# jiny2001/dcscn-super-resolution

Hardware: AMD Instinct MI355X
Metric: LR Mpixels/sec at 48x48 patches, L12_F196to48 x2 (higher is better)
Workload: dtype f32-equivalent (3x3 stack, wide 1x1 convs and folded tail: f16 hi/lo split, 3 products per MAC, f32 accumulate -- error at the f32 kernels' level, same parity bars; everything else f32)

## Files before the change

dcscn-super-resolution_amd/build.py:

```python

import os
import shutil
import subprocess
import sys
from concurrent.futures import ThreadPoolExecutor

PKG_DIR = os.path.dirname(os.path.abspath(__file__))
CSRC = os.path.join(PKG_DIR, "csrc")
INCLUDE = os.path.join(os.path.dirname(PKG_DIR), "include")
LIB_NAME = "libdcscn_hip.so"
LIB_PATH = os.path.join(PKG_DIR, LIB_NAME)
SOURCES = ["api.hip", "graph.hip", "pack.hip", "exec.hip", "kernels.hip", "resample.hip", "ensemble.hip", "color.hip", "metrics.hip", "conv_k1.hip", "conv_k3.hip", "conv_k5.hip", "conv_k7.hip", "conv_wino2.hip", "conv_nin.hip", "feat_stream.hip", "conv_nin_h.hip", "conv_nin_h_w8.hip", "conv3_h.hip", "conv3_h8.hip", "conv5_h.hip", "conv3_h_p16.hip", "conv3_h8_p16.hip", "feat_stream_redo.hip", "feat3_stream.hip", "train.hip", "train_data.hip"]
HEADERS = [os.path.join(CSRC, h) for h in ("kernels.h", "plan.h", "conv_igemm.hpp", "conv_wino2.hpp", "conv_nin.hpp", "conv_variants.hpp", "feat_stream.hpp", "tail_stream.hpp", "feat3_stream.hpp",
                                              "split16.hpp", "split16_pack.hpp", "p16.hpp", "conv_nin_h.hpp", "conv3_h.hpp", "conv3_h8.hpp", "conv5_h.hpp")] + \
          [os.path.join(INCLUDE, "dcscn.h")]
ARCH = "gfx950"
NO_PK_F32 = ["-Xclang", "-target-feature", "-Xclang", "-packed-fp32-ops"]
FLAGS = ["--offload-arch=" + ARCH, "-O3", "-std=c++17", "-fPIC", "-Wall", "-Wno-unused-function"] + NO_PK_F32
EXTRA_FLAGS = {"conv_wino2.hip": ["-fno-slp-vectorize", "-Rpass-analysis=kernel-resource-usage"],
               "conv_nin.hip": ["-fno-slp-vectorize", "-Rpass-analysis=kernel-resource-usage"],
               "conv_nin_h.hip": ["-fno-slp-vectorize", "-Rpass-analysis=kernel-resource-usage"], "conv_nin_h_w8.hip": ["-fno-slp-vectorize", "-Rpass-analysis=kernel-resource-usage"], "conv3_h.hip": ["-fno-slp-vectorize", "-Rpass-analysis=kernel-resource-usage"], "conv3_h8.hip": ["-fno-slp-vectorize", "-Rpass-analysis=kernel-resource-usage"], "conv3_h_p16.hip": ["-fno-slp-vectorize", "-Rpass-analysis=kernel-resource-usage"], "conv3_h8_p16.hip": ["-fno-slp-vectorize", "-Rpass-analysis=kernel-resource-usage"], "conv5_h.hip": ["-fno-slp-vectorize", "-Rpass-analysis=kernel-resource-usage"], "color.hip": ["-ffp-contract=off"], "metrics.hip": ["-ffp-contract=off"], "feat_stream.hip": ["-fno-slp-vectorize", "-Rpass-analysis=kernel-resource-usage"], "feat_stream_redo.hip": ["-fno-slp-vectorize"], "feat3_stream.hip": ["-fno-slp-vectorize", "-Rpass-analysis=kernel-resource-usage"]}
NO_SCRATCH = ("conv_wino2.hip", "conv_nin.hip", "feat_stream.hip", "conv_nin_h.hip", "conv_nin_h_w8.hip", "conv_nin_h_w8.hip", "conv3_h.hip", "conv3_h8.hip", "conv5_h.hip", "conv3_h_p16.hip", "conv3_h8_p16.hip", "feat3_stream.hip")


def hipcc_path():
    for cand in (shutil.which("hipcc"), "/opt/rocm/bin/hipcc"):
        if cand and os.path.isfile(cand):
            return cand
    raise RuntimeError("hipcc not found; the DCSCN HIP extension cannot be built")


def _stale(target, deps):
    if not os.path.isfile(target):
        return True
    t = os.path.getmtime(target)
    return any(os.path.getmtime(d) > t for d in deps)


def _run(cmd):
    proc = subprocess.run(cmd, stdout=subprocess.PIPE, stderr=subprocess.STDOUT, text=True)
    proc.stdout = "\n".join(ln for ln in proc.stdout.splitlines() if "'-packed-fp32-ops' is not a recognized feature" not in ln)
    if proc.returncode != 0:
        raise RuntimeError("command failed (%d): %s\n%s" % (proc.returncode, " ".join(cmd), proc.stdout))
    if any(cmd[-3].endswith(n) for n in NO_SCRATCH if len(cmd) >= 3):
        import re
        bad = [ln for ln in proc.stdout.splitlines() if re.search(r"(ScratchSize \[bytes/lane\]|VGPRs Spill): [1-9]", ln)]
        if bad:
            os.remove(cmd[-1])
            raise RuntimeError("register spill in a kernel that must not spill (%s):\n%s" % (cmd[-3], "\n".join(bad[:6])))
        return ""
    return proc.stdout


def build(force=False, verbose=False):
    hipcc = hipcc_path()
    obj_dir = os.path.join(PKG_DIR, "build")
    os.makedirs(obj_dir, exist_ok=True)
    jobs = []
    objs = []
    for src in SOURCES:
        src_path = os.path.join(CSRC, src)
        obj = os.path.join(obj_dir, os.path.splitext(src)[0] + ".o")
        objs.append(obj)
        if force or _stale(obj, [src_path, os.path.abspath(__file__)] + HEADERS):
            jobs.append([hipcc] + FLAGS + EXTRA_FLAGS.get(src, []) + ["-I", INCLUDE, "-c", src_path, "-o", obj])
    if jobs:
        with ThreadPoolExecutor(max_workers=len(jobs)) as pool:
            for out in pool.map(_run, jobs):
                if verbose and out.strip():
                    print(out, file=sys.stderr)
    if jobs or force or _stale(LIB_PATH, objs):
        out = _run([hipcc, "--offload-arch=" + ARCH, "-shared", "-fPIC"] + objs + ["-o", LIB_PATH])
        if verbose and out.strip():
            print(out, file=sys.stderr)
    return LIB_PATH


if __name__ == "__main__":
    print(build(force="--force" in sys.argv, verbose=True))
```

dcscn-super-resolution_amd/csrc/api.hip:

```cpp
#include "plan.h"

#pragma clang fp contract(off)

namespace dcscn_impl {

thread_local std::string g_global_error;

void set_global_error(const char* fmt, ...) {
    char buf[512];
    va_list ap;
    va_start(ap, fmt);
    vsnprintf(buf, sizeof buf, fmt, ap);
    va_end(ap);
    g_global_error = buf;
}

int fail(dcscn_ctx* h, int code, const char* fmt, ...) {
    char buf[512];
    va_list ap;
    va_start(ap, fmt);
    vsnprintf(buf, sizeof buf, fmt, ap);
    va_end(ap);
    if (h) h->error = buf;
    g_global_error = buf;
// ... 22 lines not shown
    if (!out || layers <= 0 || gamma <= 0.0) {
        set_global_error("dcscn_filter_schedule: bad arguments");
        return DCSCN_ERR_INVALID_ARG;
    }
    std::vector<int> s;
    filter_schedule(layers, filters, std::min(filters, min_filters), gamma, s);
    for (int i = 0; i < layers; ++i) out[i] = s[i];
    return DCSCN_OK;
}

int dcscn_create(const dcscn_config* cfg, int device, dcscn_handle* out) {
    if (!cfg || !out) return fail(nullptr, DCSCN_ERR_INVALID_ARG, "dcscn_create: null argument");
    *out = nullptr;
    if (cfg->struct_size != (int32_t)sizeof(dcscn_config))
        return fail(nullptr, DCSCN_ERR_INVALID_ARG, "dcscn_create: struct_size %d != %zu", cfg->struct_size, sizeof(dcscn_config));
    dcscn_config c = *cfg;
    c.min_filters = std::min(c.filters, c.min_filters);
    c.reconstruct_layers = std::max(c.reconstruct_layers, 1);
    if (c.scale < 2 || c.scale > 4) return fail(nullptr, DCSCN_ERR_UNSUPPORTED, "scale %d (supported: 2, 3, 4)", c.scale);
    if (c.layers < 1 || c.layers > 256 || c.filters < 1) return fail(nullptr, DCSCN_ERR_INVALID_ARG, "bad layers/filters");
    if (c.layers > 1 && !(c.filters_decay_gamma > 0.0)) return fail(nullptr, DCSCN_ERR_INVALID_ARG, "filters_decay_gamma must be > 0");
    if (c.cnn_size != 1 && c.cnn_size != 3 && c.cnn_size != 5 && c.cnn_size != 7)
        return fail(nullptr, DCSCN_ERR_UNSUPPORTED, "cnn_size %d (supported: 1, 3, 5, 7)", c.cnn_size);
    if (c.channels != 1) return fail(nullptr, DCSCN_ERR_UNSUPPORTED, "channels %d (the reference itself only supports 1)", c.channels);
    if (c.batch_norm) return fail(nullptr, DCSCN_ERR_UNSUPPORTED, "batch_norm is not implemented");
    float dummy;
    if (kernel_act(c.activator, &dummy) < 0) return fail(nullptr, DCSCN_ERR_INVALID_ARG, "Not implemented activator:%d", c.activator);
    if (c.legacy_no_c && c.use_nin) return fail(nullptr, DCSCN_ERR_INVALID_ARG, "legacy_no_c requires use_nin = 0");
    if (c.reconstruct_layers > 1 && c.reconstruct_filters < 1) return fail(nullptr, DCSCN_ERR_INVALID_ARG, "reconstruct_filters must be positive");

    int ndev = 0;
    hipError_t e = hipGetDeviceCount(&ndev);
    if (e != hipSuccess || ndev <= 0)
        return fail(nullptr, DCSCN_ERR_HIP, "no HIP device available (%s); this library has no CPU fallback",
                    e != hipSuccess ? hipGetErrorString(e) : "device count 0");
    if (device < 0 || device >= ndev) return fail(nullptr, DCSCN_ERR_INVALID_ARG, "device %d out of range [0, %d)", device, ndev);

    dcscn_ctx* h = new (std::nothrow) dcscn_ctx();
    if (!h) return fail(nullptr, DCSCN_ERR_NOMEM, "out of host memory");
    h->cfg = c;
    h->device = device;
    int rc = DCSCN_OK;
    do {
        if ((e = hipSetDevice(device)) != hipSuccess) { rc = fail(h, DCSCN_ERR_HIP, "hipSetDevice: %s", hipGetErrorString(e)); break; }
        hipDeviceProp_t prop;
        if ((e = hipGetDeviceProperties(&prop, device)) != hipSuccess) { rc = fail(h, DCSCN_ERR_HIP, "hipGetDeviceProperties: %s", hipGetErrorString(e)); break; }
        if (strncmp(prop.gcnArchName, "gfx950", 6) != 0) {
            rc = fail(h, DCSCN_ERR_HIP, "device %d is %s; this library is built for gfx950 (MI355X) only", device, prop.gcnArchName);
            break;
        }
        h->n_cus = prop.multiProcessorCount > 0 ? prop.multiProcessorCount : 256;
        if ((e = hipStreamCreateWithFlags(&h->stream, hipStreamNonBlocking)) != hipSuccess) { rc = fail(h, DCSCN_ERR_HIP, "hipStreamCreate: %s", hipGetErrorString(e)); break; }
        if ((e = hipEventCreateWithFlags(&h->done_ev, hipEventDisableTiming)) != hipSuccess) { rc = fail(h, DCSCN_ERR_HIP, "hipEventCreate: %s", hipGetErrorString(e)); break; }
        if ((e = conv_init_kernels()) != hipSuccess) { rc = fail(h, DCSCN_ERR_HIP, "kernel attribute setup: %s", hipGetErrorString(e)); break; }
        {
            size_t free_b = 0, total_b = 0;
            if (hipMemGetInfo(&free_b, &total_b) == hipSuccess && free_b > 0)
                h->workspace_budget = std::min<int64_t>(h->workspace_budget, std::max<int64_t>((int64_t)(free_b / 10 * 6), (int64_t)256 << 20));
        }
        rc = build_graph(h);
    } while (0);
    if (rc != DCSCN_OK) {
        g_global_error = h->error;
        dcscn_destroy(h);
        return rc;
    }
    *out = h;
    return DCSCN_OK;
}

int dcscn_num_tensors(dcscn_handle h) { return h ? (int)h->tensors.size() : -DCSCN_ERR_INVALID_ARG; }

int dcscn_tensor_info(dcscn_handle h, int index, char* name, int name_capacity, int64_t* shape, int* rank) {
    if (!h) return DCSCN_ERR_INVALID_ARG;
    if (index < 0 || index >= (int)h->tensors.size() || !name || name_capacity <= 0 || !shape || !rank)
        return fail(h, DCSCN_ERR_INVALID_ARG, "dcscn_tensor_info: bad argument");
    const TensorSpec& t = h->tensors[index];
    snprintf(name, (size_t)name_capacity, "%s", t.name.c_str());
    *rank = (int)t.shape.size();
    for (int i = 0; i < 4; ++i) shape[i] = i < *rank ? t.shape[i] : 1;
    return DCSCN_OK;
}

int dcscn_set_tensor(dcscn_handle h, const char* name, const float* data, const int64_t* shape, int rank) {
    if (!h) return DCSCN_ERR_INVALID_ARG;
    if (!name || !data || !shape) return fail(h, DCSCN_ERR_INVALID_ARG, "dcscn_set_tensor: null argument");
    if (h->finalized) return fail(h, DCSCN_ERR_STATE, "dcscn_set_tensor after dcscn_finalize");
    auto it = h->tensor_index.find(name);
    if (it == h->tensor_index.end()) return fail(h, DCSCN_ERR_SHAPE, "variable '%s' is not part of this graph", name);
    TensorSpec& t = h->tensors[it->second];
    bool same = rank == (int)t.shape.size();
    for (int i = 0; same && i < rank; ++i) same = shape[i] == t.shape[i];
    if (!same) {
        std::string want, got;
        for (int64_t d : t.shape) want += std::to_string(d) + ",";
        for (int i = 0; i < rank && i < 8; ++i) got += std::to_string(shape[i]) + ",";
        return fail(h, DCSCN_ERR_SHAPE, "variable '%s': shape [%s] does not match graph shape [%s]", name, got.c_str(), want.c_str());
    }
    size_t count = 1;
    for (int64_t d : t.shape) count *= (size_t)d;
    for (size_t i = 0; i < count; ++i)
        if (!std::isfinite(data[i])) return fail(h, DCSCN_ERR_INVALID_ARG, "variable '%s' holds a non-finite value", name);
    t.data.assign(data, data + count);
    t.set = true;
    return DCSCN_OK;
}

static int pack_ops(dcscn_ctx* h) {
    const size_t first = h->device_allocs.size();
    int rc = DCSCN_OK;
    for (Op& op : h->ops) {
        rc = finalize_op(h, op);
        if (rc) break;
    }
    h->pack_allocs.insert(h->pack_allocs.end(), h->device_allocs.begin() + first, h->device_allocs.end());
    h->device_allocs.resize(first);
    return rc;
}

}

namespace dcscn_impl {
int repack_weights(dcscn_ctx* h) {
    HIP_TRY(h, hipDeviceSynchronize());
    if (h->graph_exec) {
        (void)hipGraphExecDestroy(h->graph_exec);
        h->graph_exec = nullptr;
        h->graph_key = dcscn_ctx::GraphKey();
    }
    h->graph_seen = dcscn_ctx::GraphKey();
    for (void* p : h->pack_allocs) (void)hipFree(p);
    h->pack_allocs.clear();
    return pack_ops(h);
}
}

extern "C" {

int dcscn_finalize(dcscn_handle h) {
    if (!h) return DCSCN_ERR_INVALID_ARG;
    if (h->finalized) return DCSCN_OK;
    for (const TensorSpec& t : h->tensors)
        if (!t.set) return fail(h, DCSCN_ERR_MISSING_TENSOR, "variable '%s' was never set", t.name.c_str());
    HIP_TRY(h, hipSetDevice(h->device));
    if (h->fold_tail) fold_linear_tail(h);
    fuse_tail_stream(h);
    fuse_feat_stream(h);
    densify_features(h);
    fuse_feat3_stream(h);
    fold_whole_tail(h);
    int rc0 = pack_ops(h);
    if (rc0) return rc0;
    plan_p16(h);
    for (Op& op : h->ops) {
        int rc = DCSCN_OK;
        if (op.kind == OP_CONV && op.shape.nin && op.h16.on && op.h16.in16_ok) {
            op.h16.h_tab16.assign((size_t)4 * op.h16.n_chunks, NinSrcQuad{0, 0, 0});
            rc = upload(h, op.h16.h_tab16.data(), op.h16.h_tab16.size() * sizeof(NinSrcQuad), (void**)&op.h16.d_tab16);
            if (rc) return rc;
        }
        auto alloc_srctab = [&](Op& o) {
            if (o.multi.empty()) return (int)DCSCN_OK;
            o.h_srctab.assign(std::max<size_t>((size_t)4 * o.n_chunks, (size_t)8 * ((o.cin_phys + kNinHKC - 1) / kNinHKC)), NinSrcQuad{0, 0, 0});
            return upload(h, o.h_srctab.data(), o.h_srctab.size() * sizeof(NinSrcQuad), (void**)&o.d_srctab);
        };
        rc = alloc_srctab(op);
        if (rc) return rc;
        for (Op& sub : op.fused) {
            rc = alloc_srctab(sub);
            if (rc) return rc;
        }
    }
    h->finalized = true;
    return DCSCN_OK;
}

int dcscn_num_layers(dcscn_handle h) { return h ? (int)h->layers.size() : -DCSCN_ERR_INVALID_ARG; }

int dcscn_layer_info_get(dcscn_handle h, int index, dcscn_layer_info* out) {
    if (!h) return DCSCN_ERR_INVALID_ARG;
    if (!out || index < 0 || index >= (int)h->layers.size()) return fail(h, DCSCN_ERR_INVALID_ARG, "dcscn_layer_info_get: bad argument");
    *out = h->layers[index];
    return DCSCN_OK;
}

int dcscn_num_ops(dcscn_handle h) { return h ? (int)h->ops.size() : -DCSCN_ERR_INVALID_ARG; }

int dcscn_op_info_get(dcscn_handle h, int index, dcscn_op_info* out) {
    if (!h) return DCSCN_ERR_INVALID_ARG;
    if (!out || index < 0 || index >= (int)h->ops.size()) return fail(h, DCSCN_ERR_INVALID_ARG, "dcscn_op_info_get: bad argument");
    const Op& op = h->ops[index];
    memset(out, 0, sizeof *out);
    snprintf(out->name, sizeof out->name, "%s", op.name.c_str());
    const bool s16 = op_on_split16(h, op);
    snprintf(out->kernel, sizeof out->kernel, "%s", kernel_name(op_kernel(h, op)));
    out->kernel_size = op.ks;
    out->in_channels = op.cin;
    out->out_channels = op.cout;
    out->resolution = op.res;
    out->macs_per_lr_pixel = op.macs;
    out->bytes_per_lr_pixel = op.bytes;
    out->executed_macs_per_lr_pixel = op.macs;
    if (op.kind == OP_FOLDX && h->finalized && s16) {
        out->nt = 1; out->kc = 32; out->n_tiles = 1;
        out->executed_macs_per_lr_pixel = 3 * 25 * (int64_t)op.h16.n_chunks * 32 * 16;
    }
    if (op.kind == OP_CONV && h->finalized) {
        out->mt = op.shape.mt; out->nt = op.shape.nt; out->kc = op.shape.kc; out->n_tiles = op.n_tiles;
        const int64_t r2 = (int64_t)op.res * op.res;
        const int64_t k_exec = (int64_t)op.n_chunks * op.shape.kc;
        if (s16) {
            const int64_t tiles = (int64_t)op.h16.n_tiles * (op.h16.nt - 1) + op.h16.n_full;
            out->nt = op.h16.nt; out->kc = 32; out->n_tiles = op.h16.n_tiles;
            const int64_t ksteps = op.shape.nin ? op.h16.n_chunks : op.fold_s > 0 ? 25 * (int64_t)op.h16.n_chunks
                                                : 9 * (int64_t)(op.h16.n_chunks - (op.h16.tail_octs ? 1 : 0)) + (op.h16.tail_octs ? c3h_tail_steps(op.h16.tail_octs) : 0);
            out->executed_macs_per_lr_pixel = r2 * 3 * ksteps * 32 * tiles * 16;
        } else if (op.shape.nin) {
            const int64_t tiles = (int64_t)op.n_tiles * (op.shape.nt - 1) + op.n_full;
            out->executed_macs_per_lr_pixel = r2 * k_exec * tiles * 16;
        } else if (op.shape.wino) {
            const int64_t tiles = (int64_t)op.n_tiles * (op.shape.nt - 1) + op.n_full;
            out->executed_macs_per_lr_pixel = r2 * 4 * k_exec * tiles * 16;
        } else {
            out->executed_macs_per_lr_pixel = r2 * op.ks * op.ks * k_exec * (int64_t)op.n_tiles * op.shape.nt * 16;
        }
    }
    return DCSCN_OK;
}

int dcscn_set_option(dcscn_handle h, const char* key, int64_t value) {
    if (!h) return DCSCN_ERR_INVALID_ARG;
    if (!key) return fail(h, DCSCN_ERR_INVALID_ARG, "dcscn_set_option: null key");
    if (!strcmp(key, "sub_batch_pixels")) {
        if (value < 1) return fail(h, DCSCN_ERR_INVALID_ARG, "sub_batch_pixels must be >= 1");
        h->sub_batch_pixels = value;
        return DCSCN_OK;
    }
    if (!strcmp(key, "workspace_budget_bytes")) {
        if (value < 1) return fail(h, DCSCN_ERR_INVALID_ARG, "workspace_budget_bytes must be >= 1");
        h->workspace_budget = value;
        return DCSCN_OK;
    }
    if (!strcmp(key, "spatial_tiling")) {
        h->spatial_tiling = value != 0;
        return DCSCN_OK;
    }
    if (!strcmp(key, "fold_whole_tail")) {
        if (h->finalized) return fail(h, DCSCN_ERR_STATE, "the fold_whole_tail option must be set before dcscn_finalize");
        h->fold_whole = value != 0;
        return DCSCN_OK;
    }
    if (!strcmp(key, "fold_linear_tail")) {
        if (h->finalized) return fail(h, DCSCN_ERR_STATE, "the fold_linear_tail option must be set before dcscn_finalize");
        h->fold_tail = value != 0;
        h->fold_force = value == 2;
        return DCSCN_OK;
    }
    if (!strcmp(key, "stream_tail")) {
        if (h->finalized) return fail(h, DCSCN_ERR_STATE, "the stream_tail option must be set before dcscn_finalize");
        h->stream_tail = value != 0;
        return DCSCN_OK;
    }
    if (!strcmp(key, "stream_features")) {
        if (h->finalized) return fail(h, DCSCN_ERR_STATE, "the stream_features option must be set before dcscn_finalize");
        h->stream_features = value != 0;
        return DCSCN_OK;
    }
    if (!strcmp(key, "stream_nin")) {
        if (h->finalized) return fail(h, DCSCN_ERR_STATE, "the stream_nin option must be set before dcscn_finalize");
        h->stream_nin = value != 0;
        return DCSCN_OK;
    }
    if (!strcmp(key, "stream_dense")) {
        if (h->finalized) return fail(h, DCSCN_ERR_STATE, "the stream_dense option must be set before dcscn_finalize");
        h->stream_dense = value != 0;
        return DCSCN_OK;
    }
    if (!strcmp(key, "dense_features")) {
        if (h->finalized) return fail(h, DCSCN_ERR_STATE, "the dense_features option must be set before dcscn_finalize");
        h->dense_features = value != 0;
        return DCSCN_OK;
    }
    if (!strcmp(key, "nin_gemm")) {
        if (h->finalized) return fail(h, DCSCN_ERR_STATE, "the nin_gemm option must be set before dcscn_finalize");
        h->nin = value != 0;
        return DCSCN_OK;
    }
    if (!strcmp(key, "winograd")) {
        if (h->finalized) return fail(h, DCSCN_ERR_STATE, "the winograd option must be set before dcscn_finalize");
        h->winograd = value != 0;
        return DCSCN_OK;
    }
    if (!strcmp(key, "split16")) {
        h->split16 = value != 0;
        h->split16_mask = value == 2 ? 1 : value == 3 ? 2 : 3;
        return DCSCN_OK;
    }
    if (!strcmp(key, "p16")) {
        h->p16 = value != 0;
        return DCSCN_OK;
    }
    if (!strcmp(key, "conv3_h8")) {
        h->conv3_h8 = value != 0;
        return DCSCN_OK;
    }
    if (!strcmp(key, "nin_h8")) {
        h->nin_h8 = value != 0;
        return DCSCN_OK;
    }
    if (!strcmp(key, "debug_digest")) {
        if ((int)h->ops.size() + 1 > 1024) return fail(h, DCSCN_ERR_UNSUPPORTED, "debug_digest: more than 1023 launches");
        h->debug_digest = value != 0;
        return DCSCN_OK;
    }
    if (!strcmp(key, "debug_poison")) {
        h->debug_poison = (int)value;
        return DCSCN_OK;
    }
    if (!strcmp(key, "profile")) {
        h->profile = value != 0;
        return DCSCN_OK;
    }
    if (!strcmp(key, "graph_replay")) {
        h->graph_replay = value != 0;
        if (!h->graph_replay && h->graph_exec) {
            (void)hipGraphExecDestroy(h->graph_exec);
            h->graph_exec = nullptr;
        }
        h->graph_seen = dcscn_ctx::GraphKey{};
        return DCSCN_OK;
    }
    return fail(h, DCSCN_ERR_INVALID_ARG, "unknown option '%s'", key);
}

int dcscn_forward_device(dcscn_handle h, const float* x, const float* x2, float* y, int n, int height, int width, void* stream) {
    if (!h) return DCSCN_ERR_INVALID_ARG;
    if (h->finalized)
        if (int rc_ = train_sync_inference(h)) return rc_;
    return run_forward(h, x, x2, y, n, height, width, stream ? (hipStream_t)stream : h->stream);
}

static int ensure_io(dcscn_ctx* h, size_t lr_floats, size_t hr_floats) {
    int rc = grow(h, &h->io_x, &h->io_x_cap, lr_floats, h->stream, DCSCN_ERR_HIP);
    if (!rc) rc = grow(h, &h->io_x2, &h->io_x2_cap, hr_floats, h->stream, DCSCN_ERR_HIP);
    if (!rc) rc = grow(h, &h->io_y, &h->io_y_cap, hr_floats, h->stream, DCSCN_ERR_HIP);
    return rc;
}

static int forward_host_chunked(dcscn_ctx* h, const float* x, const float* x2, float* y, int n, int height, int width) {
    const int s = h->cfg.scale;
    const size_t lr1 = (size_t)height * width, hr1 = lr1 * s * s;
    int rc = ensure_io(h, lr1 * n, hr1 * n);
    if (rc) return rc;
    const int chunks = (hr1 * n * sizeof(float) >= ((size_t)8 << 20) && n >= 8) ? 4 : 1;
    while ((int)h->host_ev.size() < chunks) {
        hipEvent_t e;
        HIP_TRY(h, hipEventCreateWithFlags(&e, hipEventDisableTiming));
        h->host_ev.push_back(e);
    }
    int begin[5];
    for (int i = 0; i <= chunks; ++i) begin[i] = (int)((int64_t)n * i / chunks);
    auto span = [&](int i, int* b, int* cnt) { *b = begin[chunks - 1 - i] ; *cnt = begin[chunks - i] - begin[chunks - 1 - i]; };
    auto download = [&](int i) -> int {
        int b, cnt;
        span(i, &b, &cnt);
        HIP_TRY(h, hipEventSynchronize(h->host_ev[i]));
        HIP_TRY(h, hipMemcpy(y + (size_t)b * hr1, h->io_y + (size_t)b * hr1, (size_t)cnt * hr1 * sizeof(float), hipMemcpyDeviceToHost));
        return DCSCN_OK;
    };
    for (int i = 0; i < chunks; ++i) {
        int b, cnt;
        span(i, &b, &cnt);
        if (cnt > 0) {
            HIP_TRY(h, hipMemcpy(h->io_x + (size_t)b * lr1, x + (size_t)b * lr1, (size_t)cnt * lr1 * sizeof(float), hipMemcpyHostToDevice));
            if (x2) HIP_TRY(h, hipMemcpy(h->io_x2 + (size_t)b * hr1, x2 + (size_t)b * hr1, (size_t)cnt * hr1 * sizeof(float), hipMemcpyHostToDevice));
            else rc = resize_device(h, h->io_x + (size_t)b * lr1, h->io_x2 + (size_t)b * hr1, cnt, height, width, height * s, width * s, h->stream);
            if (!rc) rc = run_forward(h, h->io_x + (size_t)b * lr1, h->io_x2 + (size_t)b * hr1, h->io_y + (size_t)b * hr1, cnt, height, width, h->stream);
            if (rc) return rc;
        }
        HIP_TRY(h, hipEventRecord(h->host_ev[i], h->stream));
        if (i > 0 && (rc = download(i - 1))) return rc;
    }
    if ((rc = download(chunks - 1))) return rc;
    return DCSCN_OK;
}

int dcscn_forward(dcscn_handle h, const float* x, const float* x2, float* y, int n, int height, int width) {
    if (!h) return DCSCN_ERR_INVALID_ARG;
    if (!h->finalized) return fail(h, DCSCN_ERR_STATE, "dcscn_forward before dcscn_finalize");
    if (int rc_ = train_sync_inference(h)) return rc_;
    if (n < 0 || height <= 0 || width <= 0) return fail(h, DCSCN_ERR_INVALID_ARG, "bad shape n=%d h=%d w=%d", n, height, width);
    if (n == 0) return DCSCN_OK;
    if (!x || !x2 || !y) return fail(h, DCSCN_ERR_INVALID_ARG, "null image pointer");
    HIP_TRY(h, hipSetDevice(h->device));
    return forward_host_chunked(h, x, x2, y, n, height, width);
}

int dcscn_resample_table(int in_size, int out_size, int* ksize, int* bounds, double* weights, int capacity) {
    if (in_size <= 0 || out_size <= 0 || !ksize) return DCSCN_ERR_INVALID_ARG;
    std::vector<int> b;
    std::vector<double> k;
    *ksize = resample_coeffs(in_size, out_size, &b, &k);
    if (!bounds && !weights) return DCSCN_OK;
    if (!bounds || !weights || capacity < (int)k.size()) return DCSCN_ERR_INVALID_ARG;
    std::copy(b.begin(), b.end(), bounds);
    std::copy(k.begin(), k.end(), weights);
    return DCSCN_OK;
}

int dcscn_resize_bicubic(dcscn_handle h, const float* in, float* out, int n, int height, int width, int out_height, int out_width) {
    if (!h) return DCSCN_ERR_INVALID_ARG;
    if (n < 0 || height <= 0 || width <= 0 || out_height <= 0 || out_width <= 0)
        return fail(h, DCSCN_ERR_INVALID_ARG, "bad shape n=%d %dx%d -> %dx%d", n, height, width, out_height, out_width);
    if (n == 0) return DCSCN_OK;
    if (!in || !out) return fail(h, DCSCN_ERR_INVALID_ARG, "null image pointer");
    HIP_TRY(h, hipSetDevice(h->device));
    const size_t ni = (size_t)n * height * width, no = (size_t)n * out_height * out_width;
    int rc = grow(h, &h->rs_in, &h->rs_in_cap, ni, h->stream);
    if (!rc) rc = grow(h, &h->rs_out, &h->rs_out_cap, no, h->stream);
    if (rc) return rc;
    HIP_TRY(h, hipMemcpy(h->rs_in, in, ni * sizeof(float), hipMemcpyHostToDevice));
    rc = resize_device(h, h->rs_in, h->rs_out, n, height, width, out_height, out_width, h->stream);
    if (rc) return rc;
    HIP_TRY(h, hipStreamSynchronize(h->stream));
    HIP_TRY(h, hipMemcpy(out, h->rs_out, no * sizeof(float), hipMemcpyDeviceToHost));
    return DCSCN_OK;
}

int dcscn_resize_bicubic_device(dcscn_handle h, const float* in, float* out, int n, int height, int width, int out_height,
                                int out_width, void* stream) {
    if (!h) return DCSCN_ERR_INVALID_ARG;
    if (n < 0 || height <= 0 || width <= 0 || out_height <= 0 || out_width <= 0)
        return fail(h, DCSCN_ERR_INVALID_ARG, "bad shape n=%d %dx%d -> %dx%d", n, height, width, out_height, out_width);
    if (n == 0) return DCSCN_OK;
    if (!in || !out) return fail(h, DCSCN_ERR_INVALID_ARG, "null image pointer");
    HIP_TRY(h, hipSetDevice(h->device));
    hipStream_t st = stream ? (hipStream_t)stream : h->stream;
    if (h->has_last && h->last_stream != st) HIP_TRY(h, hipStreamWaitEvent(st, h->done_ev, 0));
    const int rc = resize_device(h, in, out, n, height, width, out_height, out_width, st);
    if (rc) return rc;
    return forward_done(h, st);
}

int dcscn_forward_lr(dcscn_handle h, const float* x, float* y, int n, int height, int width) {
    if (!h) return DCSCN_ERR_INVALID_ARG;
    if (!h->finalized) return fail(h, DCSCN_ERR_STATE, "dcscn_forward_lr before dcscn_finalize");
    if (int rc_ = train_sync_inference(h)) return rc_;
    if (n < 0 || height <= 0 || width <= 0) return fail(h, DCSCN_ERR_INVALID_ARG, "bad shape n=%d h=%d w=%d", n, height, width);
    if (n == 0) return DCSCN_OK;
    if (!x || !y) return fail(h, DCSCN_ERR_INVALID_ARG, "null image pointer");
    HIP_TRY(h, hipSetDevice(h->device));
    return forward_host_chunked(h, x, nullptr, y, n, height, width);
}

static int ensemble_on_device(dcscn_ctx* h, int height, int width, int n) {
    const int s = h->cfg.scale;
    const size_t lr = (size_t)height * width, hr = lr * s * s;
    const int na = std::min(n, 4), nb = n - na;
    int rc = grow(h, &h->ens_x, &h->ens_x_cap, n * lr, h->stream);
    if (!rc) rc = grow(h, &h->ens_x2, &h->ens_x2_cap, n * hr, h->stream);
    if (!rc) rc = grow(h, &h->ens_y, &h->ens_y_cap, n * hr, h->stream);
    if (!rc) rc = grow(h, &h->ens_out, &h->ens_out_cap, 2 * hr, h->stream);
// ... 158 lines not shown

static int metric_shape(dcscn_ctx* h, int height, int width, int border, const char* what, int* sh, int* sw) {
    if (height <= 0 || width <= 0) return fail(h, DCSCN_ERR_INVALID_ARG, "%s: bad shape h=%d w=%d", what, height, width);
    if (border < 0) return fail(h, DCSCN_ERR_INVALID_ARG, "%s: negative border_size %d (win_size cannot be placed)", what, border);
    *sh = height - 2 * border;
    *sw = width - 2 * border;
    if (*sh < kMetricTaps || *sw < 1)
        return fail(h, DCSCN_ERR_INVALID_ARG, "%s: win_size exceeds image extent (%d x %d after shaving %d: needs %d rows and 1 column)", what,
                    *sh, *sw, border, kMetricTaps);
    return DCSCN_OK;
}

static int metric_buffers(dcscn_ctx* h, int sh, int sw) {
    return grow(h, &h->met_buf, &h->met_buf_cap, (size_t)8 + 2 * (size_t)metric_segments(sh) * sw, h->stream);
}

static int metric_enqueue(dcscn_ctx* h, int slot, const double* a64, const float* a32, const double* b64, const float* b32, int width, int border,
                          int sh, int sw) {
    double* part_s = h->met_buf + 8;
    long long* part_e = reinterpret_cast<long long*>(part_s + (size_t)metric_segments(sh) * sw);
    HIP_TRY(h, metrics_launch(a64, a32, b64, b32, width, border, sh, sw, metric_weights(), part_s, part_e,
                              reinterpret_cast<long long*>(h->met_buf) + 4 * slot, h->stream));
    return DCSCN_OK;
}

static int metric_download(dcscn_ctx* h, dcscn_metrics* first, dcscn_metrics* second) {
    long long words[8];
    HIP_TRY(h, hipStreamSynchronize(h->stream));
    HIP_TRY(h, hipMemcpy(words, h->met_buf, sizeof words, hipMemcpyDeviceToHost));
    dcscn_metrics* outs[2] = {first, second};
    for (int i = 0; i < 2; ++i) {
        if (!outs[i]) continue;
        dcscn_metrics& m = *outs[i];
        m.sq_err_sum = words[4 * i];
        m.n_pixels = words[4 * i + 1];
        memcpy(&m.ssim, &words[4 * i + 2], sizeof(double));
        const double err = (double)m.sq_err_sum / (double)m.n_pixels;
        m.psnr = m.sq_err_sum == 0 ? (double)INFINITY : 10.0 * log10((255.0 * 255.0) / err);
    }
    return DCSCN_OK;
}

int dcscn_psnr_ssim(dcscn_handle h, const double* a, const double* b, int height, int width, int border_size, dcscn_metrics* out) {
    if (!h) return DCSCN_ERR_INVALID_ARG;
    if (!a || !b || !out) return fail(h, DCSCN_ERR_INVALID_ARG, "dcscn_psnr_ssim: null pointer");
    int sh, sw;
    int rc = metric_shape(h, height, width, border_size, "dcscn_psnr_ssim", &sh, &sw);
    if (rc) return rc;
    HIP_TRY(h, hipSetDevice(h->device));
    const size_t n = (size_t)height * width;
    rc = grow(h, &h->col_d, &h->col_d_cap, 2 * n, h->stream);
    if (!rc) rc = grow(h, &h->col_d2, &h->col_d2_cap, 2 * n, h->stream);
    if (!rc) rc = metric_buffers(h, sh, sw);
    if (rc) return rc;
    const double* da = reinterpret_cast<const double*>(h->col_d);
    const double* db = reinterpret_cast<const double*>(h->col_d2);
    HIP_TRY(h, hipMemcpy(h->col_d, a, n * sizeof(double), hipMemcpyHostToDevice));
    HIP_TRY(h, hipMemcpy(h->col_d2, b, n * sizeof(double), hipMemcpyHostToDevice));
    rc = metric_enqueue(h, 0, da, nullptr, db, nullptr, width, border_size, sh, sw);
    if (!rc) rc = metric_download(h, out, nullptr);
    return rc;
}

int dcscn_evaluate_rgb_metrics(dcscn_handle h, const uint8_t* rgb, int height, int width, int n_ensemble, int border_size, dcscn_metrics* model,
                               dcscn_metrics* bicubic, double* y) {
    if (!h) return DCSCN_ERR_INVALID_ARG;
    if (!h->finalized) return fail(h, DCSCN_ERR_STATE, "dcscn_evaluate_rgb_metrics before dcscn_finalize");
    if (!rgb || !model) return fail(h, DCSCN_ERR_INVALID_ARG, "dcscn_evaluate_rgb_metrics: null pointer");
    int sh, sw;
    int rc = metric_shape(h, height, width, border_size, "dcscn_evaluate_rgb_metrics", &sh, &sw);
    if (!rc) rc = evaluate_rgb_on_device(h, rgb, height, width, n_ensemble, "dcscn_evaluate_rgb_metrics");
    if (!rc) rc = metric_buffers(h, sh, sw);
    if (rc) return rc;
    const double* true_y = reinterpret_cast<const double*>(h->col_d);
    rc = metric_enqueue(h, 0, true_y, nullptr, n_ensemble > 1 ? reinterpret_cast<const double*>(h->ens_out) : nullptr,
                        n_ensemble > 1 ? nullptr : h->io_y, width, border_size, sh, sw);
    if (!rc && bicubic) rc = metric_enqueue(h, 1, true_y, nullptr, nullptr, h->io_x2, width, border_size, sh, sw);
    if (!rc) rc = metric_download(h, model, bicubic);
    if (!rc && y) rc = download_sr(h, (size_t)height * width, n_ensemble, y);
    return rc;
}

int dcscn_sr_rgb(dcscn_handle h, const uint8_t* rgb, const uint8_t* rgb_upscaled, int height, int width, int n_ensemble, double* y, double* rgb_out) {
    if (!h) return DCSCN_ERR_INVALID_ARG;
    if (!h->finalized) return fail(h, DCSCN_ERR_STATE, "dcscn_sr_rgb before dcscn_finalize");
    if (int rc_ = train_sync_inference(h)) return rc_;
    if (!rgb || !rgb_upscaled || !rgb_out) return fail(h, DCSCN_ERR_INVALID_ARG, "dcscn_sr_rgb: null pointer");
    if (n_ensemble < 1 || n_ensemble > 8) return fail(h, DCSCN_ERR_INVALID_ARG, "n_ensemble %d outside [1, 8]", n_ensemble);
    if (height <= 0 || width <= 0) return fail(h, DCSCN_ERR_INVALID_ARG, "bad shape h=%d w=%d", height, width);
    HIP_TRY(h, hipSetDevice(h->device));
    const int s = h->cfg.scale;
    const size_t lrn = (size_t)height * width, hr = lrn * s * s;
    int rc = ensure_io(h, lrn, hr);
    if (!rc) rc = grow(h, &h->col_rgb, &h->col_rgb_cap, (3 * hr + 3) / 4 + (3 * lrn + 3) / 4 + 4, h->stream);
    if (!rc) rc = grow(h, &h->col_d2, &h->col_d2_cap, 6 * hr, h->stream);
    if (rc) return rc;
    uint8_t* d_up = reinterpret_cast<uint8_t*>(h->col_rgb);
    uint8_t* d_lr = d_up + ((3 * hr + 15) & ~(size_t)15);
    HIP_TRY(h, hipMemcpy(d_lr, rgb, 3 * lrn, hipMemcpyHostToDevice));
    HIP_TRY(h, hipMemcpy(d_up, rgb_upscaled, 3 * hr, hipMemcpyHostToDevice));
    HIP_TRY(h, rgb_to_y_launch(d_lr, nullptr, h->io_x, (long long)lrn, h->stream));
    rc = sr_from_lr_on_device(h, height, width, n_ensemble);
    if (rc) return rc;
    HIP_TRY(h, y_cbcr_to_rgb_launch(n_ensemble > 1 ? reinterpret_cast<const double*>(h->ens_out) : nullptr, n_ensemble > 1 ? nullptr : h->io_y,
                                    nullptr, d_up, reinterpret_cast<double*>(h->col_d2), (long long)hr, h->stream));
    if (y) rc = download_sr(h, hr, n_ensemble, y);
    else HIP_TRY(h, hipStreamSynchronize(h->stream));
    if (rc) return rc;
    HIP_TRY(h, hipMemcpy(rgb_out, h->col_d2, 3 * hr * sizeof(double), hipMemcpyDeviceToHost));
    return DCSCN_OK;
}

int dcscn_get_profile(dcscn_handle h, double* ms, int capacity) {
    if (!h) return DCSCN_ERR_INVALID_ARG;
    if (!ms || capacity < 0) return fail(h, DCSCN_ERR_INVALID_ARG, "dcscn_get_profile: bad argument");
    const int nops = (int)h->ops.size();
    std::vector<double> acc(nops + 1, 0.0);
    const int forwards = h->ev_forwards;
    if (h->ev_used > 0) {
        HIP_TRY(h, hipDeviceSynchronize());
        const size_t launches = h->ev_used / 2;
        for (size_t l = 0; l < launches && l < h->ev_op.size(); ++l) {
            float t = 0.0f;
            HIP_TRY(h, hipEventElapsedTime(&t, h->ev[2 * l], h->ev[2 * l + 1]));
            acc[std::min(std::max(h->ev_op[l], 0), nops)] += t;
        }
    }
    h->ev_used = 0;
    h->ev_forwards = 0;
    h->ev_op.clear();
    if (forwards > 1)
        for (double& v : acc) v /= forwards;
    for (int i = 0; i < std::min(capacity, nops + 1); ++i) ms[i] = acc[i];
    return DCSCN_OK;
}

int dcscn_debug_digests(dcscn_handle h, uint64_t* out, int capacity) {
    if (!h) return DCSCN_ERR_INVALID_ARG;
    if (!out || capacity < 0) return fail(h, DCSCN_ERR_INVALID_ARG, "dcscn_debug_digests: bad argument");
    if (!h->d_digest) return fail(h, DCSCN_ERR_STATE, "dcscn_debug_digests: no forward has run with the debug_digest option on");
    HIP_TRY(h, hipDeviceSynchronize());
    const int n = std::min(capacity, (int)h->ops.size() + 1);
    HIP_TRY(h, hipMemcpy(out, h->d_digest, (size_t)n * sizeof(uint64_t), hipMemcpyDeviceToHost));
    return DCSCN_OK;
}

int64_t dcscn_workspace_bytes(dcscn_handle h) { return h ? (int64_t)h->arena_bytes : -1; }

int dcscn_num_presplit_tensors(dcscn_handle h) {
    if (!h) return -DCSCN_ERR_INVALID_ARG;
    if (!h->finalized || !p16_active(h)) return 0;
    int n = 0;
    for (const WsBuf& b : h->bufs) n += b.p16_ok && b.stride > 0;
    return n;
}

const char* dcscn_last_error(dcscn_handle h) { return h ? h->error.c_str() : g_global_error.c_str(); }

int dcscn_get_stream(dcscn_handle h, void** stream) {
    if (!h) return DCSCN_ERR_INVALID_ARG;
    if (!stream) return fail(h, DCSCN_ERR_INVALID_ARG, "dcscn_get_stream: null pointer");
    *stream = (void*)h->stream;
    return DCSCN_OK;
}

int dcscn_synchronize(dcscn_handle h) {
    if (!h) return DCSCN_ERR_INVALID_ARG;
    HIP_TRY(h, hipSetDevice(h->device));
    if (h->has_last) HIP_TRY(h, hipStreamSynchronize(h->last_stream));
    HIP_TRY(h, hipStreamSynchronize(h->stream));
    return DCSCN_OK;
}

int dcscn_destroy(dcscn_handle h) {
    if (!h) return DCSCN_OK;
    (void)hipSetDevice(h->device);
    if (h->has_last) (void)hipStreamSynchronize(h->last_stream);
    if (h->stream) (void)hipStreamSynchronize(h->stream);
    if (h->graph_exec) (void)hipGraphExecDestroy(h->graph_exec);
    if (h->done_ev) (void)hipEventDestroy(h->done_ev);
    for (hipEvent_t e : h->host_ev) (void)hipEventDestroy(e);
    for (hipEvent_t e : h->ev) (void)hipEventDestroy(e);
    train_free(h);
    train_batches_free(h);
    for (void* p : h->device_allocs) (void)hipFree(p);
    for (void* p : h->pack_allocs) (void)hipFree(p);
    if (h->arena) (void)hipFree(h->arena);
    if (h->d_zrec) (void)hipFree(h->d_zrec);
    if (h->d_digest) (void)hipFree(h->d_digest);
    for (float* p : {h->io_x, h->io_x2, h->io_y, h->tile_x, h->tile_x2, h->tile_y, h->rs_tmp, h->rs_in, h->rs_out, h->ens_x, h->ens_x2, h->ens_y, h->ens_out, h->col_rgb, h->col_d,
                     h->col_d2, h->col_y32})
        if (p) (void)hipFree(p);
    if (h->met_buf) (void)hipFree(h->met_buf);
    if (h->stream) (void)hipStreamDestroy(h->stream);
    delete h;
    return DCSCN_OK;
}

}
```

dcscn-super-resolution_amd/csrc/conv_nin_h.hip:

```cpp
#include "conv_nin_h.hpp"

namespace dcscn {

constexpr int kNinHStages = 3;
constexpr int kNinHMaxTable = 16 * 1024;

template <int NT>
static hipError_t nin_h_set_attr() {
    hipError_t e = hipFuncSetAttribute(reinterpret_cast<const void*>(&conv_nin_h<NT, 0, kNinHStages>), hipFuncAttributeMaxDynamicSharedMemorySize,
                                       NinHGeom<NT, kNinHStages>::LDS_BYTES);
    if (e != hipSuccess) return e;
    e = hipFuncSetAttribute(reinterpret_cast<const void*>(&conv_nin_h<NT, 2, kNinHStages>), hipFuncAttributeMaxDynamicSharedMemorySize,
                            NinHGeom<NT, kNinHStages>::LDS_BYTES + kNinHMaxTable);
    if (e != hipSuccess) return e;
    return hipFuncSetAttribute(reinterpret_cast<const void*>(&conv_nin_h<NT, 1, kNinHStages>), hipFuncAttributeMaxDynamicSharedMemorySize,
                               NinHGeom<NT, kNinHStages>::LDS_BYTES + kNinHMaxTable);
}

hipError_t nin_h8_init_kernels();
hipError_t nin_h8_launch(const ConvArgs& a, int n_groups, hipStream_t stream);
constexpr int kNinH8MinChunks = 32;

hipError_t nin_h_init_kernels() {
    hipError_t e = nin_h8_init_kernels();
    if (e != hipSuccess) return e;
    e = nin_h_set_attr<1>();
    if (e == hipSuccess) e = nin_h_set_attr<2>();
    if (e == hipSuccess) e = nin_h_set_attr<3>();
    if (e == hipSuccess) e = nin_h_set_attr<4>();
    if (e == hipSuccess) e = nin_h_set_attr<5>();
    return e != hipSuccess ? e : nin_h_set_attr<6>();
}

template <int NT>
static hipError_t nin_h_launch_one(const ConvArgs& a, int n_groups, hipStream_t stream) {
    using G = NinHGeom<NT, kNinHStages>;
    const long long npix = (long long)a.N * a.H * a.W;
    const dim3 grid((unsigned)((npix + G::PIX - 1) / G::PIX), (unsigned)n_groups);
    if (a.in16.base) {
        const size_t table = (size_t)a.n_chunks * 64;
        if (!a.srctab || table > (size_t)kNinHMaxTable || npix > kP16MaxPixels) return hipErrorInvalidValue;
        hipLaunchKernelGGL((conv_nin_h<NT, 2, kNinHStages>), grid, dim3(NinHGeom<NT, kNinHStages>::THREADS), G::LDS_BYTES + table, stream, a);
    } else if (a.srctab) {
        const size_t table = (size_t)a.n_chunks * 128;
        if (table > (size_t)kNinHMaxTable) return hipErrorInvalidValue;
        hipLaunchKernelGGL((conv_nin_h<NT, 1, kNinHStages>), grid, dim3(NinHGeom<NT, kNinHStages>::THREADS), G::LDS_BYTES + table, stream, a);
    } else {
        hipLaunchKernelGGL((conv_nin_h<NT, 0, kNinHStages>), grid, dim3(NinHGeom<NT, kNinHStages>::THREADS), G::LDS_BYTES, stream, a);
    }
    return hipGetLastError();
}

hipError_t nin_h_launch(int nt, const ConvArgs& a, int n_groups, bool w8, hipStream_t stream) {
    if (a.n_full < 1 || a.n_full > n_groups || (nt == 1 && a.n_full != n_groups) || !a.wpack16) return hipErrorInvalidValue;
    if (w8 && nt == 6 && a.in16.base && a.n_chunks >= kNinH8MinChunks && a.n_full == n_groups) return nin_h8_launch(a, n_groups, stream);
    switch (nt) {
        case 1: return nin_h_launch_one<1>(a, n_groups, stream);
        case 2: return nin_h_launch_one<2>(a, n_groups, stream);
        case 3: return nin_h_launch_one<3>(a, n_groups, stream);
        case 4: return nin_h_launch_one<4>(a, n_groups, stream);
        case 5: return nin_h_launch_one<5>(a, n_groups, stream);
        case 6: return nin_h_launch_one<6>(a, n_groups, stream);
        default: return hipErrorInvalidValue;
    }
}

}
```

dcscn-super-resolution_amd/csrc/conv_nin_h.hpp:

```cpp
#pragma once
#include "conv_nin.hpp"
#include "split16.hpp"
#include "p16.hpp"

namespace dcscn {

template <int NT, int S = 2, int WAVES = 4, int MT_ = 2>
struct NinHGeom {
    static constexpr int W = WAVES;
    static constexpr int THREADS = 64 * W;
    static constexpr int KC = 32;
    static constexpr int PIX = 16 * MT_ * W;
    static constexpr int MT = MT_;
    static constexpr int PSTRIDE = 128;
    static constexpr int A_SLOTS = PIX * 8;
    static constexpr int A_DMA = A_SLOTS / 64;
    static constexpr int A_BYTES = A_SLOTS * 16;
    static constexpr int A_ROUNDS = A_DMA / W;
    static constexpr int B_BYTES = NT * 2048;
    static constexpr int B_PIECES = 2 * NT;
    static constexpr int B_ROUNDS = (B_PIECES + W - 1) / W;
    static constexpr int B_STAGE = B_BYTES;
    static constexpr int B_BASE = S * A_BYTES;
    static constexpr int BA_BASE = S * A_BYTES + 2 * B_STAGE;
    static constexpr int LDS_BYTES = BA_BASE + NT * 128;
    static_assert(S == 2 || S == 3, "2 or 3 input stages");
};

template <int NT, int NTV, int SRC, int S, int WAVES, int MT>
__device__ __forceinline__ void conv_nin_h_body(const ConvArgs& a, float* smem, long long pix0, int ntile) {
    using G = NinHGeom<NT, S, WAVES, MT>;
    constexpr bool MULTI = SRC != 0, IN16 = SRC == 2;
    const int tid = threadIdx.x;
    const int lane = tid & 63;
    const int wave = __builtin_amdgcn_readfirstlane(tid >> 6);
    const int lj = lane & 15;
    const int lk = lane >> 4;
    const long long npix = (long long)a.N * a.H * a.W;
    const unsigned lds0 = (unsigned)(uintptr_t)(__attribute__((address_space(3))) float*)smem;

    const int d_kq = (((lane & 7) >> 1) - ((lane >> 4) & 3)) & 3;
    const int dq = 2 * d_kq + ((lane & 1) ^ (d_kq & 1));
    unsigned a_off[G::A_ROUNDS];
    long long a_pix[G::A_ROUNDS];
    static_for<0, G::A_ROUNDS>([&](auto r_) DCSCN_INL {
        constexpr int r = decltype(r_)::value;
        long long p = pix0 + (wave + G::W * r) * 8 + (lane >> 3);
        p = p < npix ? p : npix - 1;
        a_pix[r] = p;
        a_off[r] = (unsigned)((p - pix0) * a.in_stride * 4);
    });
    const float* a_base = a.in + (size_t)pix0 * a.in_stride + a.in_off;
    const char* b_base = reinterpret_cast<const char*>(a.wpack16) + (size_t)ntile * a.n_chunks * G::B_BYTES;
    const unsigned b_off = (unsigned)(lane * 16);

    auto dma_b = [&](auto r_, int chunk, unsigned stage) DCSCN_INL {
        constexpr int r = decltype(r_)::value;
        const int piece = (wave + G::W * r) % G::B_PIECES;
        glds16(b_base + (size_t)chunk * G::B_BYTES + 1024 * piece, b_off, lds0 + G::B_BASE + stage * G::B_STAGE + (unsigned)piece * 1024u);
    };
    typedef const volatile __attribute__((address_space(3))) u32x4* lds_u32x4_ptr;
    u32x4 ent = {0u, 0u, 0u, 0u};
    auto load_ent = [&](int chunk) DCSCN_INL {
        if constexpr (IN16) ent = *(lds_u32x4_ptr)(uintptr_t)(lds0 + G::LDS_BYTES + (unsigned)(chunk * 4 + d_kq) * 16u);
        else if constexpr (MULTI) ent = *(lds_u32x4_ptr)(uintptr_t)(lds0 + G::LDS_BYTES + (unsigned)(chunk * 8 + dq) * 16u);
    };
    auto dma_a = [&](auto r_, int chunk, unsigned stage) DCSCN_INL {
        constexpr int r = decltype(r_)::value;
        if constexpr (MULTI) {
            const char* src = reinterpret_cast<const char*>(((unsigned long long)ent.y << 32) | ent.x) + (unsigned long long)a_pix[r] * ent.z + (IN16 ? (dq & 1) * 16 : 0);
            glds16v(src, lds0 + stage * G::A_BYTES + (unsigned)(wave + G::W * r) * 1024u);
        } else {
            const int c0 = chunk * G::KC + 4 * dq;
            glds16(a_base, a_off[r] + (unsigned)((c0 < a.cin_phys ? c0 : 0) * 4), lds0 + stage * G::A_BYTES + (unsigned)(wave + G::W * r) * 1024u);
        }
    };

    {
        if constexpr (MULTI)
            for (int i = tid; i < (IN16 ? 4 : 8) * a.n_chunks; i += G::THREADS)
                *reinterpret_cast<f32x4*>(reinterpret_cast<char*>(smem) + G::LDS_BYTES + 16 * i) = reinterpret_cast<const f32x4*>(a.srctab)[i];
        __syncthreads();
    }

    if (tid < NTV * 4) *reinterpret_cast<f32x4*>(reinterpret_cast<char*>(smem) + G::BA_BASE + tid * 16) = reinterpret_cast<const f32x4*>(a.bias + ntile * NT * 16)[tid];
    else if (tid >= 64 && tid < 64 + NTV * 4 && a.act == ACT_ALPHA)
        *reinterpret_cast<f32x4*>(reinterpret_cast<char*>(smem) + G::BA_BASE + NT * 64 + (tid - 64) * 16) = reinterpret_cast<const f32x4*>(a.alpha + ntile * NT * 16)[tid - 64];

    f32x4 acc[G::MT][NTV];
    static_for<0, G::MT>([&](auto m_) DCSCN_INL {
        static_for<0, NTV>([&](auto n_) DCSCN_INL { acc[decltype(m_)::value][decltype(n_)::value] = f32x4{0.0f, 0.0f, 0.0f, 0.0f}; });
    });

    const unsigned a_rel = (unsigned)((16 * G::MT * wave + lj) * G::PSTRIDE + ((((lk + (lj >> 1)) & 3) << 1) | (lk & 1)) * 16);
    const unsigned a_lane = lds0 + a_rel, a_lane2 = lds0 + (a_rel ^ 16u);
    const unsigned b_lane = lds0 + (unsigned)(G::B_BASE + lane * 16);
    typedef const volatile __attribute__((address_space(3))) f32x4* lds_f32x4_ptr;
    typedef const volatile __attribute__((address_space(3))) h8* lds_h8_ptr;
    const float m1 = opaque_minus_one();

    const int last = a.n_chunks - 1;
    static_for<0, G::B_ROUNDS>([&](auto r_) DCSCN_INL { dma_b(r_, 0, 0); });
    load_ent(0);
    static_for<0, S>([&](auto st_) DCSCN_INL {
        constexpr int st = decltype(st_)::value;
        static_for<0, G::A_ROUNDS>([&](auto r_) DCSCN_INL { dma_a(r_, last < st ? last : st, st); });
        load_ent(last < st + 1 ? last : st + 1);
    });
    asm volatile("s_waitcnt vmcnt(0)" ::: "memory");
    __syncthreads();
    f32x4 xa[G::MT], xb[G::MT];
    static_for<0, G::MT>([&](auto m_) DCSCN_INL {
        constexpr int m = decltype(m_)::value;
        xa[m] = *(lds_f32x4_ptr)(uintptr_t)(a_lane + m * 16 * G::PSTRIDE);
        xb[m] = *(lds_f32x4_ptr)(uintptr_t)(a_lane2 + m * 16 * G::PSTRIDE);
    });
    __syncthreads();
    unsigned sa = 0;
    for (int chunk = 0; chunk < a.n_chunks; ++chunk) {
        const unsigned sb = chunk & 1;
        const int cb = chunk + 1 < last ? chunk + 1 : last;
        const int ca = chunk + S < last ? chunk + S : last;
        const unsigned sn = sa + 1 == S ? 0 : sa + 1;
        const unsigned Bs = b_lane + sb * G::B_STAGE;
        const unsigned An = a_lane + sn * G::A_BYTES, An2 = a_lane2 + sn * G::A_BYTES;
        static_for<0, G::B_ROUNDS>([&](auto r_) DCSCN_INL { dma_b(r_, cb, sb ^ 1); });
        f32x4 na[G::MT], nb[G::MT];
        static_for<0, G::MT>([&](auto m_) DCSCN_INL {
            constexpr int m = decltype(m_)::value;
            h8 xh, xl;
            if constexpr (IN16) { xh = __builtin_bit_cast(h8, xa[m]); xl = __builtin_bit_cast(h8, xb[m]); }
            else split8(xa[m], xb[m], m1, xh, xl);
            static_for<0, NTV>([&](auto n_) DCSCN_INL {
                constexpr int n = decltype(n_)::value;
                const h8 wh = *(lds_h8_ptr)(uintptr_t)(Bs + (2 * n) * 1024);
                const h8 wl = *(lds_h8_ptr)(uintptr_t)(Bs + (2 * n + 1) * 1024);
                acc[m][n] = __builtin_amdgcn_mfma_f32_16x16x32_f16(wl, xh, acc[m][n], 0, 0, 0);
                acc[m][n] = __builtin_amdgcn_mfma_f32_16x16x32_f16(wh, xl, acc[m][n], 0, 0, 0);
                acc[m][n] = __builtin_amdgcn_mfma_f32_16x16x32_f16(wh, xh, acc[m][n], 0, 0, 0);
                if constexpr (m * NTV + n < G::A_ROUNDS) dma_a(std::integral_constant<int, m * NTV + n>{}, ca, sa);
            });
            if constexpr (m == G::MT - 1 && G::MT * NTV < G::A_ROUNDS)
                static_for<G::MT * NTV, G::A_ROUNDS>([&](auto r_) DCSCN_INL { dma_a(r_, ca, sa); });
            na[m] = *(lds_f32x4_ptr)(uintptr_t)(An + m * 16 * G::PSTRIDE);
            nb[m] = *(lds_f32x4_ptr)(uintptr_t)(An2 + m * 16 * G::PSTRIDE);
        });
        load_ent(chunk + S + 1 < last ? chunk + S + 1 : last);
        if constexpr (S == 2) asm volatile("s_waitcnt vmcnt(0)" ::: "memory");
        else asm volatile("s_waitcnt vmcnt(%0)" ::"n"(G::A_ROUNDS) : "memory");
        __syncthreads();
        static_for<0, G::MT>([&](auto m_) DCSCN_INL { xa[decltype(m_)::value] = na[decltype(m_)::value]; xb[decltype(m_)::value] = nb[decltype(m_)::value]; });
        sa = sn;
    }
    if constexpr (S > 2) asm volatile("s_waitcnt vmcnt(0)" ::: "memory");

    const int cbase = ntile * NT * 16 + 4 * lk;
    const int obase = cbase - 16 * (ntile > a.n_full ? ntile - a.n_full : 0);
    const int act = a.act;
    const float inv = a.inv_scale;
    float chk[G::MT];
    static_for<0, G::MT>([&](auto m_) DCSCN_INL { chk[decltype(m_)::value] = 0.0f; });
    const float zero = opaque_zero();
    const h2 zero2 = p16_opaque_zero2();
    auto finish = [&](auto act_c) DCSCN_INL {
        constexpr int ACT_C = decltype(act_c)::value;
        const int act_e = ACT_C >= 0 ? ACT_C : act;
        static_for<0, NTV>([&](auto n_) DCSCN_INL {
            constexpr int n = decltype(n_)::value;
            const int c = obase + n * 16;
            const f32x4 bv = *reinterpret_cast<const f32x4*>(reinterpret_cast<const char*>(smem) + G::BA_BASE + (n * 4 + lk) * 16);
            f32x4 av = {0.0f, 0.0f, 0.0f, 0.0f};
            if (act_e == ACT_ALPHA) av = *reinterpret_cast<const f32x4*>(reinterpret_cast<const char*>(smem) + G::BA_BASE + NT * 64 + (n * 4 + lk) * 16);
            const bool first = c < a.split;
            float* optr = first ? a.out0.ptr : a.out1.ptr;
            const int ostride = first ? a.out0.stride : a.out1.stride;
            const int ooff = first ? a.out0.off : a.out1.off;
            const int owidth = first ? a.out0.width : a.out1.width;
            const int cc = first ? c : c - a.split;
            const OutDesc& od = first ? a.out0 : a.out1;
            if (od.p16.base != nullptr) {
                const int oct0 = (ooff + cc - 4 * lk) >> 3;
                const int chunk = oct0 >> 2, rem = od.p16.octs - 4 * chunk;
                const int rec = rem >= 4 ? 128 : 32 * rem;
                char* base = od.p16.base + (long long)chunk * od.p16.plane + 128 + (oct0 & 3) * 32 + lk * 16;
                const bool chan_ok = oct0 + (lk >> 1) < od.p16.octs;
                static_for<0, G::MT>([&](auto m_) DCSCN_INL {
                    constexpr int m = decltype(m_)::value;
                    const long long p = pix0 + 16 * G::MT * wave + 16 * m + lj;
                    f32x4 v = acc[m][n] * inv + bv;
                    v.x = activate1(v.x, av.x, act_e);
                    v.y = activate1(v.y, av.y, act_e);
                    v.z = activate1(v.z, av.z, act_e);
                    v.w = activate1(v.w, av.w, act_e);
                    if (ACT_C < 0 && p < npix && chan_ok) chk[m] = nonfinite_acc(chk[m], acc[m][n], zero);
                    const u32x4 unit = p16_unit(v, m1, chk[m], zero2, p < npix && chan_ok);
                    if (p < npix && chan_ok) *reinterpret_cast<u32x4*>(base + (size_t)p * rec) = unit;
                });
            } else if (cc < owidth) {
                static_for<0, G::MT>([&](auto m_) DCSCN_INL {
                    constexpr int m = decltype(m_)::value;
                    const long long p = pix0 + 16 * G::MT * wave + 16 * m + lj;
                    f32x4 v = acc[m][n] * inv + bv;
                    v.x = activate1(v.x, av.x, act_e);
                    v.y = activate1(v.y, av.y, act_e);
                    v.z = activate1(v.z, av.z, act_e);
                    v.w = activate1(v.w, av.w, act_e);
                    if (p < npix) {
                        chk[m] = nonfinite_acc(chk[m], acc[m][n], zero);
                        *reinterpret_cast<f32x4*>(optr + (size_t)p * ostride + ooff + cc) = v;
                    }
                });
            }
        });
    };
    if (act == ACT_ALPHA) finish(std::integral_constant<int, ACT_ALPHA>{});
    else if (act == ACT_NONE) finish(std::integral_constant<int, ACT_NONE>{});
    else finish(std::integral_constant<int, -1>{});
    static_for<0, G::MT>([&](auto m_) DCSCN_INL {
        constexpr int m = decltype(m_)::value;
        if (chk[m] != chk[m] && a.redo) {
            long long p = pix0 + 16 * G::MT * wave + 16 * m + lj;
            p = p < npix ? p : npix - 1;
            a.redo[0] = 1;
            a.redo[1 + (int)(p / ((long long)a.H * a.W))] = 1;
        }
    });
}

template <int NT, int SRC = 0, int S = 2, int WPS = 2, int WAVES = 4, int MT = 2>
__global__ __launch_bounds__(64 * WAVES, (WPS * WAVES / 4) * 128 / (16 * MT * WAVES) > 0 ? (WPS * WAVES / 4) * 128 / (16 * MT * WAVES) : 1) void conv_nin_h(const ConvArgs a) {
    extern __shared__ __attribute__((aligned(16))) float smem[];
    const long long pix0 = (long long)blockIdx.x * NinHGeom<NT, S, WAVES, MT>::PIX;
    const int ntile = blockIdx.y;
    if (ntile < a.n_full) conv_nin_h_body<NT, NT, SRC, S, WAVES, MT>(a, smem, pix0, ntile);
    else if constexpr (NT >= 2) conv_nin_h_body<NT, NT - 1, SRC, S, WAVES, MT>(a, smem, pix0, ntile);
}

}
```

dcscn-super-resolution_amd/csrc/conv_nin_h_w8.hip:

```cpp
#include "conv_nin_h.hpp"

namespace dcscn {

constexpr int kNinH8Stages = 3;
constexpr int kNinH8MaxTable = 16 * 1024;
constexpr int kNinH8Waves = 8, kNinH8Tiles = 2;

hipError_t nin_h8_init_kernels() {
    return hipFuncSetAttribute(reinterpret_cast<const void*>(&conv_nin_h<6, 2, kNinH8Stages, 2, kNinH8Waves, kNinH8Tiles>),
                               hipFuncAttributeMaxDynamicSharedMemorySize, NinHGeom<6, kNinH8Stages, kNinH8Waves, kNinH8Tiles>::LDS_BYTES + kNinH8MaxTable);
}

hipError_t nin_h8_launch(const ConvArgs& a, int n_groups, hipStream_t stream) {
    using G = NinHGeom<6, kNinH8Stages, kNinH8Waves, kNinH8Tiles>;
    const long long npix = (long long)a.N * a.H * a.W;
    const size_t table = (size_t)a.n_chunks * 64;
    if (!a.in16.base || !a.srctab || table > (size_t)kNinH8MaxTable || npix > kP16MaxPixels) return hipErrorInvalidValue;
    const dim3 grid((unsigned)((npix + G::PIX - 1) / G::PIX), (unsigned)n_groups);
    hipLaunchKernelGGL((conv_nin_h<6, 2, kNinH8Stages, 2, kNinH8Waves, kNinH8Tiles>), grid, dim3(G::THREADS), G::LDS_BYTES + table, stream, a);
    return hipGetLastError();
}

}
```

dcscn-super-resolution_amd/csrc/exec.hip:

```cpp
#include "plan.h"

#pragma clang fp contract(off)

namespace dcscn_impl {


static int ensure_workspace(dcscn_ctx* h, int nb, int H, int W, hipStream_t stream) {
    const bool want16 = p16_active(h);
    if (h->arena && nb <= h->lay_n && H == h->lay_h && W == h->lay_w && want16 == h->p16_now) return DCSCN_OK;
    std::vector<size_t> offsets(h->bufs.size()), sizes(h->bufs.size());
    size_t total = 0;
    for (size_t i = 0; i < h->bufs.size(); ++i) {
        const WsBuf& b = h->bufs[i];
        offsets[i] = total;
        sizes[i] = ws_tensor_bytes(b, (long long)nb * H * b.res * W * b.res, want16);
        total += ws_granules(sizes[i]);
    }
    const size_t redo_ints = 1 + (size_t)nb;
    h->redo_off = total;
    h->redo_ints = redo_ints;
    total += ws_granules(redo_ints * sizeof(int32_t));
    total = std::max<size_t>(total, 256);
    if (total > h->arena_bytes) {
        if (h->has_last) HIP_TRY(h, hipStreamSynchronize(h->last_stream));
        HIP_TRY(h, hipStreamSynchronize(h->stream));
        if (h->arena) HIP_TRY(h, hipFree(h->arena));
        h->arena = nullptr;
        h->arena_bytes = 0;
        h->lay_n = h->lay_h = h->lay_w = 0;
        hipError_t e = hipMalloc(&h->arena, total);
        if (e != hipSuccess) {
            (void)hipGetLastError();
            return fail(h, DCSCN_ERR_NOMEM, "workspace of %zu bytes: %s", total, hipGetErrorString(e));
        }
        h->arena_bytes = total;
    } else if (h->has_last && h->last_stream != stream) {
        HIP_TRY(h, hipStreamWaitEvent(stream, h->done_ev, 0));
    }
    for (size_t i = 0; i < h->bufs.size(); ++i) {
        WsBuf& b = h->bufs[i];
        b.offset = offsets[i];
        b.bytes = sizes[i];
        b.p16 = want16 && b.p16_ok && b.stride > 0;
        b.plane = p16_plane_bytes((long long)nb * H * b.res * W * b.res);
    }
    h->p16_now = want16;
    HIP_TRY(h, hipMemsetAsync(h->arena, 0, total, stream));
    h->carve_gen += 1;
    h->lay_n = nb;
    h->lay_h = H;
    h->lay_w = W;
    return DCSCN_OK;
}

static P16Desc p16_desc(const dcscn_ctx* h, int id) {
    const WsBuf& b = h->bufs[id];
    return P16Desc{static_cast<char*>(h->arena) + b.offset, b.plane, b.octs, 0};
}

bool op_on_split16(const dcscn_ctx* h, const Op& op) {
    if (op.kind == OP_STREAM || op.kind == OP_TAIL || op.kind == OP_STREAM3 || op.kind == OP_FOLDX) return h->split16 && op.h16.on && (h->split16_mask & 1);
    return op.kind == OP_CONV && h->split16 && op.h16.on && (h->split16_mask & (op.shape.nin ? 2 : 1));
}

static bool op_takes_h8(const dcscn_ctx* h, const Op& op) {
    if (!op_on_split16(h, op) || !h->conv3_h8 || op.shape.nin || op.fold_s > 0) return false;
    ConvArgs a{};
    a.n_full = op.h16.n_full; a.ps = op.ps; a.res = op.residual ? reinterpret_cast<const float*>(1) : nullptr; a.act = op.act; a.n_chunks = op.h16.n_chunks;
    if (!c3e_eligible(op.h16.nt, a, op.h16.n_tiles)) return false;
    const bool on16 = p16_active(h);
    const bool in16 = on16 && op.h16.in16_ok;
    bool all16 = true, any16 = false;
    for_each_dst(op, [&](int buf, int) {
        const bool o = on16 && buf >= 0 && h->bufs[buf].p16_ok && h->bufs[buf].stride > 0;
        all16 = all16 && o; any16 = any16 || o;
    });
    return in16 ? all16 : !any16;
}


Kernel op_kernel(const dcscn_ctx* h, const Op& op, bool redo) {
    const bool s16 = !redo && op_on_split16(h, op);
    switch (op.kind) {
        case OP_CONV:
            if (s16) return op.shape.nin ? K_CONV_NIN_H : op.fold_s > 0 ? K_CONV5_H : op_takes_h8(h, op) ? K_CONV3_H8 : K_CONV3_H;
            return op.shape.nin ? K_CONV_NIN : op.shape.wino ? K_CONV_WINO2 : K_CONV_IGEMM;
        case OP_CIN1: return K_CONV_CIN1;
        case OP_COUT1: return K_CONV_COUT1;
        case OP_DW: return K_DEPTHWISE;
        case OP_STREAM: return K_FEAT_STREAM;
        case OP_TAIL: return K_TAIL_STREAM;
        case OP_STREAM3: return s16 ? K_FEAT3_STREAM : K_LAYER_BY_LAYER;
        case OP_FOLDX: return s16 ? K_CONV5_H : K_LAYER_BY_LAYER;
    }
    return K_CONV_IGEMM;
}

const char* kernel_name(Kernel k) {
    static const char* const names[] = {"conv_igemm", "conv_wino2", "conv_nin", "conv_nin_h", "conv5_h", "conv3_h8", "conv3_h", "conv_cin1", "conv_cout1",
                                        "depthwise", "feat_stream", "tail_stream", "feat3_stream", "layer by layer"};
    static_assert(sizeof names / sizeof names[0] == K_LAYER_BY_LAYER + 1, "one name per Kernel");
    return names[k];
}

struct Pass {
    int nb, H, W;
    const float* x; const float* x2; float* y;
    hipStream_t stream;
    bool redo;
};

static int32_t* redo_flags(const dcscn_ctx* h) { return reinterpret_cast<int32_t*>(static_cast<char*>(h->arena) + h->redo_off); }

template <class Args>
static int stream_geometry(Args& a, const Pass& p, int halo, int workgroups) {
    a.N = p.nb; a.H = p.H; a.W = p.W;
    a.halo = halo;
    if (p.W <= kStreamPX) { a.n_strips = 1; a.useful_w = p.W; }
    else { a.useful_w = kStreamPX - 2 * a.halo; a.n_strips = (p.W + a.useful_w - 1) / a.useful_w; }
    const int64_t cols = (int64_t)p.nb * a.n_strips;
    const int want = (int)std::max<int64_t>(1, (512 + cols - 1) / cols);
    a.useful_h = std::max(32, (p.H + want - 1) / want);
    a.n_blocks = (p.H + a.useful_h - 1) / a.useful_h;
    a.rows_c = a.n_blocks == 1 ? p.H : a.useful_h + 2 * a.halo;
    a.n_jobs = (int)(cols * a.n_blocks);
    a.jobs_per_wg = (a.n_jobs + workgroups - 1) / workgroups;
    return (a.n_jobs + a.jobs_per_wg - 1) / a.jobs_per_wg;
}

static int launch_stream3(dcscn_ctx* h, const Op& op, const Pass& p) {
    Stream3Args a = op.stream3;
    a.x = p.x;
    a.blob = op.d_w;
    const int grid = stream_geometry(a, p, a.L + (a.nin.on ? 1 : 0), h->n_cus);
    auto out_desc = [&](int id, int lo, int hi) {
        S3Out o{};
        o.ptr = buf_ptr(h, id);
        o.stride = h->bufs[id].stride;
        o.width = h->bufs[id].stride;
        o.p16 = h->bufs[id].p16 ? p16_desc(h, id) : P16Desc{nullptr, 0, 0, 0};
        o.lo = lo; o.hi = hi < 0 ? o.width : hi;
        return o;
    };
    if (a.nin.on) {
        for (int i = 0; i < kS3MaxL; ++i) a.out[i] = S3Out{};
        a.out[a.L] = out_desc(op.extra_out[0], 0, 8);
        a.out2 = out_desc(op.extra_out[0], 8, 32);
    } else {
        for (size_t i = 0; i < op.extra_out.size(); ++i) a.out[i] = out_desc(op.extra_out[i], 0, -1);
    }
    a.redo = redo_flags(h);
    HIP_TRY(h, stream3_launch(a, grid, p.stream));
    return DCSCN_OK;
}

static int launch_foldx(dcscn_ctx* h, const Op& op, const Pass& p) {
    ConvArgs b{};
    b.in = buf_ptr(h, op.in_buf);
    b.in_stride = h->bufs[op.in_buf].stride;
    b.in_off = op.in_off;
    b.cin_phys = op.cin_phys;
    if (h->p16_now && op.h16.in16_ok) {
        b.in16 = p16_desc(h, op.in_buf);
        b.in = nullptr;
    }
    b.n_chunks = op.h16.n_chunks;
    b.wpack16 = op.h16.d_w;
    b.bias = op.h16.d_bias;
    b.inv_scale = op.h16.inv_scale;
    b.act = ACT_NONE;
    b.N = p.nb; b.H = p.H; b.W = p.W;
    b.tiles_x = (p.W + 15) / 16;
    b.tiles_y = (p.H + 15) / 16;
    b.out0.ptr = p.y; b.out0.stride = 1; b.out0.width = 1;
    b.out1 = b.out0;
    b.split = kNoSplit;
    b.ps = op.fold_s; b.ps_c = 1;
    b.res = p.x2; b.res_stride = 1;
    b.fold = 2;
    b.redo = redo_flags(h);
    HIP_TRY(h, c5h_launch(1, b, p.stream));
    HIP_TRY(h, c5h_border_launch(b, p.stream));
    return DCSCN_OK;
}

static int launch_tail(dcscn_ctx* h, const Op& op, const Pass& p, bool stream16) {
    TailArgs a = op.tail;
    a.c2 = buf_ptr(h, op.in_buf);
    a.c2_stride = h->bufs[op.in_buf].stride;
    a.x2 = p.x2;
    a.y = p.y;
    a.blob = stream16 ? static_cast<const float*>(op.h16.d_w) : op.d_w;
    a.redo = redo_flags(h); a.redo_check = p.redo ? 1 : 0;
    const int grid = stream_geometry(a, p, 2, 256);
    HIP_TRY(h, tail_launch(a, grid, stream16, p.stream));
    return DCSCN_OK;
}

static int launch_stream(dcscn_ctx* h, const Op& op, const Pass& p, bool stream16) {
    StreamArgs a = op.stream;
    a.x = p.x;
    a.out = buf_ptr(h, op.out_buf[0]);
    a.out_stride = h->bufs[op.out_buf[0]].stride;
    a.blob = stream16 ? static_cast<const float*>(op.h16.d_w) : op.d_w;
    a.redo = redo_flags(h); a.redo_check = p.redo ? 1 : 0;
    const int grid = stream_geometry(a, p, a.L + 1, 256);
    HIP_TRY(h, stream_launch(a, grid, stream16, p.stream));
    return DCSCN_OK;
}

static int launch_dw(dcscn_ctx* h, const Op& op, const Pass& p) {
    DwArgs a{};
    a.in = op.in_buf == EXT_X ? p.x : buf_ptr(h, op.in_buf);
    a.in_stride = op.in_buf == EXT_X ? 1 : h->bufs[op.in_buf].stride;
    a.in_off = op.in_off;
    a.chan_map = op.d_map;
    a.w = op.d_w;
    a.ks = op.ks;
    a.cin = op.cin;
    a.cout_phys = pad4(op.cin);
    a.N = p.nb; a.H = p.H * op.res; a.W = p.W * op.res;
    a.out = buf_ptr(h, op.out_buf[0]);
    a.out_stride = pad4(op.cin);
    a.redo = redo_flags(h); a.redo_check = p.redo ? 1 : 0;
    HIP_TRY(h, depthwise_launch(a, p.stream));
    return DCSCN_OK;
}

static int launch_cout1(dcscn_ctx* h, const Op& op, const Pass& p) {
    Cout1Args a{};
    a.in = buf_ptr(h, op.in_buf);
    a.in_stride = h->bufs[op.in_buf].stride;
    a.in_off = op.in_off;
    a.cin_phys = op.cin_phys;
    a.w = op.d_w;
    a.scale = op.out_scale;
    a.bias = 0.0f;
    a.ks = op.ks;
    a.N = p.nb; a.H = p.H * op.res; a.W = p.W * op.res;
    a.out = p.y;
    a.out_stride = 1;
    a.res = op.residual ? p.x2 : nullptr;
    a.res_stride = 1;
    a.redo = redo_flags(h); a.redo_check = p.redo ? 1 : 0;
    HIP_TRY(h, cout1_launch(a, p.stream));
    return DCSCN_OK;
}

static int launch_cin1(dcscn_ctx* h, const Op& op, const Pass& p) {
    Cin1Args a{};
    a.x = p.x;
    a.w = op.d_w; a.bias = op.d_bias; a.alpha = op.d_alpha;
    a.act = op.act;
    a.ks = op.ks;
    a.N = p.nb; a.H = p.H * op.res; a.W = p.W * op.res;
    a.cs = op.out_width[0];
    a.out.ptr = buf_ptr(h, op.out_buf[0]);
    a.out.stride = h->bufs[op.out_buf[0]].stride;
    a.out.off = op.out_off[0];
    a.out.width = op.out_width[0];
    if (!p.redo && h->bufs[op.out_buf[0]].p16) a.out.p16 = p16_desc(h, op.out_buf[0]);
    a.redo = redo_flags(h); a.redo_check = p.redo ? 1 : 0;
    HIP_TRY(h, cin1_launch(a, p.stream));
    return DCSCN_OK;
}

static int launch_conv(dcscn_ctx* h, const Op& op, const Pass& p, Kernel kernel) {
    const int Hr = p.H * op.res, Wr = p.W * op.res;
    ConvArgs a{};
    a.in = buf_ptr(h, op.in_buf);
    a.in_stride = op.in_stride_override > 0 ? op.in_stride_override : h->bufs[op.in_buf].stride;
    a.in_off = op.in_off;
    a.cin_phys = op.cin_phys;
    a.n_chunks = op.n_chunks;
    a.wpack = op.d_w; a.bias = op.d_bias; a.alpha = op.d_alpha;
    a.act = op.act;
    a.N = p.nb; a.H = Hr; a.W = Wr;
    a.tiles_x = (Wr + 15) / 16;
    a.tiles_y = (Hr + 4 * op.shape.mt - 1) / (4 * op.shape.mt);
    a.n_full = op.n_full;
    for (int i = 0; i < 2; ++i) {
        OutDesc& o = i == 0 ? a.out0 : a.out1;
        const int id = op.out_buf[i];
        o.ptr = id == EXT_Y ? p.y : buf_ptr(h, id);
        o.stride = id == EXT_Y ? 1 : h->bufs[id].stride;
        o.off = op.out_off[i];
        o.width = op.out_width[i];
    }
    a.split = op.split;
    a.ps = op.ps;
    a.ps_c = op.ps == 1 ? 1 : op.ps_c;
    a.vec4 = op.vec4 ? 1 : 0;
    a.res = op.residual ? p.x2 : nullptr;
    a.res_stride = 1;
    a.dww = op.d_dww;
    a.dwk = op.dwk;
    a.fold = op.fold_s > 0 ? 1 : 0;
    a.srctab = op.multi.empty() ? nullptr : op.d_srctab;
    a.redo = redo_flags(h);
    if (kernel == K_CONV_NIN || kernel == K_CONV_WINO2 || kernel == K_CONV_IGEMM) {
        a.redo_check = p.redo ? 1 : 0;
        if (kernel == K_CONV_NIN) HIP_TRY(h, nin_launch(op.shape.nt, a, op.n_tiles, p.stream));
        else if (kernel == K_CONV_WINO2) HIP_TRY(h, wino_launch(op.shape.nt, a, op.n_tiles, p.stream));
        else HIP_TRY(h, conv_launch(op.shape, a, op.n_tiles, p.stream));
        return DCSCN_OK;
    }
    ConvArgs b = a;
    b.wpack16 = op.h16.d_w;
    b.inv_scale = op.h16.inv_scale;
    b.n_chunks = op.h16.n_chunks;
    b.n_full = op.h16.n_full;
    if (h->p16_now && op.h16.in16_ok) {
        b.in16 = p16_desc(h, op.multi.empty() ? op.in_buf : op.multi[0].first);
        b.in = nullptr;
        if (op.shape.nin) b.srctab = op.h16.d_tab16;
    }
    if (op.out_buf[0] >= 0 && h->bufs[op.out_buf[0]].p16) b.out0.p16 = p16_desc(h, op.out_buf[0]);
    if (op.out_buf[1] >= 0 && h->bufs[op.out_buf[1]].p16) b.out1.p16 = p16_desc(h, op.out_buf[1]);
    if (kernel == K_CONV_NIN_H) {
        HIP_TRY(h, nin_h_launch(op.h16.nt, b, op.h16.n_tiles, h->nin_h8, p.stream));
    } else if (kernel == K_CONV5_H) {
        b.bias = op.h16.d_bias;
        HIP_TRY(h, c5h_launch(op.h16.nt, b, p.stream));
    } else {
        b.bias = op.h16.d_bias;
        b.tail_octs = op.h16.tail_octs;
        b.alpha = op.h16.d_alpha;
        b.tiles_y = (Hr + 15) / 16;
        if (kernel == K_CONV3_H8) HIP_TRY(h, c3e_launch(op.h16.nt, b, op.h16.n_tiles, h->n_cus, p.stream));
        else HIP_TRY(h, c3h_launch(op.h16.nt, b, op.h16.n_tiles, p.stream));
    }
    return DCSCN_OK;
}

static int launch_op(dcscn_ctx* h, const Op& op, const Pass& p) {
    const Kernel kernel = op_kernel(h, op, p.redo);
    if (kernel == K_LAYER_BY_LAYER) {
        for (const Op& sub : op.fused) {
            const int rc = launch_op(h, sub, p);
            if (rc) return rc;
        }
        return DCSCN_OK;
    }
    switch (op.kind) {
        case OP_STREAM3: return launch_stream3(h, op, p);
        case OP_FOLDX: return launch_foldx(h, op, p);
        case OP_TAIL: return launch_tail(h, op, p, !p.redo && op_on_split16(h, op));
        case OP_STREAM: return launch_stream(h, op, p, !p.redo && op_on_split16(h, op));
        case OP_DW: return launch_dw(h, op, p);
        case OP_COUT1: return launch_cout1(h, op, p);
        case OP_CIN1: return launch_cin1(h, op, p);
        case OP_CONV: return launch_conv(h, op, p, kernel);
    }
    return DCSCN_OK;
}

static int halo_lr_pixels(const dcscn_ctx* h) {
    double r = 0.0;
    for (const Op& op : h->ops) {
        const int k = op.kind == OP_CONV && op.dwk ? op.dwk : op.ks;
        r += (double)(op.halo >= 0 ? op.halo : k / 2) / op.res;
    }
    return (int)std::ceil(r - 1e-9);
}

static int run_tiled(dcscn_ctx* h, const float* x, const float* x2, float* y, int n, int H, int W, int64_t pass_pixels, hipStream_t stream) {
    const int R = halo_lr_pixels(h), s = h->cfg.scale;
    int Ht = (int)std::min<int64_t>(H, std::max<int64_t>(1, (int64_t)std::sqrt((double)pass_pixels)));
    int Wt = (int)std::min<int64_t>(W, std::max<int64_t>(1, pass_pixels / Ht));
    if (Wt == W) Ht = (int)std::min<int64_t>(H, pass_pixels / Wt);
    if ((Ht < H && Ht <= 2 * R) || (Wt < W && Wt <= 2 * R))
        return fail(h, DCSCN_ERR_NOMEM, "image %dx%d needs spatial tiling, but a pass of %lld LR pixels is too small for windows "
                    "with a %d-pixel halo; raise sub_batch_pixels / workspace_budget_bytes", H, W, (long long)pass_pixels, R);
    auto starts = [&](int full, int win) {
        std::vector<int> v;
        if (win >= full) { v.push_back(0); return v; }
        const int stride = win - 2 * R;
        for (int a = 0; a + win < full; a += stride) v.push_back(a);
        v.push_back(full - win);
        return v;
    };
    const std::vector<int> ys = starts(H, Ht), xs = starts(W, Wt);
    const size_t tiles = (size_t)n * ys.size() * xs.size();
    const size_t lr = tiles * Ht * Wt, hr = lr * s * s;
    if ((lr > h->tile_x_cap || hr > h->tile_x2_cap || hr > h->tile_y_cap) && h->has_last) HIP_TRY(h, hipStreamSynchronize(h->last_stream));
    int rc = grow(h, &h->tile_x, &h->tile_x_cap, lr, stream, DCSCN_ERR_HIP);
    if (!rc) rc = grow(h, &h->tile_x2, &h->tile_x2_cap, hr, stream, DCSCN_ERR_HIP);
    if (!rc) rc = grow(h, &h->tile_y, &h->tile_y_cap, hr, stream, DCSCN_ERR_HIP);
    if (rc) return rc;
    size_t t = 0;
    for (int img = 0; img < n; ++img)
        for (int wy : ys)
            for (int wx : xs) {
                HIP_TRY(h, hipMemcpy2DAsync(h->tile_x + t * Ht * Wt, (size_t)Wt * sizeof(float),
                                            x + ((size_t)img * H + wy) * W + wx, (size_t)W * sizeof(float),
                                            (size_t)Wt * sizeof(float), Ht, hipMemcpyDeviceToDevice, stream));
                HIP_TRY(h, hipMemcpy2DAsync(h->tile_x2 + t * Ht * Wt * s * s, (size_t)Wt * s * sizeof(float),
                                            x2 + ((size_t)img * H * s + (size_t)wy * s) * W * s + (size_t)wx * s, (size_t)W * s * sizeof(float),
                                            (size_t)Wt * s * sizeof(float), (size_t)Ht * s, hipMemcpyDeviceToDevice, stream));
                ++t;
            }
    if ((rc = run_forward(h, h->tile_x, h->tile_x2, h->tile_y, (int)tiles, Ht, Wt, stream))) return rc;
    auto owned = [&](const std::vector<int>& st, size_t i, int full, int* lo, int* hi) {
        *lo = st[i] + (st[i] > 0 ? R : 0);
        *hi = i + 1 < st.size() ? st[i + 1] + R : full;
    };
    t = 0;
    for (int img = 0; img < n; ++img)
        for (size_t iy = 0; iy < ys.size(); ++iy)
            for (size_t ix = 0; ix < xs.size(); ++ix) {
                int y0, y1, x0, x1;
                owned(ys, iy, H, &y0, &y1);
                owned(xs, ix, W, &x0, &x1);
                if (y1 > y0 && x1 > x0) {
                    const float* src = h->tile_y + t * Ht * Wt * s * s + ((size_t)(y0 - ys[iy]) * s) * Wt * s + (size_t)(x0 - xs[ix]) * s;
                    float* dst = y + ((size_t)img * H * s + (size_t)y0 * s) * W * s + (size_t)x0 * s;
                    HIP_TRY(h, hipMemcpy2DAsync(dst, (size_t)W * s * sizeof(float), src, (size_t)Wt * s * sizeof(float),
                                                (size_t)(x1 - x0) * s * sizeof(float), (size_t)(y1 - y0) * s,
                                                hipMemcpyDeviceToDevice, stream));
                }
                ++t;
            }
    return DCSCN_OK;
}


static void pass_pixels(const dcscn_ctx* h, int64_t* pass, int64_t* budget) {
    const bool want16 = p16_active(h);
    constexpr long long kRef = 1 << 20;
    int64_t ws_per_lr_pixel = 0;
    for (const WsBuf& b : h->bufs) ws_per_lr_pixel += (int64_t)b.res * b.res * (int64_t)(ws_tensor_bytes(b, kRef, want16) / kRef);
    ws_per_lr_pixel += (ws_per_lr_pixel + 63) / 64;
    *budget = h->workspace_budget / std::max<int64_t>(ws_per_lr_pixel, 1);
    if (want16) *budget = std::min<int64_t>(*budget, kP16MaxPixels / ((int64_t)h->p16_max_res * h->p16_max_res));
    *pass = std::min(h->sub_batch_pixels, *budget);
}

static int refill_tables(dcscn_ctx* h, hipStream_t stream) {
    std::vector<Op*> with_tables;
    for (Op& op : h->ops) {
        with_tables.push_back(&op);
        for (Op& sub : op.fused) with_tables.push_back(&sub);
    }
    for (Op* opp : with_tables) {
        Op& op = *opp;
        if (op.multi.empty() || !op.d_srctab) continue;
        const unsigned long long pad_ptr = (unsigned long long)(uintptr_t)buf_ptr(h, op.multi[0].first);
        size_t q = 0;
        for (const auto& sg : op.multi) {
            const char* base = reinterpret_cast<const char*>(buf_ptr(h, sg.first));
            const unsigned stride = (unsigned)(h->bufs[sg.first].stride * sizeof(float));
            for (int c4 = 0; c4 < ((sg.second + 7) & ~7) / 4 && q < op.h_srctab.size(); ++c4, ++q)
                op.h_srctab[q] = c4 < sg.second / 4 ? NinSrcQuad{(unsigned long long)(uintptr_t)(base + 16 * c4), stride, 1u} : NinSrcQuad{pad_ptr, 0, 0};
        }
        for (; q < op.h_srctab.size(); ++q) op.h_srctab[q] = NinSrcQuad{pad_ptr, 0, 0};
        HIP_TRY(h, hipMemcpyAsync(op.d_srctab, op.h_srctab.data(), op.h_srctab.size() * sizeof(NinSrcQuad), hipMemcpyHostToDevice, stream));
    }
    for (Op& op : h->ops) {
        if (!op.h16.d_tab16 || !h->p16_now || !op.h16.in16_ok) continue;
        std::vector<std::pair<int, int>> srcs = op.multi;
        if (srcs.empty()) srcs.push_back({op.in_buf, op.cin_phys});
        const unsigned long long zero_rec = (unsigned long long)(uintptr_t)buf_ptr(h, srcs[0].first);
        size_t q = 0;
        for (const auto& sg : srcs) {
            const WsBuf& wb = h->bufs[sg.first];
            const char* base = reinterpret_cast<const char*>(buf_ptr(h, sg.first));
            for (int o = 0; o < wb.octs && q < op.h16.h_tab16.size(); ++o, ++q)
                op.h16.h_tab16[q] = NinSrcQuad{(unsigned long long)(uintptr_t)(base + (long long)(o >> 2) * wb.plane + 128 + (o & 3) * 32),
                                               (unsigned)p16_rec_bytes(wb.octs, o >> 2), 1u};
        }
        for (; q < op.h16.h_tab16.size(); ++q) op.h16.h_tab16[q] = NinSrcQuad{zero_rec, 0, 0};
        HIP_TRY(h, hipMemcpyAsync(op.h16.d_tab16, op.h16.h_tab16.data(), op.h16.h_tab16.size() * sizeof(NinSrcQuad), hipMemcpyHostToDevice, stream));
    }
    h->h_zrec.clear();
    for (const WsBuf& wb : h->bufs)
        if (wb.p16)
            for (int c = 0; c < (wb.octs + 3) / 4; ++c) h->h_zrec.push_back((unsigned long long)(uintptr_t)(static_cast<char*>(h->arena) + wb.offset + (long long)c * wb.plane));
    if (!h->h_zrec.empty()) {
        if (h->h_zrec.size() > h->zrec_cap) {
            const int rc = grow(h, &h->d_zrec, &h->zrec_cap, h->h_zrec.size() * 2, stream, DCSCN_ERR_HIP);
            if (rc) return rc;
        }
        HIP_TRY(h, hipMemcpyAsync(h->d_zrec, h->h_zrec.data(), h->h_zrec.size() * sizeof(unsigned long long), hipMemcpyHostToDevice, stream));
    }
    h->tables_gen = h->carve_gen;
    return DCSCN_OK;
}

static int profile_begin(dcscn_ctx* h, int op_index, const Pass& p, size_t* evi) {
    *evi = h->ev_used;
    h->ev_used += 2;
    h->ev_op.push_back(op_index);
    HIP_TRY(h, hipEventRecord(h->ev[*evi], p.stream));
    return DCSCN_OK;
}

static int run_pass(dcscn_ctx* h, const Pass& p) {
    const int nops = (int)h->ops.size(), s = h->cfg.scale;
    const size_t y_floats = (size_t)p.nb * p.H * s * p.W * s;
    bool any_h16 = false;
    for (const Op& op : h->ops) any_h16 = any_h16 || op_on_split16(h, op);
    if (any_h16)
        HIP_TRY(h, pass_begin_launch(redo_flags(h), (int)h->redo_ints, h->p16_now ? h->d_zrec : nullptr, h->p16_now ? (int)h->h_zrec.size() : 0, p.stream));
    for (int i = 0; i < nops; ++i) {
        const Op& op = h->ops[i];
        size_t evi = 0;
        if (h->profile)
            if (int rc = profile_begin(h, i, p, &evi)) return rc;
        if (h->debug_poison) HIP_TRY(h, debug_poison_launch(h->debug_poison, p.stream));
        if (int rc = launch_op(h, op, p)) return rc;
        if (h->profile) HIP_TRY(h, hipEventRecord(h->ev[evi + 1], p.stream));
        if (h->debug_digest) {
            for (int k = 0; k < 2; ++k) {
                const int idx = op.out_buf[k];
                if (k == 1 && idx == op.out_buf[0]) break;
                if (idx >= 0) {
                    const WsBuf& wb = h->bufs[idx];
                    HIP_TRY(h, debug_digest_launch(static_cast<const char*>(h->arena) + wb.offset, wb.p16 ? wb.bytes / 4 : (size_t)p.nb * p.H * wb.res * p.W * wb.res * wb.stride, h->d_digest + i, p.stream));
                } else if (idx == EXT_Y) {
                    HIP_TRY(h, debug_digest_launch(p.y, y_floats, h->d_digest + i, p.stream));
                }
            }
        }
    }
    if (any_h16) {
        Pass redo = p;
        redo.redo = true;
        size_t evi = 0;
        if (h->profile)
            if (int rc = profile_begin(h, nops, p, &evi)) return rc;
        for (const Op& op : h->ops) {
            if (!op.h16.rerun) continue;
            if (int rc = launch_op(h, op, redo)) return rc;
        }
        if (h->profile) HIP_TRY(h, hipEventRecord(h->ev[evi + 1], p.stream));
    }
    if (h->debug_digest) HIP_TRY(h, debug_digest_launch(p.y, y_floats, h->d_digest + nops, p.stream));
    return DCSCN_OK;
}

struct CaptureGuard {
    hipStream_t stream;
    bool capturing = false;
    ~CaptureGuard() {
        if (!capturing) return;
        hipGraph_t g = nullptr;
        (void)hipStreamEndCapture(stream, &g);
        if (g) (void)hipGraphDestroy(g);
    }
};

int forward_done(dcscn_ctx* h, hipStream_t stream) {
    HIP_TRY(h, hipEventRecord(h->done_ev, stream));
    h->last_stream = stream;
    h->has_last = true;
    return DCSCN_OK;
}

int run_forward(dcscn_ctx* h, const float* x, const float* x2, float* y, int n, int H, int W, hipStream_t stream) {
    if (!h->finalized) return fail(h, DCSCN_ERR_STATE, "dcscn_forward before dcscn_finalize");
    if (n < 0 || H <= 0 || W <= 0) return fail(h, DCSCN_ERR_INVALID_ARG, "bad shape n=%d h=%d w=%d", n, H, W);
    if (n == 0) return DCSCN_OK;
    if (!x || !x2 || !y) return fail(h, DCSCN_ERR_INVALID_ARG, "null image pointer");
    HIP_TRY(h, hipSetDevice(h->device));
    const int64_t per_image = (int64_t)H * W;
    int64_t pass_px, budget_px;
    pass_pixels(h, &pass_px, &budget_px);
    if (h->has_last && h->last_stream != stream) HIP_TRY(h, hipStreamWaitEvent(stream, h->done_ev, 0));
    if (per_image > budget_px && h->spatial_tiling) return run_tiled(h, x, x2, y, n, H, W, budget_px, stream);
    int nb = (int)std::max<int64_t>(1, std::min<int64_t>(n, pass_px / per_image));
    int rc = ensure_workspace(h, nb, H, W, stream);
    while (rc == DCSCN_ERR_NOMEM && nb > 1) {
        nb = (nb + 1) / 2;
        rc = ensure_workspace(h, nb, H, W, stream);
    }
    if (rc) return rc;
    if (h->tables_gen != h->carve_gen)
        if ((rc = refill_tables(h, stream))) return rc;
    const int s = h->cfg.scale;
    const int batches = (n + nb - 1) / nb;
    const int nops = (int)h->ops.size();
    if (h->profile) {
        const size_t need = h->ev_used + (size_t)batches * (nops + 1) * 2;
        while (h->ev.size() < need) {
            hipEvent_t e;
            HIP_TRY(h, hipEventCreate(&e));
            h->ev.push_back(e);
        }
        h->ev_forwards += 1;
    }
    dcscn_ctx::GraphKey gkey;
    gkey.x = x; gkey.x2 = x2; gkey.y = y; gkey.stream = stream; gkey.n = n; gkey.H = H; gkey.W = W;
    gkey.split16 = h->split16 ? h->split16_mask : 0;
    gkey.nb = nb;
    gkey.h8 = h->conv3_h8 ? 1 : 0;
    gkey.nin_h8 = h->nin_h8 ? 1 : 0;
    gkey.p16 = h->p16_now ? 1 : 0;
    gkey.carve = (unsigned long long)h->carve_gen;
    const bool graphs = h->graph_replay && !h->profile && !h->debug_digest && !h->debug_poison;
    if (graphs && h->graph_exec && gkey == h->graph_key) {
        HIP_TRY(h, hipGraphLaunch(h->graph_exec, stream));
        return forward_done(h, stream);
    }
    CaptureGuard capture{stream};
    if (graphs && gkey == h->graph_seen) {
        if (hipStreamBeginCapture(stream, hipStreamCaptureModeThreadLocal) == hipSuccess) capture.capturing = true;
        else (void)hipGetLastError();
    }
    h->graph_seen = gkey;
    if (h->debug_digest) {
        if (nops + 1 > 1024) return fail(h, DCSCN_ERR_UNSUPPORTED, "debug_digest: more than 1023 launches");
        if (!h->d_digest) HIP_TRY(h, hipMalloc((void**)&h->d_digest, 1024 * sizeof(unsigned long long)));
        HIP_TRY(h, hipMemsetAsync(h->d_digest, 0, 1024 * sizeof(unsigned long long), stream));
    }
    for (int b = 0; b < batches; ++b) {
        const size_t b0 = (size_t)b * nb;
        const Pass pass{std::min(nb, n - b * nb), H, W, x + b0 * H * W, x2 + b0 * H * s * W * s, y + b0 * H * s * W * s, stream, false};
        if ((rc = run_pass(h, pass))) return rc;
    }
    if (capture.capturing) {
        capture.capturing = false;
        hipGraph_t g = nullptr;
        hipError_t ce = hipStreamEndCapture(stream, &g);
        if (h->graph_exec) {
            (void)hipGraphExecDestroy(h->graph_exec);
            h->graph_exec = nullptr;
        }
        if (ce == hipSuccess) ce = hipGraphInstantiate(&h->graph_exec, g, nullptr, nullptr, 0);
        if (g) (void)hipGraphDestroy(g);
        if (ce == hipSuccess) ce = hipGraphLaunch(h->graph_exec, stream);
        if (ce != hipSuccess) {
            (void)hipGetLastError();
            if (h->graph_exec) (void)hipGraphExecDestroy(h->graph_exec);
            h->graph_exec = nullptr;
            h->graph_seen = dcscn_ctx::GraphKey{};
            const bool was = h->graph_replay;
            h->graph_replay = false;
            const int rr = run_forward(h, x, x2, y, n, H, W, stream);
            h->graph_replay = was;
            return rr;
        }
        h->graph_key = gkey;
    }
    return forward_done(h, stream);
}

int resample_table(dcscn_ctx* h, int in_size, int out_size, const dcscn_ctx::ResampleTable** out) {
    auto key = std::make_pair(in_size, out_size);
    auto it = h->resample_tables.find(key);
    if (it == h->resample_tables.end()) {
        std::vector<int> bounds;
        std::vector<double> kk;
        dcscn_ctx::ResampleTable t;
        t.ksize = resample_coeffs(in_size, out_size, &bounds, &kk);
        int rc = upload(h, bounds.data(), bounds.size() * sizeof(int), (void**)&t.d_bounds);
        if (!rc) rc = upload(h, kk.data(), kk.size() * sizeof(double), (void**)&t.d_kk);
        if (rc) return rc;
        it = h->resample_tables.emplace(key, t).first;
    }
    *out = &it->second;
    return DCSCN_OK;
}

int resize_device(dcscn_ctx* h, const float* in, float* out, int n, int H, int W, int OH, int OW, hipStream_t stream) {
    if (n <= 0) return DCSCN_OK;
    const float* src = in;
    if (OW != W) {
        const dcscn_ctx::ResampleTable* t;
        int rc = resample_table(h, W, OW, &t);
        if (rc) return rc;
        float* dst = out;
        if (OH != H) {
            rc = grow(h, &h->rs_tmp, &h->rs_tmp_cap, (size_t)n * H * OW, stream);
            if (rc) return rc;
            dst = h->rs_tmp;
        }
        HIP_TRY(h, resample_h_launch(src, dst, t->d_bounds, t->d_kk, t->ksize, (long long)n * H, W, OW, stream));
        src = dst;
    }
    if (OH != H) {
        const dcscn_ctx::ResampleTable* t;
        int rc = resample_table(h, H, OH, &t);
        if (rc) return rc;
        HIP_TRY(h, resample_v_launch(src, out, t->d_bounds, t->d_kk, t->ksize, n, H, OH, OW, stream));
    } else if (OW == W) {
        HIP_TRY(h, hipMemcpyAsync(out, in, (size_t)n * H * W * sizeof(float), hipMemcpyDeviceToDevice, stream));
    }
    return DCSCN_OK;
}

}
```

dcscn-super-resolution_amd/csrc/graph.hip:

```cpp
#include "plan.h"

#pragma clang fp contract(off)

namespace dcscn_impl {

void filter_schedule(int layers, int filters, int min_filters, double gamma, std::vector<int>& out) {
    out.clear();
    int n = filters;
    for (int i = 0; i < layers; ++i) {
        if (min_filters != 0 && i > 0) {
            const double x1 = (double)i / (double)(layers - 1);
            const double y1 = std::pow(x1, 1.0 / gamma);
            const double v = (double)(filters - min_filters) * (1.0 - y1) + (double)min_filters;
            n = (int)v;
        }
        out.push_back(n);
    }
}

int add_tensor(dcscn_ctx* h, const std::string& name, std::vector<int64_t> shape) {
    TensorSpec t;
    t.name = name;
    t.shape = std::move(shape);
    h->tensors.push_back(std::move(t));
// ... 619 lines not shown
    }
    if (consumers.empty() || h->concat_slices.size() < 2) return;
    std::vector<int> nb;
    for (const auto& sl : h->concat_slices) nb.push_back(new_buf(h, pad4(sl.second), 1));
    for (Op& op : h->ops) {
        for (size_t k = 0; k < h->concat_slices.size(); ++k) {
            const int off = h->concat_slices[k].first, w4 = pad4(h->concat_slices[k].second);
            for (int o = 0; o < 2; ++o)
                if (op.out_buf[o] == cat && op.out_off[o] == off) { op.out_buf[o] = nb[k]; op.out_off[o] = 0; }
            if (op.in_buf == cat && op.in_off == off && op.cin_phys == w4 && !(off == 0 && w4 == cat_stride)) { op.in_buf = nb[k]; op.in_off = 0; }
        }
    }
    for (int ci : consumers) {
        Op& op = h->ops[ci];
        for (size_t k = 0; k < nb.size(); ++k) op.multi.push_back({nb[k], pad4(h->concat_slices[k].second)});
    }
    release_if_unused(h, cat);
}

void fuse_feat3_stream(dcscn_ctx* h) {
    const dcscn_config& c = h->cfg;
    const int L = c.layers;
    if (!h->stream_dense || c.depthwise_separable || c.cnn_size != 3 || L < 2 || L > kS3MaxL || (int)h->ops.size() < L) return;
    int waves = 1;
    size_t lds = 0;
    for (int i = 0; i < L; ++i) {
        if (h->sched[i] > 32) return;
        if (i > 0) waves += 1;
        if (i + 1 < L) lds += (size_t)4 * kStreamRowPx * (2 * ((h->sched[i] + 7) / 8) + 1) * 16;
    }
    if (waves > kS3MaxWaves || lds > 158 * 1024) return;
    const Op& c1 = h->ops[0];
    if (c1.kind != OP_CIN1 || c1.ks != 3 || c1.in_buf != EXT_X || c1.act != ACT_ALPHA || c1.out_off[0] != 0 || c1.out_buf[0] < 0 || c1.segs.size() != 1) return;
    for (int i = 1; i < L; ++i) {
        const Op& o = h->ops[i];
        if (o.kind != OP_CONV || o.ks != 3 || o.dwk != 0 || o.ps != 1 || o.residual || o.act != ACT_ALPHA || o.segs.size() != 1 || o.tconv_s > 0 || o.fold_s > 0 ||
            o.res != 1 || o.cin != h->sched[i - 1] || o.cout != h->sched[i] || o.in_buf != h->ops[i - 1].out_buf[0] || o.in_off != 0 || o.out_off[0] != 0 ||
            o.out_buf[0] < 0 || has_second_dst(o) || !o.multi.empty())
            return;
        for (size_t k = 0; k < o.chan_map.size(); ++k)
            if (o.chan_map[k] != (int)k) return;
        for (int k = 0; k < i; ++k)
            if (h->ops[k].out_buf[0] == o.out_buf[0]) return;
    }
    bool nin_on = false;
    if (h->stream_nin && c.use_nin && L == 7 && c.nin_filters2 == 8 && c.nin_filters == 24 && (int)h->ops.size() >= L + 2) {
        const Op& nin = h->ops[L];
        const Op& b2 = h->ops[L + 1];
        auto octs = [&](int i) { return (h->sched[i] + 7) / 8; };
        bool ok = nin.kind == OP_CONV && nin.ks == 1 && nin.dwk == 0 && nin.segs.size() == 2 && nin.act == ACT_ALPHA && nin.ps == 1 && !nin.residual &&
                  nin.segs[0].dw1 < 0 && nin.segs[1].dw1 < 0 && (int)nin.multi.size() == L && nin.out_buf[0] >= 0 && nin.out_buf[1] >= 0 &&
                  nin.out_off[0] == 0 && nin.out_off[1] == 8 && nin.cin == [&] { int k = 0; for (int i = 0; i < L; ++i) k += h->sched[i]; return k; }();
        for (int i = 0; ok && i < L; ++i) ok = nin.multi[i].first == h->ops[i].out_buf[0];
        ok = ok && b2.kind == OP_CONV && b2.ks == 3 && b2.dwk == 0 && b2.cin == 8 && b2.cout == 8 && b2.act == ACT_ALPHA && b2.ps == 1 && !b2.residual &&
             b2.segs.size() == 1 && b2.in_buf == nin.out_buf[0] && b2.in_off == 0 && b2.out_buf[0] == nin.out_buf[1] && b2.out_off[0] == 0 &&
             !has_second_dst(b2) && b2.tconv_s == 0 && b2.fold_s == 0 && b2.res == 1 && h->bufs[nin.out_buf[1]].stride == 32;
        ok = ok && octs(L - 4) == 3 && octs(L - 3) == 2 && octs(L - 2) == 2 && h->sched[L - 3] <= 16 && h->sched[L - 2] <= 16 && h->sched[L - 1] <= 16;
        const size_t lds2 = lds + (size_t)4 * kStreamRowPx * (2 * octs(L - 1) + 1) * 16 + (size_t)4 * kStreamRowPx * 3 * 16;
        nin_on = ok && lds2 <= 158 * 1024;
    }
    Op f;
    f.kind = OP_STREAM3;
    f.name = "CNN1.." + h->ops[nin_on ? L + 1 : L - 1].name + " (streamed)";
    f.ks = 3;
    f.cin = 1;
    f.cout = nin_on ? c.nin_filters + c.nin_filters2 : h->sched[L - 1];
    f.res = 1;
    f.act = ACT_ALPHA;
    f.in_buf = EXT_X;
    f.out_buf[0] = f.out_buf[1] = nin_on ? h->ops[L].out_buf[1] : h->ops[L - 1].out_buf[0];
    f.out_width[0] = nin_on ? 32 : pad4(h->sched[L - 1]);
    f.halo = nin_on ? L + 1 : L;
    f.bytes = 4;
    const int n_rep = nin_on ? L + 2 : L;
    for (int i = 0; i < n_rep; ++i) {
        f.macs += h->ops[i].macs;
        if (!nin_on) {
            f.bytes += 4 * (int64_t)pad4(h->sched[i]);
            f.extra_out.push_back(h->ops[i].out_buf[0]);
        }
        f.fused.push_back(h->ops[i]);
    }
    if (nin_on) {
        f.bytes += 4 * 32;
        f.extra_out.push_back(f.out_buf[0]);
        f.stream3.nin.on = 1;
    }
    h->ops.erase(h->ops.begin(), h->ops.begin() + n_rep);
    h->ops.insert(h->ops.begin(), f);
}

void plan_p16(dcscn_ctx* h) {
    const size_t nbuf = h->bufs.size();
    std::vector<char> ok(nbuf, 0), written(nbuf, 0), read(nbuf, 0);
    for (size_t b = 0; b < nbuf; ++b) ok[b] = h->bufs[b].stride > 0;
    auto can_read = [&](const Op& op) {
        if ((op.kind != OP_CONV && op.kind != OP_FOLDX) || !op.h16.on || op.dwk != 0 || op.in_stride_override > 0) return false;
        if (!op.multi.empty()) return op.shape.nin != 0;
        if (op.in_buf < 0 || op.in_off != 0 || op.cin_phys != h->bufs[op.in_buf].stride) return false;
        for (size_t i = 0; i < op.chan_map.size(); ++i)
            if (op.chan_map[i] != (int)i) return false;
        return true;
    };
    auto can_write = [&](const Op& op, int k) {
        if (op.kind == OP_STREAM3) return op.h16.on;
        if (op.kind == OP_CIN1) return k == 0 && op.out_off[0] == 0 && op.ks <= 3;
        if (op.kind != OP_CONV || !op.h16.on || op.fold_s > 0 || op.residual || op.dwk != 0) return false;
        if (op.ps != 1 && (op.shape.nin || op.ps_c % 16 != 0 || k != 0 || has_second_dst(op))) return false;
        if (op.out_off[k] % 16 != 0) return false;
        return k == 0 || op.split % 16 == 0;
    };
    for (bool changed = true; changed;) {
        changed = false;
        for (const Op& op : h->ops) {
            const std::vector<int> in = op_inputs(op);
            bool all = can_read(op);
            for (int b : in) all = all && ok[b];
            if (!all)
                for (int b : in)
                    if (ok[b]) { ok[b] = 0; changed = true; }
            for_each_dst(op, [&](int b, int k) {
                if (b >= 0 && ok[b] && !can_write(op, k)) { ok[b] = 0; changed = true; }
            });
        }
    }
    for (const Op& op : h->ops) {
        for (int b : op_inputs(op)) read[b] = 1;
        for_each_dst(op, [&](int b, int) { if (b >= 0) written[b] = 1; });
    }
    h->any_p16 = false;
    h->p16_max_res = 1;
    for (size_t b = 0; b < nbuf; ++b) {
        WsBuf& wb = h->bufs[b];
        wb.p16_ok = ok[b] && written[b] && read[b];
        wb.octs = (wb.stride + 7) / 8;
        if (wb.p16_ok) { h->any_p16 = true; h->p16_max_res = std::max(h->p16_max_res, wb.res); }
    }
    for (Op& op : h->ops) {
        const std::vector<int> in = op_inputs(op);
        bool all = !in.empty() && can_read(op);
        for (int b : in) all = all && h->bufs[b].p16_ok;
        op.h16.in16_ok = all;
    }
    std::vector<char> dirty(nbuf, 0);
    for (Op& op : h->ops) {
        bool r = (op.kind == OP_CONV || op.kind == OP_STREAM || op.kind == OP_TAIL || op.kind == OP_STREAM3 || op.kind == OP_FOLDX) && op.h16.on;
        for (int b : op_inputs(op)) r = r || dirty[b];
        for_each_dst(op, [&](int b, int) { r = r || (b >= 0 && h->bufs[b].p16_ok); });
        op.h16.rerun = r;
        if (r) for_each_dst(op, [&](int b, int) { if (b >= 0) dirty[b] = 1; });
    }
}

}
```

dcscn-super-resolution_amd/csrc/kernels.h:

```cpp
#pragma once
#include <hip/hip_runtime.h>
#include <stdint.h>

#include <vector>

namespace dcscn {

enum { ACT_NONE = 0, ACT_ALPHA = 1, ACT_SIGMOID = 2, ACT_TANH = 3, ACT_SELU = 4 };

struct P16Desc {
    char*     base;
    long long plane;
    int32_t   octs;
    int32_t   pad_;
};
__host__ __device__ constexpr int p16_rec_bytes(int octs, int chunk) { return octs - 4 * chunk >= 4 ? 128 : 32 * (octs - 4 * chunk); }
__host__ __device__ constexpr long long p16_plane_bytes(long long npix) { return ((npix + 1) * 128 + 255) & ~255LL; }
__host__ __device__ constexpr long long p16_tensor_bytes(long long npix, int octs) {
    return ((octs + 3) / 4 - 1) * p16_plane_bytes(npix) + ((128 + npix * p16_rec_bytes(octs, (octs + 3) / 4 - 1) + 255) & ~255LL);
}
constexpr long long kP16MaxPixels = (1LL << 25) - 2;

struct OutDesc {
    float*  ptr;
    int32_t stride;
    int32_t off;
    int32_t width;
    P16Desc p16;
};

struct NinSrcQuad {
    unsigned long long ptr;
    unsigned stride;
    unsigned valid;
};

struct ConvArgs {
    const float* in;
    P16Desc in16;
    int32_t in_stride;
    int32_t in_off;
    int32_t cin_phys;
    int32_t n_chunks;
    const float* wpack;
    const float* bias;
    const float* alpha;
    int32_t act;
    int32_t N, H, W;
    int32_t tiles_x, tiles_y;
    OutDesc out0, out1;
    int32_t split;
    int32_t ps;
    int32_t ps_c;
    int32_t vec4;
    const float* res;
    int32_t res_stride;
    const float* dww;
    int32_t dwk;
    int32_t n_full;
    int32_t n_groups;
    int32_t group_span;
    int32_t fold;
    const void* srctab;
    const void* wpack16;
    float inv_scale;
    int32_t* redo;
    int32_t tail_octs;
    int32_t redo_check;
    int32_t nt_pack;
};

struct ConvShape {
    int ks, mt, nt, kc;
    int dwk = 0;
    int nin = 0;
    int wino = 0;
};

__host__ __device__ constexpr int conv_ns(int nt) { return (nt & 1) ? nt * 16 : nt * 16 + 16; }
__host__ __device__ constexpr int conv_plane_stride(int halo_pixels) {
    return ((halo_pixels + 15) / 32) * 32 + 16;
}

ConvShape conv_pick_shape(int ks, int nt, int dwk = 0);
size_t conv_lds_bytes(const ConvShape& s);
hipError_t conv_init_kernels();
hipError_t conv_launch(const ConvShape& s, const ConvArgs& a, int n_tiles, hipStream_t stream);
constexpr int kWinoKC = 8;
constexpr int kWinoMaxNT = 3;
hipError_t wino_init_kernels();
hipError_t wino_launch(int nt, const ConvArgs& a, int n_groups, hipStream_t stream);
constexpr int kNinKC = 16;
constexpr int kNinMaxNT = 6;
hipError_t nin_init_kernels();
hipError_t nin_launch(int nt, const ConvArgs& a, int n_groups, hipStream_t stream);
constexpr int kNinHKC = 32;
hipError_t nin_h_init_kernels();
hipError_t nin_h_launch(int nt, const ConvArgs& a, int n_groups, bool w8, hipStream_t stream);
constexpr int kC3hKC = 32;
constexpr int kC3hMaxNT = 6;
inline int c3h_tail_octs(int cin_phys) {
    const int n_chunks = (cin_phys + kC3hKC - 1) / kC3hKC, tail = cin_phys - (n_chunks - 1) * kC3hKC;
    return n_chunks < 2 || tail > 24 ? 0 : (tail + 7) / 8;
}
inline int c3h_tail_steps(int octs) { return (9 * octs + 3) / 4; }
hipError_t c3h_init_kernels();
hipError_t c3h_launch(int nt, const ConvArgs& a, int n_groups, hipStream_t stream);
hipError_t c3e_init_kernels();
bool c3e_eligible(int nt, const ConvArgs& a, int n_groups);
hipError_t c3e_launch(int nt, const ConvArgs& a, int n_groups, int n_cus, hipStream_t stream);
hipError_t c5h_init_kernels();
hipError_t c5h_launch(int nt, const ConvArgs& args, hipStream_t stream);
constexpr int kFoldVariants = 16;
hipError_t c5h_border_launch(const ConvArgs& args, hipStream_t stream);

constexpr int kStreamPX = 48;
constexpr int kStreamRowPx = kStreamPX + 2;
constexpr int kStreamMaxL = 7;
constexpr int kStreamMT = kStreamPX / 16;

struct StreamRing {
    int32_t off;
    int32_t units;
    int32_t quads;
    int32_t slots;
};
struct StreamConv {
    StreamRing in, out;
    int32_t lag;
    int32_t dww;
    int32_t wp;
    int32_t ba;
    int32_t to_global;
    float inv;
};
struct StreamNinSrc {
    StreamRing ring;
    int32_t chunks;
    int32_t w;
    int32_t last_ql;
};
struct StreamArgs {
    const float* x;
    float* out;
    const float* blob;
    int32_t out_stride;
    int32_t N, H, W;
    int32_t n_strips, useful_w, halo;
    int32_t n_blocks, useful_h, rows_c;
    int32_t n_jobs, jobs_per_wg;
    int32_t L, n_conv, total_lag;
    alignas(16) int8_t role[16];
    int32_t ring_bytes, ldsw_bytes, ldsw_src;
    int32_t first_w;
    StreamRing first_out;
    StreamConv conv[kStreamMaxL];
    StreamNinSrc nin[kStreamMaxL];
    StreamRing b1;
    int32_t nin_ba;
    int32_t nb_quads;
    float nin_inv;
    int32_t* redo;
    int32_t redo_check;
};


struct TailArgs {
    const float* c2;
    const float* x2;
    float* y;
    const float* blob;
    int32_t c2_stride;
    int32_t N, H, W;
    int32_t n_strips, useful_w, halo;
    int32_t n_blocks, useful_h, rows_c;
    int32_t n_jobs, jobs_per_wg;
    StreamRing in, u;
    int32_t v_off;
    int32_t ring_bytes, ldsw_bytes;
    int32_t a_dww, a_wp, a_bias;
    int32_t b_dww, b_wp, b_bias;
    float c_w[9];
    float c_scale;
    float a_inv, b_inv;
    int32_t* redo;
    int32_t redo_check;
};
hipError_t tail_launch(const TailArgs& a, int grid, bool f16, hipStream_t stream);
void stream_init_kernels();
hipError_t stream_launch(const StreamArgs& a, int grid, bool f16, hipStream_t stream);

constexpr int kS3MaxL = 8;
constexpr int kS3MaxWaves = 8;
constexpr int kS3RolePair = 32, kS3RoleNin = 16;
struct S3Ring { int32_t off, px, octs; };
struct S3Out {
    P16Desc p16;
    float* ptr;
    int32_t stride, width;
    int32_t lo, hi;
};
struct S3Nin {
    int32_t on;
    int32_t w_off;
    int32_t ba_off;
    float inv;
    S3Ring b1;
};
struct S3Conv {
    S3Ring in, out;
    int32_t lag;
    int32_t w_off;
    int32_t ba_off;
    int32_t tiles;
    float inv;
};
struct Stream3Args {
    const float* x;
    const float* blob;
    int32_t N, H, W;
    int32_t n_strips, useful_w, halo, n_blocks, useful_h, rows_c, n_jobs, jobs_per_wg;
    int32_t L, total_lag, n_waves;
    int8_t role_conv[kS3MaxWaves];
    int32_t first_w;
    S3Ring first_out;
    S3Conv conv[kS3MaxL];
    S3Out out[kS3MaxL];
    S3Nin nin;
    S3Out out2;
    int32_t ring_bytes;
    int32_t* redo;
};
hipError_t stream3_launch(const Stream3Args& a, int grid, hipStream_t stream);

int conv_max_fused_dw_nt();

hipError_t ensemble_gather_launch(const float* in, float* out, int h, int w, int n, hipStream_t stream);
hipError_t ensemble_reduce_launch(const float* y, double* out, int h, int w, int n, hipStream_t stream);

hipError_t rgb_to_y_launch(const uint8_t* rgb, double* y64, float* y32, long long n, hipStream_t stream);
hipError_t rgb_to_ycbcr_launch(const uint8_t* rgb, double* out, long long n, hipStream_t stream);
hipError_t y_cbcr_to_rgb_launch(const double* y64, const float* y32, const double* cbcr, const uint8_t* rgb8, double* out, long long n,
                                hipStream_t stream);

constexpr int kMetricTaps = 11;
struct MetricWeights { double w[kMetricTaps]; };
int metric_segments(int h);
hipError_t metrics_launch(const double* a64, const float* a32, const double* b64, const float* b32, int stride, int border, int h, int w,
                          const MetricWeights& wt, double* part_s, long long* part_e, long long* out, hipStream_t stream);

// ... 53 lines not shown
```

dcscn-super-resolution_amd/csrc/kernels.hip:

```cpp
#include "conv_variants.hpp"
#include "p16.hpp"

namespace dcscn {

ConvShape conv_pick_shape(int ks, int nt, int dwk) { return ConvShape{ks, pick_mt(ks, nt), nt, pick_kc(ks, nt), dwk}; }
size_t conv_lds_bytes(const ConvShape& s) { return lds_bytes_for(s.ks, s.mt, s.nt, s.kc, s.dwk); }
int conv_max_fused_dw_nt() { return kMaxDwNt; }
int conv_max_nt(int ks) { return ks == 7 ? kMaxK7Nt : 13; }

hipError_t conv_init_kernels() {
    hipError_t e = conv_init_k1();
    if (e == hipSuccess) e = conv_init_k3();
    if (e == hipSuccess) e = conv_init_k5();
    if (e == hipSuccess) e = conv_init_k7();
    if (e == hipSuccess) e = wino_init_kernels();
    if (e == hipSuccess) e = nin_init_kernels();
    if (e == hipSuccess) e = nin_h_init_kernels();
    if (e == hipSuccess) e = c3h_init_kernels();
    if (e == hipSuccess) e = c3e_init_kernels();
    if (e == hipSuccess) e = c5h_init_kernels();
    if (e == hipSuccess) stream_init_kernels();
    return e;
}

hipError_t conv_launch(const ConvShape& s, const ConvArgs& a, int n_tiles, hipStream_t stream) {
    if (s.mt != pick_mt(s.ks, s.nt) || s.kc != pick_kc(s.ks, s.nt)) return hipErrorInvalidValue;
    if (s.dwk != 0 && (s.ks != 1 || a.dww == nullptr || a.dwk != s.dwk)) return hipErrorInvalidValue;
    if (s.ks == 1) return conv_launch_k1(s.nt, s.dwk, a, n_tiles, stream);
    if (s.ks == 3) return conv_launch_k3(s.nt, a, n_tiles, stream);
    if (s.ks == 5) return conv_launch_k5(s.nt, a, n_tiles, stream);
    if (s.ks == 7 && s.nt <= kMaxK7Nt) return conv_launch_k7(s.nt, a, n_tiles, stream);
    return hipErrorInvalidValue;
}

template <int KS>
__global__ __launch_bounds__(256) void conv_cin1(const Cin1Args a, int tpp_log2) {
    constexpr int TAPS = KS * KS, HALO = KS / 2, T = 16, HT = T + 2 * HALO;
    extern __shared__ __attribute__((aligned(16))) float smem[];
    const int cs = a.cs, c4n = cs >> 2;
    float* xs = smem;
    float* ws = smem + ((HT * HT + 3) & ~3);
    float* bs = ws + TAPS * cs;
    float* as = bs + cs;

    int bid = blockIdx.x;
    const int tiles_x = (a.W + T - 1) / T, tiles_y = (a.H + T - 1) / T;
    const int tx = bid % tiles_x;
    bid /= tiles_x;
    const int ty = bid % tiles_y;
    const int img = bid / tiles_y;
    const int y0 = ty * T, x0 = tx * T;
    const int tid = threadIdx.x;
    if (a.redo_check && (a.redo[0] == 0 || a.redo[1 + img] == 0)) return;

    const float* xin = a.x + (size_t)img * a.H * a.W;
    for (int i = tid; i < HT * HT; i += 256) {
        const int hy = i / HT, hx = i - hy * HT;
        const int gy = y0 + hy - HALO, gx = x0 + hx - HALO;
        xs[i] = (gy >= 0 && gy < a.H && gx >= 0 && gx < a.W) ? xin[(size_t)gy * a.W + gx] : 0.0f;
    }
    for (int i = tid; i < TAPS * cs; i += 256) ws[i] = a.w[i];
    for (int i = tid; i < cs; i += 256) {
        bs[i] = a.bias[i];
        as[i] = a.alpha[i];
    }
    __syncthreads();

    const int tpp = 1 << tpp_log2;
    const int cl = tid & (tpp - 1);
    const int pl = tid >> tpp_log2;
    const int ppi = 256 >> tpp_log2;
    const bool o16 = a.out.p16.base != nullptr;
    float chk = 0.0f;
    if (o16) {
        const int octs = a.out.p16.octs;
        int t16 = 0;
        while ((1 << t16) < octs && t16 < 6) ++t16;
        const int tpp16 = 1 << t16, cl8 = tid & (tpp16 - 1), pl8 = tid >> t16, ppi8 = 256 >> t16;
        const float m1 = opaque_minus_one();
        const h2 zero2 = p16_opaque_zero2();
        for (int c8 = cl8; c8 < octs; c8 += tpp16) {
            const bool two = 2 * c8 + 1 < c4n;
            f32x4 wr[TAPS][2];
            const f32x4 z4 = {0.0f, 0.0f, 0.0f, 0.0f};
#pragma unroll
            for (int t = 0; t < TAPS; ++t) {
                wr[t][0] = *reinterpret_cast<const f32x4*>(ws + t * cs + 8 * c8);
                wr[t][1] = two ? *reinterpret_cast<const f32x4*>(ws + t * cs + 8 * c8 + 4) : z4;
            }
            const f32x4 bv0 = *reinterpret_cast<const f32x4*>(bs + 8 * c8), bv1 = two ? *reinterpret_cast<const f32x4*>(bs + 8 * c8 + 4) : z4;
            const f32x4 av0 = *reinterpret_cast<const f32x4*>(as + 8 * c8), av1 = two ? *reinterpret_cast<const f32x4*>(as + 8 * c8 + 4) : z4;
            const int chunk = c8 >> 2, rem = octs - 4 * chunk;
            const int rec = rem >= 4 ? 128 : 32 * rem;
            char* plane = a.out.p16.base + (long long)chunk * a.out.p16.plane + 128 + (c8 & 3) * 32;
            for (int p = pl8; p < T * T; p += ppi8) {
                const int py = p >> 4, px = p & 15;
                const int gy = y0 + py, gx = x0 + px;
                if (gy >= a.H || gx >= a.W) continue;
                f32x4 s0 = z4, s1 = z4;
#pragma unroll
                for (int t = 0; t < TAPS; ++t) {
                    const float xv = xs[(py + t / KS) * HT + px + t % KS];
                    s0 += wr[t][0] * xv;
                    s1 += wr[t][1] * xv;
                }
                f32x4 v0 = bv0, v1 = bv1;
                v0 += s0; v1 += s1;
                v0.x = activate1(v0.x, av0.x, a.act); v0.y = activate1(v0.y, av0.y, a.act); v0.z = activate1(v0.z, av0.z, a.act); v0.w = activate1(v0.w, av0.w, a.act);
                if (two) { v1.x = activate1(v1.x, av1.x, a.act); v1.y = activate1(v1.y, av1.y, a.act); v1.z = activate1(v1.z, av1.z, a.act); v1.w = activate1(v1.w, av1.w, a.act); }
                else v1 = z4;
                h8 hi, lo;
                split8(v0, v1, m1, hi, lo);
                const u32x4 hu = __builtin_bit_cast(u32x4, hi);
                chk = p16_check(p16_check(p16_check(p16_check(chk, hu.x, zero2), hu.y, zero2), hu.z, zero2), hu.w, zero2);
                const size_t pix = ((size_t)img * a.H + gy) * a.W + gx;
                *reinterpret_cast<h8*>(plane + pix * rec) = hi;
                *reinterpret_cast<h8*>(plane + pix * rec + 16) = lo;
            }
        }
    } else
    for (int c4 = cl; c4 < c4n; c4 += tpp) {
        f32x4 wr[TAPS];
#pragma unroll
        for (int t = 0; t < TAPS; ++t) wr[t] = *reinterpret_cast<const f32x4*>(ws + t * cs + 4 * c4);
        const f32x4 bv = *reinterpret_cast<const f32x4*>(bs + 4 * c4);
        const f32x4 av = *reinterpret_cast<const f32x4*>(as + 4 * c4);
        for (int p = pl; p < T * T; p += ppi) {
            const int py = p >> 4, px = p & 15;
            const int gy = y0 + py, gx = x0 + px;
            if (gy >= a.H || gx >= a.W) continue;
            f32x4 v = bv;
            f32x4 s = {0.0f, 0.0f, 0.0f, 0.0f};
#pragma unroll
            for (int t = 0; t < TAPS; ++t) {
                const float xv = xs[(py + t / KS) * HT + px + t % KS];
                s += wr[t] * xv;
            }
            v += s;
            v.x = activate1(v.x, av.x, a.act);
            v.y = activate1(v.y, av.y, a.act);
            v.z = activate1(v.z, av.z, a.act);
            v.w = activate1(v.w, av.w, a.act);
            const size_t pix = ((size_t)img * a.H + gy) * a.W + gx;
            *reinterpret_cast<f32x4*>(a.out.ptr + pix * a.out.stride + a.out.off + 4 * c4) = v;
        }
    }
    if (chk != chk && a.redo) { a.redo[0] = 1; a.redo[1 + img] = 1; }
}

hipError_t cin1_launch(const Cin1Args& a, hipStream_t stream) {
    const int tiles = ((a.W + 15) / 16) * ((a.H + 15) / 16);
    const int c4n = a.cs / 4;
    int tpp_log2 = 0;
    while ((1 << tpp_log2) < c4n && tpp_log2 < 6) ++tpp_log2;
    const int halo = a.ks / 2;
    const int ht = 16 + 2 * halo;
    const size_t lds = (size_t)(((ht * ht + 3) & ~3) + (a.ks * a.ks + 2) * a.cs) * sizeof(float);
    const dim3 grid((unsigned)(a.N * tiles));
    if (lds > 64 * 1024) return hipErrorInvalidValue;
    if (a.ks == 3) hipLaunchKernelGGL(conv_cin1<3>, grid, dim3(256), lds, stream, a, tpp_log2);
    else if (a.ks == 1) hipLaunchKernelGGL(conv_cin1<1>, grid, dim3(256), lds, stream, a, tpp_log2);
    else if (a.ks == 5) hipLaunchKernelGGL(conv_cin1<5>, grid, dim3(256), lds, stream, a, tpp_log2);
    else if (a.ks == 7) hipLaunchKernelGGL(conv_cin1<7>, grid, dim3(256), lds, stream, a, tpp_log2);
    else return hipErrorInvalidValue;
    return hipGetLastError();
}

template <int KS, int LPP>
__global__ __launch_bounds__(256) void conv_cout1(const Cout1Args a) {
    constexpr int TAPS = KS * KS, HALO = KS / 2, T = 16, HT = T + 2 * HALO, HP = HT * HT;
    constexpr int SP = (HP + 3) & ~3;
    extern __shared__ __attribute__((aligned(16))) float smem[];
    float* ws = smem;
    float* sp = smem + TAPS * a.cin_phys;

    int bid = blockIdx.x;
    const int tiles_x = (a.W + T - 1) / T, tiles_y = (a.H + T - 1) / T;
    const int tx = bid % tiles_x;
    bid /= tiles_x;
    const int ty = bid % tiles_y;
    const int img = bid / tiles_y;
    const int y0 = ty * T, x0 = tx * T;
    const int tid = threadIdx.x;
    if (a.redo_check && (a.redo[0] == 0 || a.redo[1 + img] == 0)) return;

    for (int i = tid; i < TAPS * a.cin_phys; i += 256) ws[i] = a.w[i];
    __syncthreads();

    const int sub = tid % LPP;
    const int grp = tid / LPP;
    const int nq = a.cin_phys >> 2;
    const float* in_img = a.in + (size_t)img * a.H * a.W * a.in_stride + a.in_off;
    for (int hp = grp; hp < HP; hp += 256 / LPP) {
        const int hy = hp / HT, hx = hp - hy * HT;
        const int gy = y0 + hy - HALO, gx = x0 + hx - HALO;
        float acc[TAPS];
#pragma unroll
        for (int t = 0; t < TAPS; ++t) acc[t] = 0.0f;
        if (gy >= 0 && gy < a.H && gx >= 0 && gx < a.W) {
            const float* px = in_img + ((size_t)gy * a.W + gx) * a.in_stride;
            for (int q = sub; q < nq; q += LPP) {
                const f32x4 v = *reinterpret_cast<const f32x4*>(px + 4 * q);
#pragma unroll
                for (int t = 0; t < TAPS; ++t) {
                    const f32x4 w = *reinterpret_cast<const f32x4*>(ws + t * a.cin_phys + 4 * q);
                    acc[t] += v.x * w.x + v.y * w.y + v.z * w.z + v.w * w.w;
                }
            }
        }
#pragma unroll
        for (int t = 0; t < TAPS; ++t) {
            float s = acc[t];
            if constexpr (LPP >= 2) s += __shfl_xor(s, 1);
            if constexpr (LPP >= 4) s += __shfl_xor(s, 2);
            if constexpr (LPP >= 8) s += __shfl_xor(s, 4);
            if (sub == 0) sp[t * SP + hp] = s;
        }
    }
    __syncthreads();

    const int py = tid >> 4, pxl = tid & 15;
    const int gy = y0 + py, gx = x0 + pxl;
    if (gy < a.H && gx < a.W) {
        float s = 0.0f;
#pragma unroll
        for (int t = 0; t < TAPS; ++t) s += sp[t * SP + (py + t / KS) * HT + pxl + t % KS];
        s = s * a.scale + a.bias;
        const size_t pix = ((size_t)img * a.H + gy) * a.W + gx;
        if (a.res) s += a.res[pix * a.res_stride];
        a.out[pix * a.out_stride] = s;
    }
}

hipError_t cout1_launch(const Cout1Args& a, hipStream_t stream) {
    const int tiles = ((a.W + 15) / 16) * ((a.H + 15) / 16);
    const int halo = a.ks / 2;
    const int hp = (16 + 2 * halo) * (16 + 2 * halo);
    const size_t lds = (size_t)(a.ks * a.ks * a.cin_phys + a.ks * a.ks * ((hp + 3) & ~3)) * sizeof(float);
    if (lds > 64 * 1024) return hipErrorInvalidValue;
    const dim3 grid((unsigned)(a.N * tiles));
    const bool narrow = a.cin_phys <= 8;
    if (a.ks == 3) {
        if (narrow) hipLaunchKernelGGL((conv_cout1<3, 1>), grid, dim3(256), lds, stream, a);
        else hipLaunchKernelGGL((conv_cout1<3, 8>), grid, dim3(256), lds, stream, a);
    } else if (a.ks == 1) {
        if (narrow) hipLaunchKernelGGL((conv_cout1<1, 1>), grid, dim3(256), lds, stream, a);
        else hipLaunchKernelGGL((conv_cout1<1, 8>), grid, dim3(256), lds, stream, a);
    } else if (a.ks == 5) {
        if (narrow) hipLaunchKernelGGL((conv_cout1<5, 1>), grid, dim3(256), lds, stream, a);
        else hipLaunchKernelGGL((conv_cout1<5, 8>), grid, dim3(256), lds, stream, a);
    } else {
        return hipErrorInvalidValue;
    }
    return hipGetLastError();
}

__global__ __launch_bounds__(256) void depthwise_kernel(const DwArgs a, long long total) {
    const long long idx = (long long)blockIdx.x * 256 + threadIdx.x;
    if (idx >= total) return;
    const int c = (int)(idx % a.cout_phys);
    const long long pix = idx / a.cout_phys;
    if (a.redo_check && (a.redo[0] == 0 || a.redo[1 + pix / ((long long)a.H * a.W)] == 0)) return;
    float out = 0.0f;
    if (c < a.cin) {
        const int x = (int)(pix % a.W);
// ... 75 lines not shown
```

dcscn-super-resolution_amd/csrc/plan.h:

```cpp
#pragma once
#include <hip/hip_runtime.h>

#include <algorithm>
#include <cmath>
#include <cstdarg>
#include <cstdio>
#include <cstdlib>
#include <cstring>
#include <map>
#include <string>
#include <vector>

#include "../../include/dcscn.h"
#include "kernels.h"

namespace dcscn_impl {
using namespace dcscn;

inline int pad4(int c) { return (c + 3) & ~3; }
inline int pad16(int c) { return (c + 15) & ~15; }

enum { EXT_X = -1, EXT_X2 = -2, EXT_Y = -3 };
enum OpKind { OP_CONV = 0, OP_CIN1 = 1, OP_DW = 2, OP_COUT1 = 3, OP_STREAM = 4, OP_TAIL = 5, OP_STREAM3 = 6, OP_FOLDX = 7 };
enum Kernel { K_CONV_IGEMM, K_CONV_WINO2, K_CONV_NIN, K_CONV_NIN_H, K_CONV5_H, K_CONV3_H8, K_CONV3_H, K_CONV_CIN1, K_CONV_COUT1, K_DEPTHWISE,
              K_FEAT_STREAM, K_TAIL_STREAM, K_FEAT3_STREAM, K_LAYER_BY_LAYER };
constexpr int kNoSplit = 1 << 30;

struct TensorSpec {
    std::string name;
    std::vector<int64_t> shape;
    std::vector<float> data;
    bool set = false;
};

struct WsBuf {
    int stride = 0;
    int res = 1;
    size_t offset = 0;
    bool p16_ok = false, p16 = false;
    int octs = 0;
    long long plane = 0;
    size_t bytes = 0;
};

inline size_t ws_tensor_bytes(const WsBuf& b, long long npix, bool p16) {
    const size_t bytes = (size_t)npix * b.stride * sizeof(float);
    return p16 && b.p16_ok && b.stride > 0 ? std::max(bytes, (size_t)p16_tensor_bytes(npix, b.octs)) : bytes;
}
inline size_t ws_granules(size_t bytes) { return (bytes + 255) & ~(size_t)255; }

struct ColSeg {
    int w = -1, b = -1, alpha = -1;
    int cout = 0;
    int col0 = 0;
    int dst = 0;
    int dw1 = -1;
};

struct TrainState;
struct TrainBatches;

struct Op {
    OpKind kind = OP_CONV;
    std::string name;
    int ks = 3, cin = 0, cout = 0, res = 1;
    int act = ACT_NONE;
    float const_alpha = 0.0f;
    int in_buf = EXT_X, in_off = 0, cin_phys = 0;
    int in_stride_override = 0;
    std::vector<int> chan_map;
    std::vector<ColSeg> segs;
    int dw_w = -1;
    int dwk = 0;
    float out_scale = 1.0f;
    int tconv_s = 0;
    int fold_s = 0;
    int fold_c = 0;
    int fold_rw = -1;
    int out_buf[2] = {EXT_Y, EXT_Y}, out_off[2] = {0, 0}, out_width[2] = {0, 0};
    int split = kNoSplit;
    int ps = 1, ps_c = 0;
    bool residual = false;
    bool vec4 = true;
    ConvShape shape{3, 2, 1, 4};
    int n_tiles = 1, n_chunks = 0, ctot = 0;
    int n_full = 0;
    int64_t macs = 0, bytes = 0;
    float* d_w = nullptr;
    float* d_bias = nullptr;
    float* d_alpha = nullptr;
    int32_t* d_map = nullptr;
    float* d_dww = nullptr;
    std::vector<std::pair<int, int>> multi;
    std::vector<NinSrcQuad> h_srctab;
    NinSrcQuad* d_srctab = nullptr;
    std::vector<Op> fused;
    StreamArgs stream{};
    TailArgs tail{};
    Stream3Args stream3{};
    std::vector<int> extra_out;
    int halo = -1;
    struct Split16 {
        bool on = false;
        int nt = 0, n_tiles = 0, n_full = 0, n_chunks = 0;
        float inv_scale = 1.0f;
        void* d_w = nullptr;
        float* d_bias = nullptr;
        float* d_alpha = nullptr;
        int tail_octs = 0;
        bool rerun = false;
        bool in16_ok = false;
        std::vector<NinSrcQuad> h_tab16;
        NinSrcQuad* d_tab16 = nullptr;
    } h16;
};

inline bool has_second_dst(const Op& op) { return op.split < (1 << 29); }
template <class F>
inline void for_each_dst(const Op& op, F&& f) {
    f(op.out_buf[0], 0);
    if (has_second_dst(op)) f(op.out_buf[1], 1);
    for (int b : op.extra_out) f(b, 0);
}

}

using namespace dcscn_impl;

struct dcscn_ctx {
    dcscn_config cfg{};
    int device = 0;
    hipStream_t stream = nullptr;
    std::string error;
    bool finalized = false;

    std::vector<int> sched;
    std::vector<TensorSpec> tensors;
    std::map<std::string, int> tensor_index;
    std::vector<dcscn_layer_info> layers;
    std::vector<WsBuf> bufs;
    std::vector<Op> ops;

    void* arena = nullptr;
    size_t arena_bytes = 0;
    int lay_n = 0, lay_h = 0, lay_w = 0;
    float* io_x = nullptr; float* io_x2 = nullptr; float* io_y = nullptr;
    size_t io_x_cap = 0, io_x2_cap = 0, io_y_cap = 0;
    struct ResampleTable { int ksize = 0; int* d_bounds = nullptr; double* d_kk = nullptr; int* d_k8 = nullptr; };
    std::map<std::pair<int, int>, ResampleTable> resample_tables;
    float* rs_tmp = nullptr; size_t rs_tmp_cap = 0;
    float* ens_x = nullptr; float* ens_x2 = nullptr; float* ens_y = nullptr; float* ens_out = nullptr;
    size_t ens_x_cap = 0, ens_x2_cap = 0, ens_y_cap = 0, ens_out_cap = 0;
    float* rs_in = nullptr; float* rs_out = nullptr; size_t rs_in_cap = 0, rs_out_cap = 0;
    float* col_rgb = nullptr; float* col_d = nullptr; float* col_d2 = nullptr; float* col_y32 = nullptr;
    size_t col_rgb_cap = 0, col_d_cap = 0, col_d2_cap = 0, col_y32_cap = 0;
    double* met_buf = nullptr; size_t met_buf_cap = 0;
    float* tile_x = nullptr; float* tile_x2 = nullptr; float* tile_y = nullptr;
    size_t tile_x_cap = 0, tile_x2_cap = 0, tile_y_cap = 0;
    std::vector<void*> device_allocs;

    int64_t sub_batch_pixels = 4 << 20;
    int64_t workspace_budget = (int64_t)48 << 30;
    hipEvent_t done_ev = nullptr;
    std::vector<hipEvent_t> host_ev;
    hipStream_t last_stream = nullptr;
    bool has_last = false;
    bool profile = false;
    unsigned long long* d_digest = nullptr;
    int debug_digest = 0;
    bool conv3_h8 = true;
    bool nin_h8 = true;
    int n_cus = 256;
    int debug_poison = 0;
    bool graph_replay = false;
    struct GraphKey {
        const void *x = nullptr, *x2 = nullptr, *y = nullptr;
        void* stream = nullptr;
        int n = 0, H = 0, W = 0, split16 = 0, nb = 0, h8 = 0, nin_h8 = 0, p16 = 0;
        unsigned long long carve = 0;
        bool operator==(const GraphKey& o) const {
            return x == o.x && x2 == o.x2 && y == o.y && stream == o.stream && n == o.n && H == o.H && W == o.W && split16 == o.split16 && nb == o.nb &&
                   h8 == o.h8 && nin_h8 == o.nin_h8 && p16 == o.p16 && carve == o.carve;
        }
    };
    GraphKey graph_seen, graph_key;
    hipGraphExec_t graph_exec = nullptr;
    bool winograd = true;
    bool stream_tail = true;
    bool stream_nin = true;
    bool stream_dense = true;
    bool stream_features = true;
    int split16_mask = 3;
    bool split16 = true;
    size_t redo_off = 0, redo_ints = 0;
    bool p16 = true;
    bool p16_now = false;
    bool any_p16 = false;
    int p16_max_res = 1;
    bool dense_features = true;
    int concat_buf = -1;
    std::vector<std::pair<int, int>> concat_slices;
    uint64_t carve_gen = 0, tables_gen = 0;
    bool nin = true;
    bool fold_force = false;
    bool fold_tail = true;
    bool fold_whole = true;
    bool spatial_tiling = true;
    std::vector<unsigned long long> h_zrec;
    unsigned long long* d_zrec = nullptr;
    size_t zrec_cap = 0;
    std::vector<hipEvent_t> ev;
    size_t ev_used = 0;
    std::vector<int> ev_op;
    int ev_forwards = 0;
    std::vector<void*> pack_allocs;
    dcscn_impl::TrainState* train = nullptr;
    dcscn_impl::TrainBatches* batches = nullptr;
};

namespace dcscn_impl {

extern thread_local std::string g_global_error;
void set_global_error(const char* fmt, ...);
int fail(dcscn_ctx* h, int code, const char* fmt, ...);

#define HIP_TRY(h, expr)                                                                       \
    do {                                                                                       \
        hipError_t e_ = (expr);                                                                \
        if (e_ != hipSuccess)                                                                  \
            return fail(h, DCSCN_ERR_HIP, "%s failed: %s (%s:%d)", #expr, hipGetErrorString(e_), \
                        __FILE__, __LINE__);                                                   \
    } while (0)

inline float* buf_ptr(dcscn_ctx* h, int id) { return reinterpret_cast<float*>(static_cast<char*>(h->arena) + h->bufs[id].offset); }

void filter_schedule(int layers, int filters, int min_filters, double gamma, std::vector<int>& out);
int kernel_act(int activator, float* const_alpha);
int build_graph(dcscn_ctx* h);
bool nin_eligible(const dcscn_ctx* h, const Op& op);
bool wino_eligible(const dcscn_ctx* h, const Op& op);
bool h16_direct_eligible(const dcscn_ctx* h, const Op& op);
bool fold_linear_tail(dcscn_ctx* h);
bool fold_whole_tail(dcscn_ctx* h);
int stream_chunk_channel(int quads, int ch, int q, int s);
void fuse_feat_stream(dcscn_ctx* h);
void fuse_tail_stream(dcscn_ctx* h);
void fuse_feat3_stream(dcscn_ctx* h);
void densify_features(dcscn_ctx* h);
void plan_p16(dcscn_ctx* h);
inline bool p16_active(const dcscn_ctx* h) { return h->p16 && h->any_p16 && h->split16 && h->split16_mask == 3; }
int upload(dcscn_ctx* h, const void* host, size_t bytes, void** dev);
int finalize_op(dcscn_ctx* h, Op& op);
int pack_feat_stream(dcscn_ctx* h, Op& op);
int pack_tail_stream(dcscn_ctx* h, Op& op);
int pack_feat3_stream(dcscn_ctx* h, Op& op);
int pack_foldx(dcscn_ctx* h, Op& op);
int repack_weights(dcscn_ctx* h);
void train_free(dcscn_ctx* h);
int train_sync_inference(dcscn_ctx* h);
int check_patches(dcscn_ctx* h, const dcscn_patch* p, int n, int lr_size, double max_value);
int build_batch_device(dcscn_ctx* h, const dcscn_patch* p, int n, int lr_size, double max_value, float* x, float* x2, float* y_true,
                       hipStream_t stream);
void train_batches_free(dcscn_ctx* h);
bool op_on_split16(const dcscn_ctx* h, const Op& op);
Kernel op_kernel(const dcscn_ctx* h, const Op& op, bool redo = false);
const char* kernel_name(Kernel k);
int run_forward(dcscn_ctx* h, const float* x, const float* x2, float* y, int n, int H, int W, hipStream_t stream);
int forward_done(dcscn_ctx* h, hipStream_t stream);
int resample_table(dcscn_ctx* h, int in_size, int out_size, const dcscn_ctx::ResampleTable** out);
template <class T>
int grow(dcscn_ctx* h, T** p, size_t* cap, size_t count, hipStream_t stream, int nomem_code = DCSCN_ERR_NOMEM) {
    if (count <= *cap) return DCSCN_OK;
    HIP_TRY(h, hipStreamSynchronize(stream));
    if (*p) HIP_TRY(h, hipFree(*p));
    *p = nullptr;
    *cap = 0;
    hipError_t e = hipMalloc((void**)p, count * sizeof(T));
    if (e != hipSuccess) return fail(h, nomem_code, "buffer of %zu bytes: %s", count * sizeof(T), hipGetErrorString(e));
    *cap = count;
    return DCSCN_OK;
}
int resize_device(dcscn_ctx* h, const float* in, float* out, int n, int H, int W, int OH, int OW, hipStream_t stream);

}
```

dcscn-super-resolution_amd/engine.py:

```python

import ctypes
import os

import numpy as np

from . import build as _build

ABI_VERSION = 4
MAX_NAME = 128

ACTIVATORS = {None: 0, "": 0, "none": 0, "prelu": 1, "relu": 2, "leaky_relu": 3, "sigmoid": 4, "tanh": 5, "selu": 6}

STATUS_NAMES = {0: "OK", 1: "INVALID_ARG", 2: "UNSUPPORTED", 3: "MISSING_TENSOR", 4: "SHAPE", 5: "HIP", 6: "STATE",
                7: "NOMEM"}

EXPORTED_SYMBOLS = (
    "dcscn_abi_version", "dcscn_last_global_error", "dcscn_device_count", "dcscn_filter_schedule", "dcscn_create",
    "dcscn_num_tensors", "dcscn_tensor_info", "dcscn_set_tensor", "dcscn_finalize", "dcscn_num_layers",
    "dcscn_layer_info_get", "dcscn_num_ops", "dcscn_op_info_get", "dcscn_set_option", "dcscn_forward",
    "dcscn_forward_device", "dcscn_forward_ensemble", "dcscn_get_profile", "dcscn_debug_digests", "dcscn_workspace_bytes", "dcscn_num_presplit_tensors",
    "dcscn_last_error", "dcscn_destroy", "dcscn_resize_bicubic", "dcscn_resize_bicubic_device", "dcscn_forward_lr",
    "dcscn_resample_table", "dcscn_get_stream", "dcscn_synchronize", "dcscn_convert_rgb_to_y", "dcscn_convert_rgb_to_ycbcr",
    "dcscn_convert_y_and_cbcr_to_rgb", "dcscn_evaluate_rgb", "dcscn_sr_rgb",
    "dcscn_train_begin", "dcscn_train_step", "dcscn_train_step_device", "dcscn_train_gradients", "dcscn_get_tensor",
    "dcscn_set_train_tensor", "dcscn_train_add_image", "dcscn_train_build_batch", "dcscn_train_step_patches",
    "dcscn_psnr_ssim", "dcscn_evaluate_rgb_metrics",
)

OPTIMIZERS = {"adam": 0, "gd": 1, "momentum": 2, "adadelta": 3, "adagrad": 4, "rmsprop": 5}


class EngineError(RuntimeError):
    def __init__(self, status, message):
        super().__init__("dcscn: %s (%s)" % (message, STATUS_NAMES.get(status, status)))
        self.status = status
        self.message = message


class Config(ctypes.Structure):
    _fields_ = [
        ("struct_size", ctypes.c_int32),
        ("scale", ctypes.c_int32),
        ("layers", ctypes.c_int32),
        ("filters", ctypes.c_int32),
        ("min_filters", ctypes.c_int32),
        ("filters_decay_gamma", ctypes.c_double),
        ("cnn_size", ctypes.c_int32),
        ("use_nin", ctypes.c_int32),
        ("nin_filters", ctypes.c_int32),
        ("nin_filters2", ctypes.c_int32),
        ("reconstruct_layers", ctypes.c_int32),
        ("reconstruct_filters", ctypes.c_int32),
        ("activator", ctypes.c_int32),
        ("pixel_shuffler", ctypes.c_int32),
        ("pixel_shuffler_filters", ctypes.c_int32),
        ("depthwise_separable", ctypes.c_int32),
        ("channels", ctypes.c_int32),
        ("legacy_no_c", ctypes.c_int32),
        ("batch_norm", ctypes.c_int32),
        ("reserved", ctypes.c_int32 * 8),
    ]


class TrainConfig(ctypes.Structure):
    _fields_ = [
        ("struct_size", ctypes.c_int32),
        ("optimizer", ctypes.c_int32),
        ("use_l1_loss", ctypes.c_int32),
        ("reserved0", ctypes.c_int32),
        ("beta1", ctypes.c_double),
        ("beta2", ctypes.c_double),
        ("epsilon", ctypes.c_double),
        ("momentum", ctypes.c_double),
        ("l2_decay", ctypes.c_double),
        ("clipping_norm", ctypes.c_double),
        ("keep_prob", ctypes.c_double),
        ("reserved", ctypes.c_int32 * 8),
    ]


class LayerInfo(ctypes.Structure):
    _fields_ = [
        ("name", ctypes.c_char * MAX_NAME),
        ("kernel_size", ctypes.c_int32),
        ("in_channels", ctypes.c_int32),
        ("out_channels", ctypes.c_int32),
        ("depthwise_separable", ctypes.c_int32),
        ("has_bias", ctypes.c_int32),
        ("activator", ctypes.c_int32),
        ("resolution", ctypes.c_int32),
        ("macs_per_lr_pixel", ctypes.c_int64),
    ]


class OpInfo(ctypes.Structure):
    _fields_ = [
        ("name", ctypes.c_char * MAX_NAME),
        ("kernel", ctypes.c_char * 32),
        ("kernel_size", ctypes.c_int32),
        ("in_channels", ctypes.c_int32),
        ("out_channels", ctypes.c_int32),
        ("resolution", ctypes.c_int32),
        ("mt", ctypes.c_int32),
        ("nt", ctypes.c_int32),
        ("kc", ctypes.c_int32),
        ("n_tiles", ctypes.c_int32),
        ("macs_per_lr_pixel", ctypes.c_int64),
        ("bytes_per_lr_pixel", ctypes.c_int64),
        ("executed_macs_per_lr_pixel", ctypes.c_int64),
    ]


class Metrics(ctypes.Structure):
    _fields_ = [
        ("psnr", ctypes.c_double),
        ("ssim", ctypes.c_double),
        ("sq_err_sum", ctypes.c_int64),
        ("n_pixels", ctypes.c_int64),
    ]


_lib = None


def library_path():
    return _build.LIB_PATH


def load_library():
    global _lib
    if _lib is not None:
        return _lib
    path = library_path()
    if not os.path.isfile(path):
        raise EngineError(5, "HIP extension %s is missing; run `python __graft_entry__.py` (or "
                             "dcscn-super-resolution_amd/build.py) to compile it with hipcc" % path)
    try:
        lib = ctypes.CDLL(path)
    except OSError as exc:
        raise EngineError(5, "cannot load %s: %s" % (path, exc))
    c = ctypes
    fp, dp, vp = c.POINTER(c.c_float), c.POINTER(c.c_double), c.c_void_p
    lib.dcscn_abi_version.restype = c.c_int
    lib.dcscn_last_global_error.restype = c.c_char_p
    lib.dcscn_device_count.restype = c.c_int
    lib.dcscn_filter_schedule.argtypes = [c.c_int, c.c_int, c.c_int, c.c_double, c.POINTER(c.c_int32)]
    lib.dcscn_create.argtypes = [c.POINTER(Config), c.c_int, c.POINTER(vp)]
    lib.dcscn_num_tensors.argtypes = [vp]
    lib.dcscn_tensor_info.argtypes = [vp, c.c_int, c.c_char_p, c.c_int, c.POINTER(c.c_int64), c.POINTER(c.c_int)]
    lib.dcscn_set_tensor.argtypes = [vp, c.c_char_p, fp, c.POINTER(c.c_int64), c.c_int]
    lib.dcscn_finalize.argtypes = [vp]
    lib.dcscn_num_layers.argtypes = [vp]
    lib.dcscn_layer_info_get.argtypes = [vp, c.c_int, c.POINTER(LayerInfo)]
    lib.dcscn_num_ops.argtypes = [vp]
    lib.dcscn_op_info_get.argtypes = [vp, c.c_int, c.POINTER(OpInfo)]
    lib.dcscn_set_option.argtypes = [vp, c.c_char_p, c.c_int64]
    lib.dcscn_forward.argtypes = [vp, fp, fp, fp, c.c_int, c.c_int, c.c_int]
    lib.dcscn_forward_device.argtypes = [vp, vp, vp, vp, c.c_int, c.c_int, c.c_int, vp]
    lib.dcscn_forward_ensemble.argtypes = [vp, fp, fp, dp, c.c_int, c.c_int, c.c_int]
    lib.dcscn_resize_bicubic.argtypes = [vp, fp, fp, c.c_int, c.c_int, c.c_int, c.c_int, c.c_int]
    lib.dcscn_resize_bicubic_device.argtypes = [vp, vp, vp, c.c_int, c.c_int, c.c_int, c.c_int, c.c_int, vp]
    lib.dcscn_forward_lr.argtypes = [vp, fp, fp, c.c_int, c.c_int, c.c_int]
    lib.dcscn_resample_table.argtypes = [c.c_int, c.c_int, c.POINTER(c.c_int), c.POINTER(c.c_int), dp, c.c_int]
    lib.dcscn_get_profile.argtypes = [vp, dp, c.c_int]
    lib.dcscn_debug_digests.argtypes = [vp, c.POINTER(c.c_uint64), c.c_int]
    lib.dcscn_workspace_bytes.argtypes = [vp]
    lib.dcscn_num_presplit_tensors.argtypes = [vp]
    lib.dcscn_get_stream.argtypes = [vp, c.POINTER(vp)]
    u8p = c.POINTER(c.c_uint8)
    lib.dcscn_convert_rgb_to_y.argtypes = [vp, u8p, dp, c.c_int64]
    lib.dcscn_convert_rgb_to_ycbcr.argtypes = [vp, u8p, dp, c.c_int64]
    lib.dcscn_convert_y_and_cbcr_to_rgb.argtypes = [vp, dp, dp, dp, c.c_int64]
    lib.dcscn_evaluate_rgb.argtypes = [vp, u8p, c.c_int, c.c_int, c.c_int, dp, fp, dp]
    lib.dcscn_sr_rgb.argtypes = [vp, u8p, u8p, c.c_int, c.c_int, c.c_int, dp, dp]
    lib.dcscn_psnr_ssim.argtypes = [vp, dp, dp, c.c_int, c.c_int, c.c_int, c.POINTER(Metrics)]
    lib.dcscn_evaluate_rgb_metrics.argtypes = [vp, u8p, c.c_int, c.c_int, c.c_int, c.c_int, c.POINTER(Metrics), c.POINTER(Metrics), dp]
    lib.dcscn_synchronize.argtypes = [vp]
    lib.dcscn_workspace_bytes.restype = c.c_int64
    lib.dcscn_last_error.argtypes = [vp]
    lib.dcscn_last_error.restype = c.c_char_p
    lib.dcscn_destroy.argtypes = [vp]
    lib.dcscn_train_begin.argtypes = [vp, c.POINTER(TrainConfig)]
    lib.dcscn_train_step.argtypes = [vp, fp, fp, fp, c.c_int, c.c_int, c.c_int, c.c_double, c.c_uint64, dp]
    lib.dcscn_train_step_device.argtypes = [vp, vp, vp, vp, c.c_int, c.c_int, c.c_int, c.c_double, c.c_uint64, dp, vp]
    lib.dcscn_train_gradients.argtypes = [vp, fp, fp, fp, c.c_int, c.c_int, c.c_int, c.c_uint64, dp]
    lib.dcscn_get_tensor.argtypes = [vp, c.c_char_p, fp, c.c_int64]
    lib.dcscn_set_train_tensor.argtypes = [vp, c.c_char_p, fp, c.c_int64]
    lib.dcscn_train_add_image.argtypes = [vp, u8p, c.c_int, c.c_int, c.c_int, c.POINTER(c.c_int32)]
    lib.dcscn_train_build_batch.argtypes = [vp, vp, c.c_int, c.c_int, c.c_double, fp, fp, fp]
    lib.dcscn_train_step_patches.argtypes = [vp, vp, c.c_int, c.c_int, c.c_double, c.c_double, c.c_uint64, dp]
    if lib.dcscn_abi_version() != ABI_VERSION:
        raise EngineError(5, "ABI mismatch: library %d, binding %d" % (lib.dcscn_abi_version(), ABI_VERSION))
    _lib = lib
    return lib


def filter_schedule(layers, filters, min_filters, gamma):
    lib = load_library()
    out = (ctypes.c_int32 * layers)()
    rc = lib.dcscn_filter_schedule(layers, filters, min_filters, gamma, out)
    if rc:
        raise EngineError(rc, lib.dcscn_last_global_error().decode())
    return list(out)


def device_count():
    return load_library().dcscn_device_count()


def make_config(cfg):
    get = cfg.get if isinstance(cfg, dict) else (lambda k, d=None: getattr(cfg, k, d))
    c = Config()
    c.struct_size = ctypes.sizeof(Config)
    c.scale = int(get("scale", 2))
    c.layers = int(get("layers", 12))
    c.filters = int(get("filters", 196))
    c.min_filters = int(get("min_filters", 48))
    c.filters_decay_gamma = float(get("filters_decay_gamma", 1.5))
    c.cnn_size = int(get("cnn_size", 3))
    c.use_nin = int(bool(get("use_nin", True)))
    c.nin_filters = int(get("nin_filters", 64))
    c.nin_filters2 = int(get("nin_filters2", 32))
    c.reconstruct_layers = int(get("reconstruct_layers", 1))
    c.reconstruct_filters = int(get("reconstruct_filters", 32))
    act = get("activator", "prelu")
    if act not in ACTIVATORS:
        raise NameError("Not implemented activator:%s" % act)
    c.activator = ACTIVATORS[act]
    c.pixel_shuffler = int(bool(get("pixel_shuffler", True)))
    c.pixel_shuffler_filters = int(get("pixel_shuffler_filters", 0))
    c.depthwise_separable = int(bool(get("depthwise_separable", False)))
    c.channels = int(get("channels", 1))
    c.legacy_no_c = int(bool(get("legacy_no_c", False)))
    c.batch_norm = int(bool(get("batch_norm", False)))
    return c


def make_train_config(flags):
    get = flags.get if isinstance(flags, dict) else (lambda k, d=None: getattr(flags, k, d))
    opt = get("optimizer", "adam")
    if opt not in OPTIMIZERS:
        raise EngineError(1, "unknown optimizer '%s'" % opt)
    c = TrainConfig()
    c.struct_size = ctypes.sizeof(TrainConfig)
    c.optimizer = OPTIMIZERS[opt]
    c.use_l1_loss = int(bool(get("use_l1_loss", False)))
    c.beta1 = float(get("beta1", 0.9))
    c.beta2 = float(get("beta2", 0.999))
    c.epsilon = float(get("epsilon", 1e-8))
    c.momentum = float(get("momentum", 0.9))
    c.l2_decay = float(get("l2_decay", 0.0001))
    c.clipping_norm = float(get("clipping_norm", 5))
    c.keep_prob = float(get("dropout_rate", 0.8))
    return c


def resample_table(in_size, out_size):
    lib = load_library()
    ks = ctypes.c_int(0)
    rc = lib.dcscn_resample_table(int(in_size), int(out_size), ctypes.byref(ks), None, None, 0)
    if rc:
        raise EngineError(rc, "dcscn_resample_table(%d, %d)" % (in_size, out_size))
    bounds = np.zeros((int(out_size), 2), np.int32)
    weights = np.zeros((int(out_size), ks.value), np.float64)
    rc = lib.dcscn_resample_table(int(in_size), int(out_size), ctypes.byref(ks),
                                  bounds.ctypes.data_as(ctypes.POINTER(ctypes.c_int)),
                                  weights.ctypes.data_as(ctypes.POINTER(ctypes.c_double)), weights.size)
    if rc:
        raise EngineError(rc, "dcscn_resample_table(%d, %d)" % (in_size, out_size))
    return bounds, weights


class Engine:

    def __init__(self, cfg, device=0):
        self._lib = load_library()
        self._h = ctypes.c_void_p()
        self.scale = int(cfg.get("scale", 2) if isinstance(cfg, dict) else getattr(cfg, "scale", 2))
        c = make_config(cfg)
        rc = self._lib.dcscn_create(ctypes.byref(c), int(device), ctypes.byref(self._h))
        if rc:
            self._h = ctypes.c_void_p()
            raise EngineError(rc, self._lib.dcscn_last_global_error().decode())
        self.device = int(device)
        self.finalized = False

    def close(self):
        if getattr(self, "_h", None):
            self._lib.dcscn_destroy(self._h)
            self._h = ctypes.c_void_p()

    def __del__(self):
        try:
            self.close()
        except Exception:
            pass

    def __enter__(self):
        return self

    def __exit__(self, *exc):
        self.close()

    def _check(self, rc):
        if rc:
            raise EngineError(rc, self._lib.dcscn_last_error(self._h).decode())

    def tensor_specs(self):
        out = []
        name = ctypes.create_string_buffer(256)
        shape = (ctypes.c_int64 * 4)()
        rank = ctypes.c_int()
        for i in range(self._lib.dcscn_num_tensors(self._h)):
            self._check(self._lib.dcscn_tensor_info(self._h, i, name, 256, shape, ctypes.byref(rank)))
            out.append((name.value.decode(), tuple(shape[j] for j in range(rank.value))))
        return out

    def layers(self):
        out = []
        info = LayerInfo()
# ... 171 lines not shown
    def train_step_patches(self, patches, lr_size, lr, max_value=255.0, dropout_key=0):
        p, ptr = self._patches(patches)
        stats = (ctypes.c_double * 4)()
        self._check(self._lib.dcscn_train_step_patches(self._h, ptr, len(p), int(lr_size), float(max_value), float(lr),
                                                       int(dropout_key) & (2 ** 64 - 1), stats))
        return tuple(stats)

    def _numel(self, name):
        base = name
        for suffix in ("/grad", "/Adam_1", "/Adam", "/Momentum"):
            if name.endswith(suffix):
                base = name[: -len(suffix)]
                break
        if base in ("beta1_power", "beta2_power"):
            return ()
        for n, shape in self.tensor_specs():
            if n == base:
                return shape
        raise EngineError(4, "unknown tensor '%s'" % name)

    def get_tensor(self, name):
        shape = self._numel(name)
        out = np.empty(shape, np.float32)
        self._check(self._lib.dcscn_get_tensor(self._h, name.encode(), out.ctypes.data_as(ctypes.POINTER(ctypes.c_float)), out.size))
        return out

    def set_train_tensor(self, name, array):
        a = np.ascontiguousarray(array, dtype=np.float32)
        self._check(self._lib.dcscn_set_train_tensor(self._h, name.encode(), a.ctypes.data_as(ctypes.POINTER(ctypes.c_float)), a.size))

    @staticmethod
    def _rgb8(image):
        a = np.ascontiguousarray(image)
        if a.dtype != np.uint8 or a.ndim != 3 or a.shape[2] != 3:
            raise EngineError(1, "expected a uint8 RGB image [h, w, 3]")
        return a

    def convert_rgb_to_y(self, image):
        a = self._rgb8(image)
        out = np.empty(a.shape[:2] + (1,), np.float64)
        self._check(self._lib.dcscn_convert_rgb_to_y(self._h, a.ctypes.data_as(ctypes.POINTER(ctypes.c_uint8)),
                                                     out.ctypes.data_as(ctypes.POINTER(ctypes.c_double)), a.shape[0] * a.shape[1]))
        return out

    def convert_rgb_to_ycbcr(self, image):
        a = self._rgb8(image)
        out = np.empty(a.shape, np.float64)
        self._check(self._lib.dcscn_convert_rgb_to_ycbcr(self._h, a.ctypes.data_as(ctypes.POINTER(ctypes.c_uint8)),
                                                         out.ctypes.data_as(ctypes.POINTER(ctypes.c_double)), a.shape[0] * a.shape[1]))
        return out

    def convert_y_and_cbcr_to_rgb(self, y_image, cbcr_image):
        dp = ctypes.POINTER(ctypes.c_double)
        y = np.ascontiguousarray(np.asarray(y_image, np.float64).reshape(y_image.shape[0], y_image.shape[1], -1)[:, :, 0])
        cbcr = np.ascontiguousarray(np.asarray(cbcr_image, np.float64)[:, :, 0:2])
        out = np.empty(y.shape + (3,), np.float64)
        self._check(self._lib.dcscn_convert_y_and_cbcr_to_rgb(self._h, y.ctypes.data_as(dp), cbcr.ctypes.data_as(dp), out.ctypes.data_as(dp), y.size))
        return out

    def evaluate_rgb(self, true_image, n_ensemble=1, want_inputs=False):
        a = self._rgb8(true_image)
        hh, ww = a.shape[:2]
        s = self.scale
        true_y = np.empty((hh, ww, 1), np.float64)
        y = np.empty((hh, ww, 1), np.float64)
        lr = np.empty((hh // s, ww // s, 1), np.float32) if want_inputs else None
        self._check(self._lib.dcscn_evaluate_rgb(self._h, a.ctypes.data_as(ctypes.POINTER(ctypes.c_uint8)), hh, ww, max(1, int(n_ensemble)),
                                                 true_y.ctypes.data_as(ctypes.POINTER(ctypes.c_double)),
                                                 lr.ctypes.data_as(ctypes.POINTER(ctypes.c_float)) if want_inputs else None,
                                                 y.ctypes.data_as(ctypes.POINTER(ctypes.c_double))))
        if n_ensemble <= 1:
            y = y.astype(np.float32)
        return (true_y, y, lr) if want_inputs else (true_y, y)

    def psnr_ssim(self, a, b, border_size=0, full=False):
        a, b = np.asarray(a), np.asarray(b)
        if a.ndim == 2:
            a = a.reshape(a.shape[0], a.shape[1], 1)
        if b.ndim == 2:
            b = b.reshape(b.shape[0], b.shape[1], 1)
        if a.shape != b.shape:
            return None
        if a.ndim != 3 or a.shape[2] != 1:
            raise EngineError(1, "psnr_ssim expects single-channel images, got shape %s" % (a.shape,))
        a = np.ascontiguousarray(a, dtype=np.float64)
        b = np.ascontiguousarray(b, dtype=np.float64)
        dp = ctypes.POINTER(ctypes.c_double)
        out = Metrics()
        self._check(self._lib.dcscn_psnr_ssim(self._h, a.ctypes.data_as(dp), b.ctypes.data_as(dp), a.shape[0], a.shape[1], int(border_size),
                                              ctypes.byref(out)))
        return out if full else (out.psnr, out.ssim)

    def evaluate_rgb_metrics(self, true_image, n_ensemble=1, border_size=0, want_bicubic=False, want_output=False, full=False):
        a = self._rgb8(true_image)
        hh, ww = a.shape[:2]
        model = Metrics()
        bicubic = Metrics() if want_bicubic else None
        y = np.empty((hh, ww, 1), np.float64) if want_output else None
        self._check(self._lib.dcscn_evaluate_rgb_metrics(self._h, a.ctypes.data_as(ctypes.POINTER(ctypes.c_uint8)), hh, ww, max(1, int(n_ensemble)),
                                                         int(border_size), ctypes.byref(model), ctypes.byref(bicubic) if want_bicubic else None,
                                                         y.ctypes.data_as(ctypes.POINTER(ctypes.c_double)) if want_output else None))
        if want_output and n_ensemble <= 1:
            y = y.astype(np.float32)
        pair = (lambda m: m) if full else (lambda m: (m.psnr, m.ssim))
        return pair(model), pair(bicubic) if want_bicubic else None, y

    def sr_rgb(self, image, upscaled_image, n_ensemble=1):
        a, b = self._rgb8(image), self._rgb8(upscaled_image)
        h, w = a.shape[:2]
        s = self.scale
        if b.shape[:2] != (h * s, w * s):
            raise EngineError(1, "the upscaled image must be %d times the input" % s)
        y = np.empty((h * s, w * s, 1), np.float64)
        rgb = np.empty((h * s, w * s, 3), np.float64)
        u8 = ctypes.POINTER(ctypes.c_uint8)
        dp = ctypes.POINTER(ctypes.c_double)
        self._check(self._lib.dcscn_sr_rgb(self._h, a.ctypes.data_as(u8), b.ctypes.data_as(u8), h, w, max(1, int(n_ensemble)),
                                           y.ctypes.data_as(dp), rgb.ctypes.data_as(dp)))
        if n_ensemble <= 1:
            y = y.astype(np.float32)
        return y, rgb

    def forward_ensemble(self, x, x2, n_ensemble):
        x = np.ascontiguousarray(x, dtype=np.float32)
        x2 = np.ascontiguousarray(x2, dtype=np.float32)
        h, w = x.shape[:2]
        s = self.scale
        if x.size != h * w or x2.size != h * s * w * s:
            raise EngineError(1, "forward_ensemble expects single-channel images")
        y = np.empty((h * s, w * s, 1), dtype=np.float64)
        fp = ctypes.POINTER(ctypes.c_float)
        self._check(self._lib.dcscn_forward_ensemble(self._h, x.ctypes.data_as(fp), x2.ctypes.data_as(fp),
                                                     y.ctypes.data_as(ctypes.POINTER(ctypes.c_double)), h, w,
                                                     int(n_ensemble)))
        return y

    def profile(self, with_float32_plan=False):
        n = self._lib.dcscn_num_ops(self._h)
        ms = (ctypes.c_double * (n + 1))()
        self._check(self._lib.dcscn_get_profile(self._h, ms, n + 1))
        return list(ms) if with_float32_plan else list(ms)[:n]

    def debug_digests(self):
        n = self._lib.dcscn_num_ops(self._h) + 1
        out = (ctypes.c_uint64 * n)()
        self._check(self._lib.dcscn_debug_digests(self._h, out, n))
        return [int(v) for v in out]

    def workspace_bytes(self):
        return int(self._lib.dcscn_workspace_bytes(self._h))

    def num_presplit_tensors(self):
        return int(self._lib.dcscn_num_presplit_tensors(self._h))
```

include/dcscn.h:

```cpp
#ifndef DCSCN_H_
#define DCSCN_H_

#include <stdint.h>

#ifdef __cplusplus
extern "C" {
#endif

#define DCSCN_ABI_VERSION 4
#define DCSCN_MAX_NAME 128

typedef struct dcscn_ctx* dcscn_handle;

typedef enum dcscn_status {
    DCSCN_OK = 0,
    DCSCN_ERR_INVALID_ARG = 1,
    DCSCN_ERR_UNSUPPORTED = 2,
    DCSCN_ERR_MISSING_TENSOR = 3,
    DCSCN_ERR_SHAPE = 4,
    DCSCN_ERR_HIP = 5,
    DCSCN_ERR_STATE = 6,
    DCSCN_ERR_NOMEM = 7
} dcscn_status;

typedef enum dcscn_activator {
    DCSCN_ACT_NONE = 0,
    DCSCN_ACT_PRELU = 1,
    DCSCN_ACT_RELU = 2,
    DCSCN_ACT_LEAKY_RELU = 3,
    DCSCN_ACT_SIGMOID = 4,
    DCSCN_ACT_TANH = 5,
    DCSCN_ACT_SELU = 6
} dcscn_activator;

typedef struct dcscn_config {
    int32_t struct_size;
    int32_t scale;
    int32_t layers;
    int32_t filters;
    int32_t min_filters;
    double  filters_decay_gamma;
    int32_t cnn_size;
    int32_t use_nin;
    int32_t nin_filters;
    int32_t nin_filters2;
    int32_t reconstruct_layers;
    int32_t reconstruct_filters;
    int32_t activator;
    int32_t pixel_shuffler;
    int32_t pixel_shuffler_filters;
    int32_t depthwise_separable;
    int32_t channels;
    int32_t legacy_no_c;
    int32_t batch_norm;
    int32_t reserved[8];
} dcscn_config;

typedef struct dcscn_layer_info {
    char    name[DCSCN_MAX_NAME];
    int32_t kernel_size;
    int32_t in_channels;
    int32_t out_channels;
    int32_t depthwise_separable;
    int32_t has_bias;
    int32_t activator;
    int32_t resolution;
    int64_t macs_per_lr_pixel;
} dcscn_layer_info;

int dcscn_abi_version(void);

const char* dcscn_last_global_error(void);

int dcscn_device_count(void);

int dcscn_filter_schedule(int layers, int filters, int min_filters, double gamma, int32_t* out);

int dcscn_create(const dcscn_config* cfg, int device, dcscn_handle* out);

int dcscn_num_tensors(dcscn_handle h);
int dcscn_tensor_info(dcscn_handle h, int index, char* name, int name_capacity, int64_t* shape, int* rank);

int dcscn_set_tensor(dcscn_handle h, const char* name, const float* data, const int64_t* shape, int rank);

int dcscn_finalize(dcscn_handle h);

int dcscn_num_layers(dcscn_handle h);
int dcscn_layer_info_get(dcscn_handle h, int index, dcscn_layer_info* out);

typedef struct dcscn_op_info {
    char    name[DCSCN_MAX_NAME];
    char    kernel[32];
    int32_t kernel_size;
    int32_t in_channels;
    int32_t out_channels;
    int32_t resolution;
    int32_t mt, nt, kc, n_tiles;
    int64_t macs_per_lr_pixel;
    int64_t bytes_per_lr_pixel;
    int64_t executed_macs_per_lr_pixel;
} dcscn_op_info;
int dcscn_num_ops(dcscn_handle h);
int dcscn_op_info_get(dcscn_handle h, int index, dcscn_op_info* out);

int dcscn_set_option(dcscn_handle h, const char* key, int64_t value);

int dcscn_forward(dcscn_handle h, const float* x, const float* x2, float* y, int n, int height, int width);

int dcscn_resize_bicubic(dcscn_handle h, const float* in, float* out, int n, int height, int width,
                         int out_height, int out_width);
int dcscn_resample_table(int in_size, int out_size, int* ksize, int* bounds, double* weights, int capacity);
int dcscn_resize_bicubic_device(dcscn_handle h, const float* in, float* out, int n, int height, int width,
                                int out_height, int out_width, void* stream);

int dcscn_forward_lr(dcscn_handle h, const float* x, float* y, int n, int height, int width);

int dcscn_forward_device(dcscn_handle h, const float* x, const float* x2, float* y,
                         int n, int height, int width, void* stream);

int dcscn_get_stream(dcscn_handle h, void** stream);

int dcscn_synchronize(dcscn_handle h);

int dcscn_forward_ensemble(dcscn_handle h, const float* x, const float* x2, double* y,
                           int height, int width, int n_ensemble);

int dcscn_convert_rgb_to_y(dcscn_handle h, const uint8_t* rgb, double* y, int64_t n_pixels);
int dcscn_convert_rgb_to_ycbcr(dcscn_handle h, const uint8_t* rgb, double* ycbcr, int64_t n_pixels);
int dcscn_convert_y_and_cbcr_to_rgb(dcscn_handle h, const double* y, const double* cbcr, double* rgb, int64_t n_pixels);

int dcscn_evaluate_rgb(dcscn_handle h, const uint8_t* rgb, int height, int width, int n_ensemble,
                       double* true_y, float* lr, double* y);

typedef struct dcscn_metrics {
    double  psnr;
    double  ssim;
    int64_t sq_err_sum;
    int64_t n_pixels;
} dcscn_metrics;

int dcscn_psnr_ssim(dcscn_handle h, const double* a, const double* b, int height, int width, int border_size, dcscn_metrics* out);

int dcscn_evaluate_rgb_metrics(dcscn_handle h, const uint8_t* rgb, int height, int width, int n_ensemble, int border_size,
                               dcscn_metrics* model, dcscn_metrics* bicubic, double* y);

int dcscn_sr_rgb(dcscn_handle h, const uint8_t* rgb, const uint8_t* rgb_upscaled, int height, int width, int n_ensemble,
                 double* y, double* rgb_out);

int dcscn_get_profile(dcscn_handle h, double* ms, int capacity);

int dcscn_debug_digests(dcscn_handle h, uint64_t* out, int capacity);

int64_t dcscn_workspace_bytes(dcscn_handle h);
int dcscn_num_presplit_tensors(dcscn_handle h);

typedef enum dcscn_optimizer {
    DCSCN_OPTIMIZER_ADAM = 0,
    DCSCN_OPTIMIZER_GD = 1,
    DCSCN_OPTIMIZER_MOMENTUM = 2,
    DCSCN_OPTIMIZER_ADADELTA = 3,
    DCSCN_OPTIMIZER_ADAGRAD = 4,
    DCSCN_OPTIMIZER_RMSPROP = 5
} dcscn_optimizer;

typedef struct dcscn_train_config {
    int32_t struct_size;
    int32_t optimizer;
    int32_t use_l1_loss;
    int32_t reserved0;
    double beta1, beta2, epsilon, momentum, l2_decay, clipping_norm;
    double keep_prob;
    int32_t reserved[8];
} dcscn_train_config;

int dcscn_train_begin(dcscn_handle h, const dcscn_train_config* tc);
int dcscn_train_step(dcscn_handle h, const float* x, const float* x2, const float* y_true, int n, int height, int width, double lr,
                     uint64_t dropout_key, double* stats);
int dcscn_train_step_device(dcscn_handle h, const float* x, const float* x2, const float* y_true, int n, int height, int width, double lr,
                            uint64_t dropout_key, double* stats, void* stream);
int dcscn_train_gradients(dcscn_handle h, const float* x, const float* x2, const float* y_true, int n, int height, int width,
                          uint64_t dropout_key, double* stats);

typedef struct dcscn_patch {
    int32_t image, top, left, fliplr;
} dcscn_patch;
int dcscn_train_add_image(dcscn_handle h, const uint8_t* pixels, int height, int width, int channels, int32_t* image_id);
int dcscn_train_build_batch(dcscn_handle h, const dcscn_patch* patches, int n, int lr_size, double max_value, float* x, float* x2,
                            float* y_true);
int dcscn_train_step_patches(dcscn_handle h, const dcscn_patch* patches, int n, int lr_size, double max_value, double lr,
                             uint64_t dropout_key, double* stats);
int dcscn_get_tensor(dcscn_handle h, const char* name, float* out, int64_t count);
int dcscn_set_train_tensor(dcscn_handle h, const char* name, const float* data, int64_t count);

const char* dcscn_last_error(dcscn_handle h);
int dcscn_destroy(dcscn_handle h);

#ifdef __cplusplus
}
#endif
#endif
```

Baseline: 123.5.

## Recompute first cin=1 conv layer octets inside wide NIN h8 kernel

When the first source of a wide 1x1 (NIN) conv is written only by the single-input-channel 3x3 first layer, the NIN h8 kernel now recomputes those input octets on the fly. It loads the 3x3 input window per pixel and the first layer's weights, bias and alpha into LDS, applies the activation and does the f16 hi/lo split, instead of DMA-loading the stored activations. This removes global reads of that feature slice for the NIN layer, at the cost of extra ALU work, more LDS use and added pipeline-staging complexity. The first layer's octet math is moved into a shared helper that the original cin1 kernel also uses.

```diff
diff --git a/dcscn-super-resolution_amd/build.py b/dcscn-super-resolution_amd/build.py
--- a/dcscn-super-resolution_amd/build.py
+++ b/dcscn-super-resolution_amd/build.py
@@ -12,7 +12,7 @@
 LIB_PATH = os.path.join(PKG_DIR, LIB_NAME)
 SOURCES = ["api.hip", "graph.hip", "pack.hip", "exec.hip", "kernels.hip", "resample.hip", "ensemble.hip", "color.hip", "metrics.hip", "conv_k1.hip", "conv_k3.hip", "conv_k5.hip", "conv_k7.hip", "conv_wino2.hip", "conv_nin.hip", "feat_stream.hip", "conv_nin_h.hip", "conv_nin_h_w8.hip", "conv3_h.hip", "conv3_h8.hip", "conv5_h.hip", "conv3_h_p16.hip", "conv3_h8_p16.hip", "feat_stream_redo.hip", "feat3_stream.hip", "train.hip", "train_data.hip"]
 HEADERS = [os.path.join(CSRC, h) for h in ("kernels.h", "plan.h", "conv_igemm.hpp", "conv_wino2.hpp", "conv_nin.hpp", "conv_variants.hpp", "feat_stream.hpp", "tail_stream.hpp", "feat3_stream.hpp",
-                                              "split16.hpp", "split16_pack.hpp", "p16.hpp", "conv_nin_h.hpp", "conv3_h.hpp", "conv3_h8.hpp", "conv5_h.hpp")] + \
+                                              "split16.hpp", "split16_pack.hpp", "p16.hpp", "cin1_octet.hpp", "conv_nin_h.hpp", "conv3_h.hpp", "conv3_h8.hpp", "conv5_h.hpp")] + \
           [os.path.join(INCLUDE, "dcscn.h")]
 ARCH = "gfx950"
 NO_PK_F32 = ["-Xclang", "-target-feature", "-Xclang", "-packed-fp32-ops"]
diff --git a/dcscn-super-resolution_amd/csrc/api.hip b/dcscn-super-resolution_amd/csrc/api.hip
--- a/dcscn-super-resolution_amd/csrc/api.hip
+++ b/dcscn-super-resolution_amd/csrc/api.hip
@@ -198,6 +198,7 @@
     int rc0 = pack_ops(h);
     if (rc0) return rc0;
     plan_p16(h);
+    plan_nin_cin1(h);
     for (Op& op : h->ops) {
         int rc = DCSCN_OK;
         if (op.kind == OP_CONV && op.shape.nin && op.h16.on && op.h16.in16_ok) {
@@ -354,6 +355,10 @@
         h->nin_h8 = value != 0;
         return DCSCN_OK;
     }
+    if (!strcmp(key, "nin_cin1")) {
+        h->nin_cin1 = value != 0;
+        return DCSCN_OK;
+    }
     if (!strcmp(key, "debug_digest")) {
         if ((int)h->ops.size() + 1 > 1024) return fail(h, DCSCN_ERR_UNSUPPORTED, "debug_digest: more than 1023 launches");
         h->debug_digest = value != 0;
@@ -818,6 +823,14 @@
     if (!h->finalized || !p16_active(h)) return 0;
     int n = 0;
     for (const WsBuf& b : h->bufs) n += b.p16_ok && b.stride > 0;
+    return n;
+}
+
+int dcscn_num_computed_octets(dcscn_handle h) {
+    if (!h) return -DCSCN_ERR_INVALID_ARG;
+    if (!h->finalized) return 0;
+    int n = 0;
+    for (const Op& op : h->ops) n += op_nin_cin1_octs(h, op, p16_active(h));
     return n;
 }
 
diff --git a/dcscn-super-resolution_amd/csrc/cin1_octet.hpp b/dcscn-super-resolution_amd/csrc/cin1_octet.hpp
--- /dev/null
+++ b/dcscn-super-resolution_amd/csrc/cin1_octet.hpp
@@ -0,0 +1,49 @@
+#pragma once
+#include "split16.hpp"
+
+namespace dcscn {
+
+__device__ __forceinline__ f32x4 cin1_fma4(const f32x4 w, float x, const f32x4 s) {
+    return f32x4{__builtin_fmaf(w.x, x, s.x), __builtin_fmaf(w.y, x, s.y), __builtin_fmaf(w.z, x, s.z), __builtin_fmaf(w.w, x, s.w)};
+}
+
+template <int ACT_C>
+__device__ __forceinline__ f32x4 cin1_activate4(f32x4 v, const f32x4 al, int act) {
+    const int act_e = ACT_C >= 0 ? ACT_C : act;
+    v.x = activate1(v.x, al.x, act_e); v.y = activate1(v.y, al.y, act_e); v.z = activate1(v.z, al.z, act_e); v.w = activate1(v.w, al.w, act_e);
+    return v;
+}
+
+template <int TAPS, int M, class XF, class WF>
+__device__ __forceinline__ void cin1_octet(XF&& xv, WF&& wq, const f32x4 bv0, const f32x4 bv1, const f32x4 av0, const f32x4 av1, bool two, int act,
+                                           float m1, h8 (&hi)[M], h8 (&lo)[M]) {
+    const f32x4 z4 = {0.0f, 0.0f, 0.0f, 0.0f};
+    f32x4 s0[M], s1[M];
+#pragma unroll
+    for (int m = 0; m < M; ++m) { s0[m] = z4; s1[m] = z4; }
+#pragma unroll
+    for (int t = 0; t < TAPS; ++t) {
+        const f32x4 w0 = wq(t, 0), w1 = two ? wq(t, 1) : z4;
+#pragma unroll
+        for (int m = 0; m < M; ++m) {
+            const float x = xv(m, t);
+            s0[m] = cin1_fma4(w0, x, s0[m]);
+            s1[m] = cin1_fma4(w1, x, s1[m]);
+        }
+    }
+#pragma unroll
+    for (int m = 0; m < M; ++m) {
+        f32x4 v0 = bv0, v1 = bv1;
+        v0 += s0[m]; v1 += s1[m];
+        if (act == ACT_ALPHA) {
+            v0 = cin1_activate4<ACT_ALPHA>(v0, av0, act);
+            v1 = two ? cin1_activate4<ACT_ALPHA>(v1, av1, act) : z4;
+        } else {
+            v0 = cin1_activate4<-1>(v0, av0, act);
+            v1 = two ? cin1_activate4<-1>(v1, av1, act) : z4;
+        }
+        split8(v0, v1, m1, hi[m], lo[m]);
+    }
+}
+
+}
diff --git a/dcscn-super-resolution_amd/csrc/conv_nin_h.hip b/dcscn-super-resolution_amd/csrc/conv_nin_h.hip
--- a/dcscn-super-resolution_amd/csrc/conv_nin_h.hip
+++ b/dcscn-super-resolution_amd/csrc/conv_nin_h.hip
@@ -19,7 +19,6 @@
 
 hipError_t nin_h8_init_kernels();
 hipError_t nin_h8_launch(const ConvArgs& a, int n_groups, hipStream_t stream);
-constexpr int kNinH8MinChunks = 32;
 
 hipError_t nin_h_init_kernels() {
     hipError_t e = nin_h8_init_kernels();
@@ -53,7 +52,7 @@
 
 hipError_t nin_h_launch(int nt, const ConvArgs& a, int n_groups, bool w8, hipStream_t stream) {
     if (a.n_full < 1 || a.n_full > n_groups || (nt == 1 && a.n_full != n_groups) || !a.wpack16) return hipErrorInvalidValue;
-    if (w8 && nt == 6 && a.in16.base && a.n_chunks >= kNinH8MinChunks && a.n_full == n_groups) return nin_h8_launch(a, n_groups, stream);
+    if (w8 && nin_h8_eligible(nt, a.in16.base != nullptr, a.n_chunks, a.n_full, n_groups)) return nin_h8_launch(a, n_groups, stream);
     switch (nt) {
         case 1: return nin_h_launch_one<1>(a, n_groups, stream);
         case 2: return nin_h_launch_one<2>(a, n_groups, stream);
diff --git a/dcscn-super-resolution_amd/csrc/conv_nin_h.hpp b/dcscn-super-resolution_amd/csrc/conv_nin_h.hpp
--- a/dcscn-super-resolution_amd/csrc/conv_nin_h.hpp
+++ b/dcscn-super-resolution_amd/csrc/conv_nin_h.hpp
@@ -2,6 +2,7 @@
 #include "conv_nin.hpp"
 #include "split16.hpp"
 #include "p16.hpp"
+#include "cin1_octet.hpp"
 
 namespace dcscn {
 
@@ -27,10 +28,11 @@
     static_assert(S == 2 || S == 3, "2 or 3 input stages");
 };
 
-template <int NT, int NTV, int SRC, int S, int WAVES, int MT>
+template <int NT, int NTV, int SRC, int S, int WAVES, int MT, int CIN1 = 0>
 __device__ __forceinline__ void conv_nin_h_body(const ConvArgs& a, float* smem, long long pix0, int ntile) {
     using G = NinHGeom<NT, S, WAVES, MT>;
-    constexpr bool MULTI = SRC != 0, IN16 = SRC == 2;
+    constexpr bool MULTI = SRC != 0, IN16 = SRC == 2, C1 = CIN1 != 0;
+    static_assert(!C1 || (IN16 && S == 3), "computed octets: P16 sources, three input stages");
     const int tid = threadIdx.x;
     const int lane = tid & 63;
     const int wave = __builtin_amdgcn_readfirstlane(tid >> 6);
@@ -38,6 +40,9 @@
     const int lk = lane >> 4;
     const long long npix = (long long)a.N * a.H * a.W;
     const unsigned lds0 = (unsigned)(uintptr_t)(__attribute__((address_space(3))) float*)smem;
+    const int ncomp = C1 ? a.cin1.octs : 0;
+    const int f0 = ncomp >> 2;
+    const unsigned c1_base = (unsigned)(G::LDS_BYTES + a.n_chunks * 64);
 
     const int d_kq = (((lane & 7) >> 1) - ((lane >> 4) & 3)) & 3;
     const int dq = 2 * d_kq + ((lane & 1) ^ (d_kq & 1));
@@ -69,18 +74,51 @@
         constexpr int r = decltype(r_)::value;
         if constexpr (MULTI) {
             const char* src = reinterpret_cast<const char*>(((unsigned long long)ent.y << 32) | ent.x) + (unsigned long long)a_pix[r] * ent.z + (IN16 ? (dq & 1) * 16 : 0);
-            glds16v(src, lds0 + stage * G::A_BYTES + (unsigned)(wave + G::W * r) * 1024u);
+            if (!C1 || 4 * chunk + d_kq >= ncomp) glds16v(src, lds0 + stage * G::A_BYTES + (unsigned)(wave + G::W * r) * 1024u);
         } else {
             const int c0 = chunk * G::KC + 4 * dq;
             glds16(a_base, a_off[r] + (unsigned)((c0 < a.cin_phys ? c0 : 0) * 4), lds0 + stage * G::A_BYTES + (unsigned)(wave + G::W * r) * 1024u);
         }
     };
 
+    float xw[G::MT][9];
+    if constexpr (C1) {
+        const unsigned HW = (unsigned)(a.H * a.W);
+        static_for<0, G::MT>([&](auto m_) DCSCN_INL {
+            constexpr int m = decltype(m_)::value;
+            long long p = pix0 + 16 * G::MT * wave + 16 * m + lj;
+            p = p < npix ? p : npix - 1;
+            const unsigned pp = (unsigned)p, img = pp / HW, rr = pp - img * HW;
+            const int py = (int)(rr / (unsigned)a.W), px = (int)(rr - (unsigned)py * (unsigned)a.W);
+            const float* xi = a.cin1.x + (size_t)img * HW;
+            static_for<0, 9>([&](auto t_) DCSCN_INL {
+                constexpr int t = decltype(t_)::value;
+                const int yy = py + t / 3 - 1, xx = px + t % 3 - 1;
+                xw[m][t] = (yy >= 0 && yy < a.H && xx >= 0 && xx < a.W) ? xi[yy * a.W + xx] : 0.0f;
+            });
+        });
+    }
     {
         if constexpr (MULTI)
             for (int i = tid; i < (IN16 ? 4 : 8) * a.n_chunks; i += G::THREADS)
                 *reinterpret_cast<f32x4*>(reinterpret_cast<char*>(smem) + G::LDS_BYTES + 16 * i) = reinterpret_cast<const f32x4*>(a.srctab)[i];
+        if constexpr (C1) {
+            const int cs8 = 8 * ncomp, cs = a.cin1.cs;
+            float* pl = reinterpret_cast<float*>(reinterpret_cast<char*>(smem) + c1_base);
+            for (int i = tid; i < 11 * cs8; i += G::THREADS) {
+                const int row = i / cs8, col = i - row * cs8;
+                float v = 0.0f;
+                if (col < cs) v = row < 9 ? a.cin1.w[row * cs + col] : row == 9 ? a.cin1.bias[col] : a.cin1.alpha[col];
+                pl[i] = v;
+            }
+        }
         __syncthreads();
+    }
+    if constexpr (C1) {
+#pragma unroll
+        for (int m = 0; m < G::MT; ++m)
+#pragma unroll
+            for (int t = 0; t < 9; ++t) asm volatile("" : "+v"(xw[m][t]));
     }
 
     if (tid < NTV * 4) *reinterpret_cast<f32x4*>(reinterpret_cast<char*>(smem) + G::BA_BASE + tid * 16) = reinterpret_cast<const f32x4*>(a.bias + ntile * NT * 16)[tid];
@@ -99,12 +137,32 @@
     typedef const volatile __attribute__((address_space(3))) h8* lds_h8_ptr;
     const float m1 = opaque_minus_one();
 
+    typedef const __attribute__((address_space(3))) f32x4* lds_const_f32x4_ptr;
+    auto cin1_frags = [&](int c, f32x4 (&fa)[G::MT], f32x4 (&fb)[G::MT]) DCSCN_INL {
+        if constexpr (C1) {
+            const int oct = 4 * c + lk;
+            if (oct < ncomp) {
+                const unsigned wl = lds0 + c1_base + (unsigned)oct * 32u, row_bytes = (unsigned)ncomp * 32u;
+                auto wq = [&](int t, int half) DCSCN_INL { return *(lds_const_f32x4_ptr)(uintptr_t)(wl + (unsigned)t * row_bytes + (unsigned)half * 16u); };
+                const bool two = 2 * oct + 1 < (a.cin1.cs >> 2);
+                h8 hi[G::MT], lo[G::MT];
+                cin1_octet<9, G::MT>([&](int m, int t) DCSCN_INL { return xw[m][t]; }, wq, wq(9, 0), wq(9, 1), wq(10, 0), wq(10, 1), two, a.cin1.act, m1, hi, lo);
+                static_for<0, G::MT>([&](auto m_) DCSCN_INL {
+                    constexpr int m = decltype(m_)::value;
+                    fa[m] = __builtin_bit_cast(f32x4, hi[m]);
+                    fb[m] = __builtin_bit_cast(f32x4, lo[m]);
+                });
+            }
+        }
+    };
+
     const int last = a.n_chunks - 1;
     static_for<0, G::B_ROUNDS>([&](auto r_) DCSCN_INL { dma_b(r_, 0, 0); });
     load_ent(0);
     static_for<0, S>([&](auto st_) DCSCN_INL {
         constexpr int st = decltype(st_)::value;
-        static_for<0, G::A_ROUNDS>([&](auto r_) DCSCN_INL { dma_a(r_, last < st ? last : st, st); });
+        const int c = last < st ? last : st;
+        if (!C1 || c >= f0) static_for<0, G::A_ROUNDS>([&](auto r_) DCSCN_INL { dma_a(r_, c, C1 ? (unsigned)(c - f0) : (unsigned)st); });
         load_ent(last < st + 1 ? last : st + 1);
     });
     asm volatile("s_waitcnt vmcnt(0)" ::: "memory");
@@ -112,16 +170,23 @@
     f32x4 xa[G::MT], xb[G::MT];
     static_for<0, G::MT>([&](auto m_) DCSCN_INL {
         constexpr int m = decltype(m_)::value;
-        xa[m] = *(lds_f32x4_ptr)(uintptr_t)(a_lane + m * 16 * G::PSTRIDE);
-        xb[m] = *(lds_f32x4_ptr)(uintptr_t)(a_lane2 + m * 16 * G::PSTRIDE);
-    });
+        if (!C1 || f0 == 0) {
+            xa[m] = *(lds_f32x4_ptr)(uintptr_t)(a_lane + m * 16 * G::PSTRIDE);
+            xb[m] = *(lds_f32x4_ptr)(uintptr_t)(a_lane2 + m * 16 * G::PSTRIDE);
+        } else {
+            xa[m] = f32x4{0.0f, 0.0f, 0.0f, 0.0f}; xb[m] = xa[m];
+        }
+    });
+    cin1_frags(0, xa, xb);
     __syncthreads();
-    unsigned sa = 0;
+    unsigned sa = C1 ? (unsigned)((S - f0 % S) % S) : 0u;
     for (int chunk = 0; chunk < a.n_chunks; ++chunk) {
         const unsigned sb = chunk & 1;
         const int cb = chunk + 1 < last ? chunk + 1 : last;
         const int ca = chunk + S < last ? chunk + S : last;
         const unsigned sn = sa + 1 == S ? 0 : sa + 1;
+        const bool fetch = !C1 || chunk + S >= f0;
+        const bool staged = !C1 || chunk + 1 >= f0;
         const unsigned Bs = b_lane + sb * G::B_STAGE;
         const unsigned An = a_lane + sn * G::A_BYTES, An2 = a_lane2 + sn * G::A_BYTES;
         static_for<0, G::B_ROUNDS>([&](auto r_) DCSCN_INL { dma_b(r_, cb, sb ^ 1); });
@@ -138,16 +203,22 @@
                 acc[m][n] = __builtin_amdgcn_mfma_f32_16x16x32_f16(wl, xh, acc[m][n], 0, 0, 0);
                 acc[m][n] = __builtin_amdgcn_mfma_f32_16x16x32_f16(wh, xl, acc[m][n], 0, 0, 0);
                 acc[m][n] = __builtin_amdgcn_mfma_f32_16x16x32_f16(wh, xh, acc[m][n], 0, 0, 0);
-                if constexpr (m * NTV + n < G::A_ROUNDS) dma_a(std::integral_constant<int, m * NTV + n>{}, ca, sa);
+                if constexpr (m * NTV + n < G::A_ROUNDS) { if (fetch) dma_a(std::integral_constant<int, m * NTV + n>{}, ca, sa); }
             });
             if constexpr (m == G::MT - 1 && G::MT * NTV < G::A_ROUNDS)
-                static_for<G::MT * NTV, G::A_ROUNDS>([&](auto r_) DCSCN_INL { dma_a(r_, ca, sa); });
-            na[m] = *(lds_f32x4_ptr)(uintptr_t)(An + m * 16 * G::PSTRIDE);
-            nb[m] = *(lds_f32x4_ptr)(uintptr_t)(An2 + m * 16 * G::PSTRIDE);
+                static_for<G::MT * NTV, G::A_ROUNDS>([&](auto r_) DCSCN_INL { if (fetch) dma_a(r_, ca, sa); });
+            if (staged) {
+                na[m] = *(lds_f32x4_ptr)(uintptr_t)(An + m * 16 * G::PSTRIDE);
+                nb[m] = *(lds_f32x4_ptr)(uintptr_t)(An2 + m * 16 * G::PSTRIDE);
+            } else {
+                na[m] = f32x4{0.0f, 0.0f, 0.0f, 0.0f}; nb[m] = na[m];
+            }
         });
+        if (C1 && 4 * (chunk + 1) < ncomp) cin1_frags(chunk + 1, na, nb);
         load_ent(chunk + S + 1 < last ? chunk + S + 1 : last);
         if constexpr (S == 2) asm volatile("s_waitcnt vmcnt(0)" ::: "memory");
-        else asm volatile("s_waitcnt vmcnt(%0)" ::"n"(G::A_ROUNDS) : "memory");
+        else if (fetch) asm volatile("s_waitcnt vmcnt(%0)" ::"n"(G::A_ROUNDS) : "memory");
+        else asm volatile("s_waitcnt vmcnt(0)" ::: "memory");
         __syncthreads();
         static_for<0, G::MT>([&](auto m_) DCSCN_INL { xa[decltype(m_)::value] = na[decltype(m_)::value]; xb[decltype(m_)::value] = nb[decltype(m_)::value]; });
         sa = sn;
@@ -227,13 +298,13 @@
     });
 }
 
-template <int NT, int SRC = 0, int S = 2, int WPS = 2, int WAVES = 4, int MT = 2>
+template <int NT, int SRC = 0, int S = 2, int WPS = 2, int WAVES = 4, int MT = 2, int CIN1 = 0>
 __global__ __launch_bounds__(64 * WAVES, (WPS * WAVES / 4) * 128 / (16 * MT * WAVES) > 0 ? (WPS * WAVES / 4) * 128 / (16 * MT * WAVES) : 1) void conv_nin_h(const ConvArgs a) {
     extern __shared__ __attribute__((aligned(16))) float smem[];
     const long long pix0 = (long long)blockIdx.x * NinHGeom<NT, S, WAVES, MT>::PIX;
     const int ntile = blockIdx.y;
-    if (ntile < a.n_full) conv_nin_h_body<NT, NT, SRC, S, WAVES, MT>(a, smem, pix0, ntile);
-    else if constexpr (NT >= 2) conv_nin_h_body<NT, NT - 1, SRC, S, WAVES, MT>(a, smem, pix0, ntile);
+    if (ntile < a.n_full) conv_nin_h_body<NT, NT, SRC, S, WAVES, MT, CIN1>(a, smem, pix0, ntile);
+    else if constexpr (NT >= 2 && CIN1 == 0) conv_nin_h_body<NT, NT - 1, SRC, S, WAVES, MT>(a, smem, pix0, ntile);
 }
 
 }
diff --git a/dcscn-super-resolution_amd/csrc/conv_nin_h_w8.hip b/dcscn-super-resolution_amd/csrc/conv_nin_h_w8.hip
--- a/dcscn-super-resolution_amd/csrc/conv_nin_h_w8.hip
+++ b/dcscn-super-resolution_amd/csrc/conv_nin_h_w8.hip
@@ -6,9 +6,16 @@
 constexpr int kNinH8MaxTable = 16 * 1024;
 constexpr int kNinH8Waves = 8, kNinH8Tiles = 2;
 
+constexpr int kNinH8MaxCin1 = kNinCin1MaxOcts * 11 * 8 * 4;
+static_assert(NinHGeom<6, kNinH8Stages, kNinH8Waves, kNinH8Tiles>::LDS_BYTES + kNinH8MaxTable + kNinH8MaxCin1 <= 160 * 1024, "LDS of a CU");
+
 hipError_t nin_h8_init_kernels() {
-    return hipFuncSetAttribute(reinterpret_cast<const void*>(&conv_nin_h<6, 2, kNinH8Stages, 2, kNinH8Waves, kNinH8Tiles>),
-                               hipFuncAttributeMaxDynamicSharedMemorySize, NinHGeom<6, kNinH8Stages, kNinH8Waves, kNinH8Tiles>::LDS_BYTES + kNinH8MaxTable);
+    hipError_t e = hipFuncSetAttribute(reinterpret_cast<const void*>(&conv_nin_h<6, 2, kNinH8Stages, 2, kNinH8Waves, kNinH8Tiles>),
+                                       hipFuncAttributeMaxDynamicSharedMemorySize, NinHGeom<6, kNinH8Stages, kNinH8Waves, kNinH8Tiles>::LDS_BYTES + kNinH8MaxTable);
+    if (e != hipSuccess) return e;
+    return hipFuncSetAttribute(reinterpret_cast<const void*>(&conv_nin_h<6, 2, kNinH8Stages, 2, kNinH8Waves, kNinH8Tiles, 1>),
+                               hipFuncAttributeMaxDynamicSharedMemorySize,
+                               NinHGeom<6, kNinH8Stages, kNinH8Waves, kNinH8Tiles>::LDS_BYTES + kNinH8MaxTable + kNinH8MaxCin1);
 }
 
 hipError_t nin_h8_launch(const ConvArgs& a, int n_groups, hipStream_t stream) {
@@ -17,7 +24,15 @@
     const size_t table = (size_t)a.n_chunks * 64;
     if (!a.in16.base || !a.srctab || table > (size_t)kNinH8MaxTable || npix > kP16MaxPixels) return hipErrorInvalidValue;
     const dim3 grid((unsigned)((npix + G::PIX - 1) / G::PIX), (unsigned)n_groups);
-    hipLaunchKernelGGL((conv_nin_h<6, 2, kNinH8Stages, 2, kNinH8Waves, kNinH8Tiles>), grid, dim3(G::THREADS), G::LDS_BYTES + table, stream, a);
+    if (a.cin1.octs > 0) {
+        if (a.cin1.octs > kNinCin1MaxOcts || a.cin1.octs >= 4 * a.n_chunks || a.n_chunks <= kNinH8Stages || 8 * a.cin1.octs < a.cin1.cs ||
+            !a.cin1.x || !a.cin1.w || !a.cin1.bias || !a.cin1.alpha)
+            return hipErrorInvalidValue;
+        const size_t cin1 = (size_t)a.cin1.octs * 11 * 8 * 4;
+        hipLaunchKernelGGL((conv_nin_h<6, 2, kNinH8Stages, 2, kNinH8Waves, kNinH8Tiles, 1>), grid, dim3(G::THREADS), G::LDS_BYTES + table + cin1, stream, a);
+    } else {
+        hipLaunchKernelGGL((conv_nin_h<6, 2, kNinH8Stages, 2, kNinH8Waves, kNinH8Tiles>), grid, dim3(G::THREADS), G::LDS_BYTES + table, stream, a);
+    }
     return hipGetLastError();
 }
 
diff --git a/dcscn-super-resolution_amd/csrc/exec.hip b/dcscn-super-resolution_amd/csrc/exec.hip
--- a/dcscn-super-resolution_amd/csrc/exec.hip
+++ b/dcscn-super-resolution_amd/csrc/exec.hip
@@ -76,6 +76,11 @@
         all16 = all16 && o; any16 = any16 || o;
     });
     return in16 ? all16 : !any16;
+}
+
+int op_nin_cin1_octs(const dcscn_ctx* h, const Op& op, bool p16) {
+    if (!h->nin_cin1 || !h->nin_h8 || !p16 || op.h16.cin1_op < 0 || !op.h16.in16_ok || !op_on_split16(h, op)) return 0;
+    return op.h16.cin1_octs;
 }
 
 
@@ -318,6 +323,10 @@
     if (op.out_buf[0] >= 0 && h->bufs[op.out_buf[0]].p16) b.out0.p16 = p16_desc(h, op.out_buf[0]);
     if (op.out_buf[1] >= 0 && h->bufs[op.out_buf[1]].p16) b.out1.p16 = p16_desc(h, op.out_buf[1]);
     if (kernel == K_CONV_NIN_H) {
+        if (const int octs = op_nin_cin1_octs(h, op, h->p16_now)) {
+            const Op& c1 = h->ops[op.h16.cin1_op];
+            b.cin1 = NinCin1{p.x, c1.d_w, c1.d_bias, c1.d_alpha, c1.act, c1.out_width[0], octs, 0};
+        }
         HIP_TRY(h, nin_h_launch(op.h16.nt, b, op.h16.n_tiles, h->nin_h8, p.stream));
     } else if (kernel == K_CONV5_H) {
         b.bias = op.h16.d_bias;
@@ -595,6 +604,7 @@
     gkey.nb = nb;
     gkey.h8 = h->conv3_h8 ? 1 : 0;
     gkey.nin_h8 = h->nin_h8 ? 1 : 0;
+    gkey.nin_cin1 = h->nin_cin1 ? 1 : 0;
     gkey.p16 = h->p16_now ? 1 : 0;
     gkey.carve = (unsigned long long)h->carve_gen;
     const bool graphs = h->graph_replay && !h->profile && !h->debug_digest && !h->debug_poison;
diff --git a/dcscn-super-resolution_amd/csrc/graph.hip b/dcscn-super-resolution_amd/csrc/graph.hip
--- a/dcscn-super-resolution_amd/csrc/graph.hip
+++ b/dcscn-super-resolution_amd/csrc/graph.hip
@@ -795,4 +795,24 @@
     }
 }
 
-}
+void plan_nin_cin1(dcscn_ctx* h) {
+    for (Op& op : h->ops) {
+        op.h16.cin1_op = -1;
+        op.h16.cin1_octs = 0;
+        if (op.kind != OP_CONV || !op.shape.nin || !op.h16.on || !op.h16.in16_ok || op.multi.size() < 2 || op.res != 1) continue;
+        if (!nin_h8_eligible(op.h16.nt, true, op.h16.n_chunks, op.h16.n_full, op.h16.n_tiles)) continue;
+        const int src = op.multi[0].first;
+        int writer = -1, writers = 0;
+        for (size_t i = 0; i < h->ops.size(); ++i)
+            for_each_dst(h->ops[i], [&](int b, int) { if (b == src) { writer = (int)i; ++writers; } });
+        if (writers != 1) continue;
+        const Op& c1 = h->ops[writer];
+        if (c1.kind != OP_CIN1 || c1.ks != 3 || c1.in_buf != EXT_X || c1.res != 1 || c1.out_off[0] != 0 || c1.out_width[0] != h->bufs[src].stride) continue;
+        const int octs = h->bufs[src].octs;
+        if (octs < 1 || octs > kNinCin1MaxOcts || octs >= 4 * op.h16.n_chunks) continue;
+        op.h16.cin1_op = writer;
+        op.h16.cin1_octs = octs;
+    }
+}
+
+}
diff --git a/dcscn-super-resolution_amd/csrc/kernels.h b/dcscn-super-resolution_amd/csrc/kernels.h
--- a/dcscn-super-resolution_amd/csrc/kernels.h
+++ b/dcscn-super-resolution_amd/csrc/kernels.h
@@ -28,6 +28,17 @@
     int32_t width;
     P16Desc p16;
 };
+
+struct NinCin1 {
+    const float* x;
+    const float* w;
+    const float* bias;
+    const float* alpha;
+    int32_t act, cs;
+    int32_t octs;
+    int32_t pad_;
+};
+constexpr int kNinCin1MaxOcts = 64;
 
 struct NinSrcQuad {
     unsigned long long ptr;
@@ -68,6 +79,7 @@
     int32_t tail_octs;
     int32_t redo_check;
     int32_t nt_pack;
+    NinCin1 cin1;
 };
 
 struct ConvShape {
@@ -96,6 +108,8 @@
 hipError_t nin_launch(int nt, const ConvArgs& a, int n_groups, hipStream_t stream);
 constexpr int kNinHKC = 32;
 hipError_t nin_h_init_kernels();
+constexpr int kNinH8MinChunks = 32;
+inline bool nin_h8_eligible(int nt, bool in16, int n_chunks, int n_full, int n_groups) { return nt == 6 && in16 && n_chunks >= kNinH8MinChunks && n_full == n_groups; }
 hipError_t nin_h_launch(int nt, const ConvArgs& a, int n_groups, bool w8, hipStream_t stream);
 constexpr int kC3hKC = 32;
 constexpr int kC3hMaxNT = 6;
diff --git a/dcscn-super-resolution_amd/csrc/kernels.hip b/dcscn-super-resolution_amd/csrc/kernels.hip
--- a/dcscn-super-resolution_amd/csrc/kernels.hip
+++ b/dcscn-super-resolution_amd/csrc/kernels.hip
@@ -1,5 +1,6 @@
 #include "conv_variants.hpp"
 #include "p16.hpp"
+#include "cin1_octet.hpp"
 
 namespace dcscn {
 
@@ -97,20 +98,10 @@
                 const int py = p >> 4, px = p & 15;
                 const int gy = y0 + py, gx = x0 + px;
                 if (gy >= a.H || gx >= a.W) continue;
-                f32x4 s0 = z4, s1 = z4;
-#pragma unroll
-                for (int t = 0; t < TAPS; ++t) {
-                    const float xv = xs[(py + t / KS) * HT + px + t % KS];
-                    s0 += wr[t][0] * xv;
-                    s1 += wr[t][1] * xv;
-                }
-                f32x4 v0 = bv0, v1 = bv1;
-                v0 += s0; v1 += s1;
-                v0.x = activate1(v0.x, av0.x, a.act); v0.y = activate1(v0.y, av0.y, a.act); v0.z = activate1(v0.z, av0.z, a.act); v0.w = activate1(v0.w, av0.w, a.act);
-                if (two) { v1.x = activate1(v1.x, av1.x, a.act); v1.y = activate1(v1.y, av1.y, a.act); v1.z = activate1(v1.z, av1.z, a.act); v1.w = activate1(v1.w, av1.w, a.act); }
-                else v1 = z4;
-                h8 hi, lo;
-                split8(v0, v1, m1, hi, lo);
+                h8 hi1[1], lo1[1];
+                cin1_octet<TAPS, 1>([&](int, int t) { return xs[(py + t / KS) * HT + px + t % KS]; }, [&](int t, int half) { return wr[t][half]; },
+                                    bv0, bv1, av0, av1, two, a.act, m1, hi1, lo1);
+                const h8 hi = hi1[0], lo = lo1[0];
                 const u32x4 hu = __builtin_bit_cast(u32x4, hi);
                 chk = p16_check(p16_check(p16_check(p16_check(chk, hu.x, zero2), hu.y, zero2), hu.z, zero2), hu.w, zero2);
                 const size_t pix = ((size_t)img * a.H + gy) * a.W + gx;
diff --git a/dcscn-super-resolution_amd/csrc/plan.h b/dcscn-super-resolution_amd/csrc/plan.h
--- a/dcscn-super-resolution_amd/csrc/plan.h
+++ b/dcscn-super-resolution_amd/csrc/plan.h
@@ -110,6 +110,7 @@
         int tail_octs = 0;
         bool rerun = false;
         bool in16_ok = false;
+        int cin1_op = -1, cin1_octs = 0;
         std::vector<NinSrcQuad> h_tab16;
         NinSrcQuad* d_tab16 = nullptr;
     } h16;
@@ -170,17 +171,18 @@
     int debug_digest = 0;
     bool conv3_h8 = true;
     bool nin_h8 = true;
+    bool nin_cin1 = true;
     int n_cus = 256;
     int debug_poison = 0;
     bool graph_replay = false;
     struct GraphKey {
         const void *x = nullptr, *x2 = nullptr, *y = nullptr;
         void* stream = nullptr;
-        int n = 0, H = 0, W = 0, split16 = 0, nb = 0, h8 = 0, nin_h8 = 0, p16 = 0;
+        int n = 0, H = 0, W = 0, split16 = 0, nb = 0, h8 = 0, nin_h8 = 0, nin_cin1 = 0, p16 = 0;
         unsigned long long carve = 0;
         bool operator==(const GraphKey& o) const {
             return x == o.x && x2 == o.x2 && y == o.y && stream == o.stream && n == o.n && H == o.H && W == o.W && split16 == o.split16 && nb == o.nb &&
-                   h8 == o.h8 && nin_h8 == o.nin_h8 && p16 == o.p16 && carve == o.carve;
+                   h8 == o.h8 && nin_h8 == o.nin_h8 && nin_cin1 == o.nin_cin1 && p16 == o.p16 && carve == o.carve;
         }
     };
     GraphKey graph_seen, graph_key;
@@ -248,6 +250,7 @@
 void fuse_feat3_stream(dcscn_ctx* h);
 void densify_features(dcscn_ctx* h);
 void plan_p16(dcscn_ctx* h);
+void plan_nin_cin1(dcscn_ctx* h);
 inline bool p16_active(const dcscn_ctx* h) { return h->p16 && h->any_p16 && h->split16 && h->split16_mask == 3; }
 int upload(dcscn_ctx* h, const void* host, size_t bytes, void** dev);
 int finalize_op(dcscn_ctx* h, Op& op);
@@ -263,6 +266,7 @@
                        hipStream_t stream);
 void train_batches_free(dcscn_ctx* h);
 bool op_on_split16(const dcscn_ctx* h, const Op& op);
+int op_nin_cin1_octs(const dcscn_ctx* h, const Op& op, bool p16);
 Kernel op_kernel(const dcscn_ctx* h, const Op& op, bool redo = false);
 const char* kernel_name(Kernel k);
 int run_forward(dcscn_ctx* h, const float* x, const float* x2, float* y, int n, int H, int W, hipStream_t stream);
diff --git a/dcscn-super-resolution_amd/engine.py b/dcscn-super-resolution_amd/engine.py
--- a/dcscn-super-resolution_amd/engine.py
+++ b/dcscn-super-resolution_amd/engine.py
@@ -18,7 +18,7 @@
     "dcscn_abi_version", "dcscn_last_global_error", "dcscn_device_count", "dcscn_filter_schedule", "dcscn_create",
     "dcscn_num_tensors", "dcscn_tensor_info", "dcscn_set_tensor", "dcscn_finalize", "dcscn_num_layers",
     "dcscn_layer_info_get", "dcscn_num_ops", "dcscn_op_info_get", "dcscn_set_option", "dcscn_forward",
-    "dcscn_forward_device", "dcscn_forward_ensemble", "dcscn_get_profile", "dcscn_debug_digests", "dcscn_workspace_bytes", "dcscn_num_presplit_tensors",
+    "dcscn_forward_device", "dcscn_forward_ensemble", "dcscn_get_profile", "dcscn_debug_digests", "dcscn_workspace_bytes", "dcscn_num_presplit_tensors", "dcscn_num_computed_octets",
     "dcscn_last_error", "dcscn_destroy", "dcscn_resize_bicubic", "dcscn_resize_bicubic_device", "dcscn_forward_lr",
     "dcscn_resample_table", "dcscn_get_stream", "dcscn_synchronize", "dcscn_convert_rgb_to_y", "dcscn_convert_rgb_to_ycbcr",
     "dcscn_convert_y_and_cbcr_to_rgb", "dcscn_evaluate_rgb", "dcscn_sr_rgb",
@@ -166,6 +166,7 @@
     lib.dcscn_debug_digests.argtypes = [vp, c.POINTER(c.c_uint64), c.c_int]
     lib.dcscn_workspace_bytes.argtypes = [vp]
     lib.dcscn_num_presplit_tensors.argtypes = [vp]
+    lib.dcscn_num_computed_octets.argtypes = [vp]
     lib.dcscn_get_stream.argtypes = [vp, c.POINTER(vp)]
     u8p = c.POINTER(c.c_uint8)
     lib.dcscn_convert_rgb_to_y.argtypes = [vp, u8p, dp, c.c_int64]
@@ -643,3 +644,6 @@
 
     def num_presplit_tensors(self):
         return int(self._lib.dcscn_num_presplit_tensors(self._h))
+
+    def num_computed_octets(self):
+        return int(self._lib.dcscn_num_computed_octets(self._h))
diff --git a/include/dcscn.h b/include/dcscn.h
--- a/include/dcscn.h
+++ b/include/dcscn.h
@@ -153,6 +153,7 @@
 
 int64_t dcscn_workspace_bytes(dcscn_handle h);
 int dcscn_num_presplit_tensors(dcscn_handle h);
+int dcscn_num_computed_octets(dcscn_handle h);
 
 typedef enum dcscn_optimizer {
     DCSCN_OPTIMIZER_ADAM = 0,
```

Result: no change. 124.3, median of 6 (+0.7%).
